# NJUVISION/PCGCv2

Measured on AMD Instinct MI355X. Metric: encode+decode Mpoints/sec at fixed bpp (r3 ckpt), vox10 frame, higher is better.
Workload: dtype f32

## Files before the change

### include/pcgc_hip.h

```cpp
#ifndef PCGC_HIP_H
#define PCGC_HIP_H

#include <stddef.h>
#include <stdint.h>

#ifdef __cplusplus
extern "C" {
#endif

const char* pcgc_last_error(void);
int pcgc_version(void);

int64_t pcgc_hash_capacity(int64_t n);
int pcgc_hash_clear(uint64_t* keys , int32_t* vals , int64_t cap, void* stream);
int pcgc_hash_insert(const int32_t* coords , int64_t n, int32_t stride, uint64_t* keys, int32_t* vals,
                     int64_t cap, void* stream);
int pcgc_hash_insert_policy(const int32_t* coords, int64_t n, int32_t stride, uint64_t* keys, int32_t* vals, int64_t cap,
                            int keep_last, void* stream);
int pcgc_hash_first_mask(const int32_t* coords, int64_t n, int32_t stride, const uint64_t* keys, const int32_t* vals,
                         int64_t cap, uint8_t* keep , int32_t* first_row , void* stream);

int pcgc_coords_check_order(const int32_t* coords , int64_t n, int32_t* out2 , void* stream);

int pcgc_coords_quantize(const int32_t* coords, int64_t n, int32_t stride_out, int32_t* out , void* stream);
int pcgc_coords_children(const int32_t* coords, int64_t n, int32_t stride_in, int32_t* out , void* stream);
int pcgc_coords_scale(const int32_t* coords, int64_t n, float factor, int32_t* out , void* stream);

size_t pcgc_scan_workspace_bytes(int64_t n);
int pcgc_mask_scan(const uint8_t* mask , int64_t n, int32_t* prefix , int32_t* total ,
                   void* workspace , size_t workspace_bytes, void* stream);
int pcgc_mask_scan_zeroed(const uint8_t* mask, int64_t n, int32_t* prefix, int32_t* total, void* workspace, size_t workspace_bytes,
                          void* stream);
int pcgc_compact_coords(const int32_t* coords, const uint8_t* mask, const int32_t* prefix, int64_t n,
                        int32_t* out , void* stream);
int pcgc_compact_feats(const float* in, int C, int in_ld, const uint8_t* mask, const int32_t* prefix, int64_t n,
                       float* out , void* stream);

int pcgc_kmap_k3(const int32_t* coords, int64_t n, int32_t stride, const uint64_t* keys, const int32_t* vals,
                 int64_t cap, int32_t* nbr , void* stream);

int pcgc_kmap_k3_children(const int32_t* parent_nbr, int64_t n_parent, int32_t* nbr , void* stream);
int pcgc_kmap_k3_prune(const int32_t* cand_nbr , int64_t n_cand, const uint8_t* mask, const int32_t* prefix,
                       const int32_t* orig , int64_t n_out, int32_t* nbr , void* stream);
int pcgc_kmap_k3_prune_parent(const int32_t* parent_nbr , int64_t n_parent, const uint8_t* mask,
                              const int32_t* prefix, const int32_t* orig, int64_t n_out, int32_t* nbr , void* stream);
int pcgc_kmap_k3_from_coarse(const int32_t* fine , int64_t n_fine, int32_t stride_fine,
                             const int32_t* parent_of , const int32_t* coarse_nbr ,
                             const int32_t* down , int64_t n_coarse, int32_t* nbr ,
                             void* stream);
int pcgc_down_maps(const int32_t* fine, const int32_t* first_row, const int32_t* prefix, int64_t n_fine, int32_t stride_fine,
                   int64_t n_coarse, int32_t* parent_of , int32_t* down , void* stream);
int pcgc_down_prepare(const int32_t* fine , int64_t n, int32_t stride_fine, int32_t* q ,
                      uint64_t* keys, int32_t* vals, int64_t cap, uint8_t* keep , int32_t* first_row ,
                      int32_t* prefix , int32_t* total , void* scan_ws, size_t scan_ws_bytes, void* stream);
int pcgc_down_finish(const int32_t* fine, const int32_t* q, const uint8_t* keep, const int32_t* first_row, const int32_t* prefix,
                     int64_t n, int32_t stride_fine, int64_t n_coarse, int32_t* coarse ,
                     int32_t* parent_of , int32_t* down , void* stream);
int pcgc_down_level(const int32_t* fine , int64_t n, int32_t stride_fine, int32_t* q, uint64_t* keys, int32_t* vals,
                    int64_t cap, uint8_t* keep, int32_t* first_row, int32_t* prefix, int32_t* total, void* scan_ws,
                    size_t scan_ws_bytes, int32_t* coarse , int32_t* parent_of ,
                    int32_t* down , int64_t* n_coarse_out , void* stream);
size_t pcgc_pyramid_scratch_bytes(int64_t n, int levels);
int pcgc_pyramid(const int32_t* fine , int64_t n, int32_t stride, int levels, void* scratch, size_t scratch_bytes,
                 int32_t* const* coarse, int32_t* const* parent_of, int32_t* const* down, int64_t* counts , void* stream);
int pcgc_compact_index(const uint8_t* mask, const int32_t* prefix, int64_t n, int32_t* orig , void* stream);

int pcgc_conv_gather(const int32_t* nbr, int K, int64_t n_out, const float* in, int64_t n_in , int Cin,
                     int in_ld, int in_coff, const float* W, const float* bias, const float* residual, int res_ld,
                     int res_coff, int relu, float* out, int Cout, int out_ld, int out_coff, void* stream);
int pcgc_last_conv_impl(void);
int pcgc_conv_gather_unit(const int32_t* nbr , int K, int64_t n_out, const float* W, const float* bias, int relu,
                          float* out, int Cout, int out_ld, void* stream);
int pcgc_conv_unit_from_coarse(const int32_t* fine , int64_t n_fine, int32_t stride_fine, const int32_t* parent_of,
                               const int32_t* coarse_nbr , const int32_t* down , int64_t n_coarse,
                               const float* W , const float* bias, int relu, float* out, int Cout, int out_ld, void* stream);
int pcgc_set_conv_impl(int impl);
int pcgc_set_up2_impl(int mfma);
int pcgc_irn_block(const int32_t* nbr , int64_t n, const float* x , int C, int x_ld,
                   const float* const* params, float* t_scratch, float* out, int out_ld, void* stream);
int pcgc_irn_pass(const int32_t* nbr, int64_t n, const float* x, int C, int x_ld, const float* const* params,
                  float* t_scratch, float* out, int out_ld, int pass, void* stream);
int pcgc_conv_up2(int64_t n_in, const float* in, int Cin, int in_ld, const float* W , const float* bias,
                  int relu, float* out , int Cout, void* stream);
int pcgc_conv_up2_gather(int64_t n_in, const float* in, int Cin, int in_ld, const int32_t* rows, const float* W ,
                         const float* bias, int relu, float* out , int Cout, void* stream);

int pcgc_conv_child(const int32_t* parent_nbr , int64_t n_parent, const float* in ,
                    int Cin, int in_ld, const float* table , int64_t table_bytes,
                    const float* bias, const float* residual, int res_ld, int relu, float* out, int Cout, int out_ld, void* stream);
int pcgc_irn_child_pass(const int32_t* parent_nbr, int64_t n_parent, int C, int pass, const float* in, int in_ld,
                        const float* table, int64_t table_bytes, const float* b0, const float* b1, const float* b2,
                        const float* x, int x_ld, float* out, int out_ld, void* stream);
int pcgc_irn_child_q4(const int32_t* parent_nbr, int64_t n_parent, int C, int pass, const float* in, int in_ld,
                      const float* table, int64_t table_bytes, const float* b0, const float* b1, const float* b2,
                      const float* x, int x_ld, float* out, int out_ld, void* stream);
int pcgc_cls_child_q4(const int32_t* parent_nbr, int64_t n_parent, const float* in, int Cin, int in_ld, const float* table,
                      int64_t table_bytes, const float* bias, float* out, void* stream);
int pcgc_irn_rows_pass(const int32_t* nbr, int64_t n, int C, int pass, const float* in, int in_ld, const float* table,
                       int64_t table_bytes, const float* b0, const float* b1, const float* b2, const float* x, int x_ld, float* out,
                       int out_ld, void* stream);
int pcgc_irn_rows_q4_pass(const int32_t* nbr, int64_t n, int C, int pass, const float* in, int in_ld, const float* table,
                          int64_t table_bytes, const float* b0, const float* b1, const float* b2, const float* x, int x_ld, float* out,
                          int out_ld, void* stream);
int pcgc_set_rows_q4_variant(int v);
int pcgc_conv_rows(const int32_t* nbr, int64_t n, const float* in, int Cin, int in_ld, const float* table, int64_t table_bytes,
                   const float* bias, const float* residual, int res_ld, int relu, float* out, int Cout, int out_ld, void* stream);
int pcgc_conv_down_rows(const int32_t* down, int64_t n_coarse, const float* in, int64_t n_in, int Cin, int in_ld, const float* table,
                        int64_t table_bytes, const float* bias, int relu, float* out, int Cout, int out_ld, void* stream);

int pcgc_conv_packed64(const int32_t* nbr, int64_t n, const float* in, int in_ld, const float* table, int64_t table_bytes,
                       const float* bias, int relu, float* out, int out_ld, void* stream);
int pcgc_set_packed_tuning(int rows, int waves);

int pcgc_set_convention(int what, int value);

size_t pcgc_topk_workspace_bytes(int64_t n);
int pcgc_topk_mask(const float* logits , int ld, int64_t n, int64_t k, uint8_t* mask ,
                   void* workspace, size_t workspace_bytes, void* stream);
int pcgc_topk_mask_segments(const float* logits, int ld, int nseg, const int64_t* seg_rows, const int64_t* seg_k, uint8_t* mask,
                            void* workspace, size_t workspace_bytes, void* stream);
size_t pcgc_topk_select_workspace_bytes(int64_t n);
int pcgc_topk_select(const float* logits , int ld, int nseg, const int64_t* seg_rows, const int64_t* seg_k,
                     const int32_t* coords, const int32_t* parent_coords, int32_t parent_stride,
                     uint8_t* bits, int32_t* wprefix, int32_t* orig, int32_t* out_coords, void* workspace, size_t workspace_bytes, void* stream);
int pcgc_kmap_k3_prune_sel(const int32_t* cand_nbr , int64_t n_cand, const uint8_t* bits, const int32_t* wprefix,
                           const int32_t* orig , int64_t n_out, int32_t* nbr , void* stream);
int pcgc_kmap_k3_prune_parent_sel(const int32_t* parent_nbr , int64_t n_parent, const uint8_t* bits, const int32_t* wprefix,
                                  const int32_t* orig, int64_t n_out, int32_t* nbr , void* stream);
int pcgc_gather_rows_f32_ld(const float* in, int C, int in_ld, const int32_t* orig, int64_t n_out, float* out , void* stream);
int pcgc_batch_counts(const int32_t* coords , int64_t n, int32_t* counts , void* stream);

size_t pcgc_sort_workspace_bytes(int64_t n);
int pcgc_sort_zyx(const int32_t* coords, int64_t n, int32_t* perm , void* workspace, size_t workspace_bytes,
                  void* stream);
int pcgc_sort_bzyx(const int32_t* coords, int64_t n, int32_t* perm , void* workspace, size_t workspace_bytes, void* stream);
int pcgc_gather_rows_i32x4(const int32_t* in, const int32_t* perm, int64_t n, int32_t* out, void* stream);
int pcgc_gather_rows_f32(const float* in, int C, const int32_t* perm, int64_t n, float* out, void* stream);

int pcgc_relu(const float* in, int64_t count, float* out, void* stream);
int pcgc_add(const float* a, const float* b, int64_t count, float* out, void* stream);

int pcgc_round_minmax(const float* feats, int64_t count, float* minmax , void* stream);
int pcgc_symbolize(const float* feats, int64_t count, float min_v, int16_t* sym , void* stream);
int pcgc_desymbolize(const int16_t* sym, int64_t count, float min_v, float* feats, void* stream);
int pcgc_quantize_symbols(const float* feats, int64_t count, float* minmax , int16_t* sym , void* stream);
int pcgc_quantize_symbols_segments(const float* feats, int C, int nseg, const int64_t* seg_rows, float* minmax, int16_t* sym, void* stream);
int pcgc_cdf_table(const float* params , int C, float min_v, float max_v, uint16_t* cdf_u16 ,
                   float* cdf_f32 , void* stream);


size_t pcgc_loss_workspace_bytes(int64_t elements);
int pcgc_hash_contains(const int32_t* coords , int64_t n, const uint64_t* keys, const int32_t* vals, int64_t cap,
                       const uint8_t* or_mask , uint8_t* mask , void* stream);
int pcgc_eb_likelihood(const float* feats, int ld, int64_t n, int C, const float* params , float bound, float* likelihood,
                       double* bits, void* workspace, size_t workspace_bytes, void* stream);
int pcgc_neg_log2_sum(const float* x, int ld, int64_t n, int C, double* bits , void* workspace, size_t workspace_bytes, void* stream);
int pcgc_bce_logits(const float* logits, int64_t ld, int64_t n, const uint8_t* truth , const uint8_t* pred ,
                    double* bce, int64_t* counts, void* workspace, size_t workspace_bytes, void* stream);

size_t pcgc_occ_workspace_bytes(int64_t n);
int pcgc_occ_symbols(const float* logits, int64_t ld, int64_t n, const uint8_t* truth , uint16_t* packed ,
                     int64_t* sums , void* workspace, size_t workspace_bytes, void* stream);
int pcgc_occ_tables(uint16_t* p1, int32_t* cost);

size_t pcgc_occ_rans_workspace_bytes(int64_t n, int steps);
int pcgc_occ_rans_encode(const uint16_t* packed , int64_t n, int steps, const int64_t* sums , uint8_t* payload,
                         size_t payload_capacity, int64_t* host3, void* workspace, size_t workspace_bytes, void* stream);
int pcgc_occ_rans_decode(const uint16_t* packed , int64_t n, const uint8_t* payload, int64_t payload_bytes, int steps,
                         uint8_t* mask , int64_t* host2, void* workspace, size_t workspace_bytes, void* stream);

size_t pcgc_conv_wgrad_workspace_bytes(int K, int64_t n_rows, int Cin, int Cout);
int64_t pcgc_conv_wgrad_rows_per_group(int K, int64_t n_rows, int Cin, int Cout);
int pcgc_conv_wgrad(const int32_t* nbr, int K, int64_t n_out, const float* x, int64_t n_in, int Cin, int x_ld, const float* gy, int Cout,
                    int gy_ld, float* gW, float* gb, void* workspace, size_t workspace_bytes, void* stream);
int pcgc_conv_up2_wgrad(int64_t n_in, const float* x, int64_t x_rows, int Cin, int x_ld, const int32_t* rows, const float* gy, int Cout,
                        int gy_ld, float* gW, float* gb, void* workspace, size_t workspace_bytes, void* stream);
int pcgc_kmap_invert(const int32_t* nbr, int K, int64_t n_out, int64_t n_in, int32_t* inv , void* stream);
int pcgc_relu_bwd(const float* g, int g_ld, const float* y, int y_ld, int64_t n, int C, float* out, int out_ld, void* stream);
int pcgc_scatter_rows(const float* gy, int C, int gy_ld, const int32_t* orig, int64_t n_rows, float* gx, int64_t n_out, int gx_ld, void* stream);
int pcgc_bce_logits_bwd(const float* logits, int64_t ld, int64_t n, const uint8_t* truth, double scale, float* g , void* stream);
size_t pcgc_eb_bwd_workspace_bytes(int64_t n, int C);
int pcgc_eb_likelihood_bwd(const float* feats, int ld, int64_t n, int C, const float* params , float bound, double scale,
                           float* gy, float* gparams, void* workspace, size_t workspace_bytes, void* stream);

int64_t pcgc_rc_encode(const uint16_t* cdf , int C, int Lp, const int16_t* sym , int64_t n,
                       uint8_t* out , int64_t cap);
int pcgc_rc_decode(const uint16_t* cdf, int C, int Lp, const uint8_t* in, int64_t nbytes, int16_t* sym, int64_t n);
#define PCGC_RC_CKPT_WORDS 6
int64_t pcgc_rc_encode_indexed(const uint16_t* cdf, int C, int Lp, const int16_t* sym, int64_t n, uint8_t* out, int64_t cap, int n_ckpt,
                               uint32_t* ckpt );
int pcgc_rc_decode_indexed(const uint16_t* cdf, int C, int Lp, const uint8_t* in, int64_t nbytes, int16_t* sym, int64_t n, int n_ckpt,
                           const uint32_t* ckpt);
int64_t pcgc_rc_encode_ctx(const uint16_t* cdf , int R, int Lp, const uint16_t* ctx , const int16_t* sym ,
                           int64_t n, uint8_t* out , int64_t cap);
int pcgc_rc_decode_ctx(const uint16_t* cdf, int R, int Lp, const uint16_t* ctx , const uint8_t* in, int64_t nbytes,
                       int16_t* sym , int64_t n);
int pcgc_set_rc_threads(int threads);
int pcgc_set_rc_lanes(int mode);
int pcgc_set_rc_impl(int impl);

int64_t pcgc_oct_encode(const int32_t* xyz , int64_t n, uint8_t* out, int64_t cap);
int64_t pcgc_oct_decode_count(const uint8_t* in, int64_t nbytes);
int pcgc_oct_decode(const uint8_t* in, int64_t nbytes, int32_t* xyz , int64_t n);
int pcgc_set_oct_tiled(int on);
int pcgc_set_oct_model(int model);
int pcgc_oct_warm(void);

int pcgc_d1_nn(const int32_t* a , int64_t na, const uint64_t* b_keys, const int32_t* b_vals, int64_t b_cap,
               const int32_t* offsets , int n_offsets, double* sum , uint64_t* max_d2 ,
               int32_t* unresolved , void* stream);
int pcgc_d1_cell_masks(const int32_t* b , int64_t nb, const uint64_t* cell_keys, const int32_t* cell_vals, int64_t cell_cap,
                       uint64_t* masks , int64_t n_cells, void* stream);
int pcgc_d1_nn_cells(const int32_t* a , int64_t na, const uint64_t* cell_keys, const int32_t* cell_vals, int64_t cell_cap,
                     const uint64_t* masks, const int32_t* offsets , int n_offsets, int32_t reach2, double* sum, uint64_t* max_d2,
                     int32_t* unresolved, void* stream);

int pcgc_d2_runs(const int32_t* qs , int64_t nq, int32_t* runlen , void* stream);
int pcgc_d2_count(const int32_t* p , int64_t n, const int32_t* sel, const uint64_t* cell_keys, const int32_t* cell_vals,
                  int64_t cell_cap, const uint64_t* masks, const uint64_t* keys, const int32_t* vals, int64_t cap, const int32_t* runlen,
                  const int32_t* offsets , int n_offsets, int32_t reach2, int64_t* best , int32_t* cnt ,
                  int32_t* unresolved , int32_t* n_unresolved , void* stream);
int pcgc_d2_fill(const int32_t* p, int64_t n, const int32_t* sel, const uint64_t* cell_keys, const int32_t* cell_vals, int64_t cell_cap,
                 const uint64_t* masks, const uint64_t* keys, const int32_t* vals, int64_t cap, const int32_t* runlen, const int32_t* perm,
                 const int32_t* offsets, int n_offsets, int32_t reach2, const int64_t* best, const int64_t* seg , int32_t* rows, void* stream);
int pcgc_d2_exhaustive(const int32_t* p, int64_t n, const int32_t* sel, const int32_t* qs, int64_t nq, const int32_t* perm, int fill,
                       int64_t* best, int32_t* cnt, const int64_t* seg, int32_t* rows, int32_t* n_empty , void* stream);
size_t pcgc_d2_scan_workspace_bytes(int64_t n);
int pcgc_d2_scan(const int32_t* cnt , int64_t n, int64_t* seg , void* workspace, size_t workspace_bytes, void* stream);
int pcgc_d2_segment_lowest(const int64_t* seg, int64_t n, int32_t* rows, int32_t cap, int32_t* kept, void* stream);
int pcgc_d2_recv_count(const int64_t* seg, const int32_t* kept, int64_t na, const int32_t* rows, int64_t nb, int32_t* rcnt, void* stream);
int pcgc_d2_recv_fill(const int64_t* seg, const int32_t* kept, int64_t na, const int32_t* rows, int64_t nb, const int64_t* rseg, int32_t* cursor,
                      int32_t* recv, void* stream);
int pcgc_d2_normals(const int64_t* rseg, const int32_t* recv, int64_t nb, const double* na, const int64_t* seg_ba, const int32_t* kept_ba,
                    const int32_t* rows_ba, double* nb_out, void* stream);
int pcgc_d2_c2p(const int32_t* p, int64_t n, const int32_t* q, const double* nq, const int64_t* seg, const int32_t* kept, const int32_t* rows,
                double* c2p, void* stream);
size_t pcgc_d2_reduce_workspace_bytes(void);
int pcgc_d2_reduce(const int64_t* c2c, const double* c2p, int64_t n, int64_t* c2c_sum_max, double* c2p_sum, void* workspace, size_t workspace_bytes,
                   void* stream);

size_t pcgc_attr_transfer_workspace_bytes(int64_t ns, int64_t nt, int channels);
int pcgc_attr_transfer(const int64_t* seg_st, const int32_t* kept_st, const int32_t* rows_st, int64_t ns, const int64_t* seg_ts,
                       const int32_t* kept_ts, const int32_t* rows_ts, int64_t nt, const uint8_t* attr_s, int channels, uint8_t* attr_t,
                       void* workspace, size_t workspace_bytes, void* stream);
int pcgc_colour_dist(const uint8_t* cp, int64_t n, const uint8_t* cq, int64_t nq, const int64_t* seg, const int32_t* kept, const int32_t* rows,
                     int64_t* yuv2, int32_t* rgb2, void* stream);
size_t pcgc_colour_reduce_workspace_bytes(void);
int pcgc_colour_reduce(const int64_t* yuv2, const int32_t* rgb2, int64_t n, int64_t* out, void* workspace, size_t workspace_bytes, void* stream);

int64_t pcgc_normals_ball_masks(int32_t r2, uint64_t* table );
size_t pcgc_normals_workspace_bytes(int64_t n);
int pcgc_normals_estimate(const int32_t* coords , int64_t n, const int32_t* qs , const int32_t* perm,
                          const uint64_t* cell_keys, const int32_t* cell_vals, int64_t cell_cap, const uint64_t* masks, const uint64_t* keys,
                          const int32_t* vals, int64_t cap, const int32_t* runlen, const uint64_t* ball , int32_t r2, int orient,
                          const double* viewpoint , int64_t* moments , double* normals ,
                          double* lam , int32_t* count , uint8_t* valid , void* workspace,
                          size_t workspace_bytes, void* stream);
int pcgc_set_normals_mapping(int mode);

int64_t pcgc_ply_read_ascii_geo(const char* path, int32_t* xyz , int64_t cap);
int pcgc_ply_write_ascii_geo(const char* path, const int32_t* xyz , int64_t n);
int pcgc_ply_write_ascii_geo_rgb(const char* path, const int32_t* xyz , const uint8_t* rgb , int64_t n);

typedef int (*pcgc_table_fn)(const float* params, int C, float min_v, float max_v, uint16_t* table_u16, float* cdf_f32);
int pcgc_items_encode(int n_items, const char* const* stems, const int16_t* sym, const int32_t* xyz, const int64_t* rows, const float* ranges,
                      int C, const int32_t* counts, const float* eb_params, pcgc_table_fn table_fn, int index_segments, int write_coords,
                      int threads);
int pcgc_items_probe(int n_items, const char* const* stems, int64_t* rows, int32_t* channels, float* ranges, int32_t* counts,
                     int32_t* native_coords);
int pcgc_items_decode(int n_items, const char* const* stems, const int64_t* rows, int C, const float* ranges, const int32_t* native_coords,
                      const float* eb_params, pcgc_table_fn table_fn, int use_sidecar, int16_t* sym, int32_t* xyz, int coord_layout,
                      int coord_scale, int threads);

int pcgc_level_prepare_children(const int32_t* coords, int64_t n, int32_t stride, uint64_t* keys, int32_t* vals, int64_t cap, int32_t* nbr,
                                int32_t* children, int32_t* nbr_children, void* stream);

int pcgc_frame_decode(const char* stem, int C, const float* eb_params, pcgc_table_fn table_fn, int use_sidecar, int coord_scale,
                      int64_t cap_rows, int16_t* sym, int32_t* level, int64_t* info, float* range, int threads);
int pcgc_frame_decode_begin(const char* stem, int C, const float* eb_params, pcgc_table_fn table_fn, int use_sidecar, int coord_scale,
                            int64_t cap_rows, int16_t* sym, int32_t* level, int64_t* info, float* range, int threads);
int pcgc_frame_decode_end(void);
int pcgc_frame_worker_test(int delay_us);

int pcgc_table_cache(int mode);

uint32_t pcgc_crc32(uint32_t crc, const uint8_t* buf, int64_t len);

int pcgc_mesh_read(const char* path, double* verts , int64_t vcap, int32_t* faces , int64_t fcap,
                   int64_t* counts );
size_t pcgc_mesh_cdf_workspace_bytes(int64_t T);
int pcgc_mesh_area_cdf(const double* verts , int64_t V, const int32_t* faces , int64_t T,
                       double* cdf , int32_t* bad_faces , void* workspace, size_t workspace_bytes, void* stream);
int pcgc_mesh_sample(const double* verts, int64_t V, const int32_t* faces, const double* cdf, int64_t T, uint64_t seed, uint64_t first,
                     int64_t n, int32_t* tri , double* points , void* stream);
size_t pcgc_mesh_voxelize_workspace_bytes(int32_t resolution);
int pcgc_mesh_voxelize(const double* verts, int64_t V, const int32_t* faces, const double* cdf, int64_t T, uint64_t seed, int64_t n,
                       const double* R , int32_t resolution, int32_t* out , int64_t cap,
                       int32_t* count , void* workspace , size_t workspace_bytes, void* stream);

#define PCGC_COLLATE_MAX_ITEMS 16
typedef struct pcgc_collate_item {
    int64_t offset;
    int32_t first_row, rows, width, symmetry, extent, reserved;
} pcgc_collate_item;
int pcgc_collate_rows(const uint8_t* arena , const pcgc_collate_item* items , int n_items,
                      int32_t* coords_out , float* feats_out , void* stream);

#ifdef __cplusplus
}
#endif
#endif
```

### pcgcv2_amd/_build.py

```python
import os
import subprocess
import sys
from concurrent.futures import ThreadPoolExecutor

HERE = os.path.dirname(os.path.abspath(__file__))
CSRC = os.path.join(HERE, 'csrc')
VARIANT = os.environ.get('PCGC_BUILD_VARIANT', '')
OBJ = os.path.join(CSRC, '_obj' + ('_' + VARIANT if VARIANT else ''))
LIB = os.path.join(HERE, 'libpcgc_hip' + ('_' + VARIANT if VARIANT else '') + '.so')
SOURCES = ['coords.hip', 'select.hip', 'conv.hip', 'child_conv.hip', 'child_conv32.hip', 'child_cls_w.hip', 'child_irn.hip', 'child_irn_a16.hip', 'child_irn_b16.hip',
           'child_irn_a32.hip', 'child_irn_b32.hip', 'child_q4.hip', 'rows_irn.hip', 'rows_q4.hip', 'conv_packed.hip', 'entropy.hip', 'loss.hip', 'occupancy.hip', 'occupancy_rans.hip', 'grad.hip', 'metric.hip', 'colour.hip', 'normals.hip', 'mesh.hip', 'collate.hip', 'hostcodec.cpp', 'ply.cpp', 'mesh_io.cpp']
HEADERS = [os.path.join(CSRC, 'pcgc_common.h'), os.path.join(CSRC, 'mfma_util.h'), os.path.join(CSRC, 'child_kernels.h'), os.path.join(CSRC, 'child_q4.h'), os.path.join(CSRC, 'q4x.h'), os.path.join(CSRC, 'q4x_sched.h'), os.path.join(CSRC, 'rows_q4_policy.h'), os.path.join(CSRC, 'eb_logits.h'), os.path.join(CSRC, 'occupancy_tables.h'), os.path.join(HERE, '..', 'include', 'pcgc_hip.h')]
FLAGS = ['--offload-arch=gfx950', '-O3', '-std=c++17', '-ffp-contract=off', '-fPIC', '-Wall', '-Wno-unused-result'] + \
        os.environ.get('PCGC_EXTRA_HIPCC_FLAGS', '').split()


def _hipcc():
    for c in (os.environ.get('HIPCC'), '/opt/rocm/bin/hipcc', 'hipcc'):
        if c and (os.path.isabs(c) and os.path.exists(c) or not os.path.isabs(c)):
            return c
    return 'hipcc'


def _stale(target, deps):
    if not os.path.exists(target):
        return True
    t = os.path.getmtime(target)
    return any(os.path.getmtime(d) > t for d in deps)


def build(force=False, verbose=False):
    os.makedirs(OBJ, exist_ok=True)
    if VARIANT:
        import shutil
        base = os.path.join(CSRC, '_obj')
        for src in SOURCES:
            o = src.rsplit('.', 1)[0] + '.o'
            if 'child_kernels.h' not in open(os.path.join(CSRC, src)).read() and os.path.exists(os.path.join(base, o)) \
                    and not os.path.exists(os.path.join(OBJ, o)):
                shutil.copy2(os.path.join(base, o), os.path.join(OBJ, o))
    hipcc = _hipcc()
    jobs = []
    only = [t for t in os.environ.get('PCGC_BUILD_ONLY', '').split(',') if t]
    for src in SOURCES:
        s = os.path.join(CSRC, src)
        o = os.path.join(OBJ, src.rsplit('.', 1)[0] + '.o')
        if only and os.path.exists(o):
            if src.rsplit('.', 1)[0] in only:
                jobs.append((o, [hipcc] + FLAGS + (['-x', 'hip'] if src.endswith('.hip') else []) + ['-c', s, '-o', o]))
            continue
        if force or _stale(o, [s] + HEADERS):
            lang = ['-x', 'hip'] if src.endswith('.hip') else []
            jobs.append((o, [hipcc] + FLAGS + lang + ['-c', s, '-o', o]))

    def run(job):
        o, cmd = job
        if verbose:
            print(' '.join(cmd), file=sys.stderr)
        r = subprocess.run(cmd, capture_output=True, text=True)
        if r.returncode != 0:
            raise RuntimeError('hipcc failed:\n' + ' '.join(cmd) + '\n' + r.stderr[-4000:])
        return o

    with ThreadPoolExecutor(max_workers=max(2, min(8, os.cpu_count() or 4))) as ex:
        list(ex.map(run, jobs))
    objs = [os.path.join(OBJ, s.rsplit('.', 1)[0] + '.o') for s in SOURCES]
    if force or jobs or _stale(LIB, objs):
        cmd = [hipcc, '--offload-arch=gfx950', '-shared', '-fPIC', '-o', LIB] + objs + ['-lz']
        r = subprocess.run(cmd, capture_output=True, text=True)
        if r.returncode != 0:
            raise RuntimeError('link failed:\n' + r.stderr[-4000:])
    if not VARIANT:
        build_reftable(force=force)
    return LIB


REFTABLE_LIB = os.path.join(HERE, 'libpcgc_reftable.so')


def build_reftable(force=False):
    src = os.path.join(CSRC, 'reftable.cpp')
    if not (force or _stale(REFTABLE_LIB, [src])):
        return REFTABLE_LIB
    import torch
    tdir = os.path.dirname(torch.__file__)
    cmd = ['g++', '-O2', '-std=c++17', '-fPIC', '-shared', f'-D_GLIBCXX_USE_CXX11_ABI={int(torch._C._GLIBCXX_USE_CXX11_ABI)}',
           '-I' + os.path.join(tdir, 'include'), '-I' + os.path.join(tdir, 'include', 'torch', 'csrc', 'api', 'include'), src,
           '-o', REFTABLE_LIB, '-L' + os.path.join(tdir, 'lib'), '-ltorch_cpu', '-lc10', '-Wl,-rpath,' + os.path.join(tdir, 'lib')]
    r = subprocess.run(cmd, capture_output=True, text=True)
    if r.returncode != 0:
        raise RuntimeError('g++ failed:\n' + ' '.join(cmd) + '\n' + r.stderr[-4000:])
    return REFTABLE_LIB


if __name__ == '__main__':
    print(build(force='--force' in sys.argv, verbose=True))
```

### pcgcv2_amd/_lib.py

```python
import ctypes as C
import os

_HERE = os.path.dirname(os.path.abspath(__file__))
LIB_PATH = os.environ.get('PCGC_LIB') or os.path.join(_HERE, 'libpcgc_hip.so')

vp, i64, i32, f32, sz = C.c_void_p, C.c_int64, C.c_int32, C.c_float, C.c_size_t
ci = C.c_int

SIGNATURES = {
    'pcgc_last_error': (C.c_char_p, []),
    'pcgc_version': (ci, []),
    'pcgc_hash_capacity': (i64, [i64]),
    'pcgc_hash_clear': (ci, [vp, vp, i64, vp]),
    'pcgc_hash_insert': (ci, [vp, i64, i32, vp, vp, i64, vp]),
    'pcgc_hash_insert_policy': (ci, [vp, i64, i32, vp, vp, i64, ci, vp]),
    'pcgc_set_convention': (ci, [ci, ci]),
    'pcgc_hash_first_mask': (ci, [vp, i64, i32, vp, vp, i64, vp, vp, vp]),
    'pcgc_coords_check_order': (ci, [vp, i64, vp, vp]),
    'pcgc_coords_quantize': (ci, [vp, i64, i32, vp, vp]),
    'pcgc_coords_children': (ci, [vp, i64, i32, vp, vp]),
    'pcgc_coords_scale': (ci, [vp, i64, f32, vp, vp]),
    'pcgc_scan_workspace_bytes': (sz, [i64]),
    'pcgc_mask_scan': (ci, [vp, i64, vp, vp, vp, sz, vp]),
    'pcgc_mask_scan_zeroed': (ci, [vp, i64, vp, vp, vp, sz, vp]),
    'pcgc_compact_coords': (ci, [vp, vp, vp, i64, vp, vp]),
    'pcgc_compact_feats': (ci, [vp, ci, ci, vp, vp, i64, vp, vp]),
    'pcgc_kmap_k3': (ci, [vp, i64, i32, vp, vp, i64, vp, vp]),
    'pcgc_kmap_k3_children': (ci, [vp, i64, vp, vp]),
    'pcgc_kmap_k3_prune': (ci, [vp, i64, vp, vp, vp, i64, vp, vp]),
    'pcgc_kmap_k3_prune_parent': (ci, [vp, i64, vp, vp, vp, i64, vp, vp]),
    'pcgc_kmap_k3_from_coarse': (ci, [vp, i64, i32, vp, vp, vp, i64, vp, vp]),
    'pcgc_down_maps': (ci, [vp, vp, vp, i64, i32, i64, vp, vp, vp]),
    'pcgc_down_prepare': (ci, [vp, i64, i32, vp, vp, vp, i64, vp, vp, vp, vp, vp, sz, vp]),
    'pcgc_down_finish': (ci, [vp, vp, vp, vp, vp, i64, i32, i64, vp, vp, vp, vp]),
    'pcgc_down_level': (ci, [vp, i64, i32, vp, vp, vp, i64, vp, vp, vp, vp, vp, sz, vp, vp, vp, vp, vp]),
    'pcgc_pyramid_scratch_bytes': (sz, [i64, ci]),
    'pcgc_pyramid': (ci, [vp, i64, i32, ci, vp, sz, vp, vp, vp, vp, vp]),
    'pcgc_compact_index': (ci, [vp, vp, i64, vp, vp]),
    'pcgc_conv_gather': (ci, [vp, ci, i64, vp, i64, ci, ci, ci, vp, vp, vp, ci, ci, ci, vp, ci, ci, ci, vp]),
    'pcgc_conv_gather_unit': (ci, [vp, ci, i64, vp, vp, ci, vp, ci, ci, vp]),
    'pcgc_conv_unit_from_coarse': (ci, [vp, i64, i32, vp, vp, vp, i64, vp, vp, ci, vp, ci, ci, vp]),
    'pcgc_set_conv_impl': (ci, [ci]),
    'pcgc_last_conv_impl': (ci, []),
    'pcgc_set_up2_impl': (ci, [ci]),
    'pcgc_irn_block': (ci, [vp, i64, vp, ci, ci, vp, vp, vp, ci, vp]),
    'pcgc_irn_pass': (ci, [vp, i64, vp, ci, ci, vp, vp, vp, ci, ci, vp]),
    'pcgc_conv_child': (ci, [vp, i64, vp, ci, ci, vp, i64, vp, vp, ci, ci, vp, ci, ci, vp]),
    'pcgc_irn_child_pass': (ci, [vp, i64, ci, ci, vp, ci, vp, i64, vp, vp, vp, vp, ci, vp, ci, vp]),
    'pcgc_irn_child_q4': (ci, [vp, i64, ci, ci, vp, ci, vp, i64, vp, vp, vp, vp, ci, vp, ci, vp]),
    'pcgc_cls_child_q4': (ci, [vp, i64, vp, ci, ci, vp, i64, vp, vp, vp]),
    'pcgc_conv_down_rows': (ci, [vp, i64, vp, i64, ci, ci, vp, i64, vp, ci, vp, ci, ci, vp]),
    'pcgc_conv_rows': (ci, [vp, i64, vp, ci, ci, vp, i64, vp, vp, ci, ci, vp, ci, ci, vp]),
    'pcgc_irn_rows_pass': (ci, [vp, i64, ci, ci, vp, ci, vp, i64, vp, vp, vp, vp, ci, vp, ci, vp]),
    'pcgc_irn_rows_q4_pass': (ci, [vp, i64, ci, ci, vp, ci, vp, i64, vp, vp, vp, vp, ci, vp, ci, vp]),
    'pcgc_set_rows_q4_variant': (ci, [ci]),
    'pcgc_conv_packed64': (ci, [vp, i64, vp, ci, vp, i64, vp, ci, vp, ci, vp]),
    'pcgc_set_packed_tuning': (ci, [ci, ci]),
    'pcgc_conv_up2': (ci, [i64, vp, ci, ci, vp, vp, ci, vp, ci, vp]),
    'pcgc_conv_up2_gather': (ci, [i64, vp, ci, ci, vp, vp, vp, ci, vp, ci, vp]),
    'pcgc_topk_workspace_bytes': (sz, [i64]),
    'pcgc_topk_mask': (ci, [vp, ci, i64, i64, vp, vp, sz, vp]),
    'pcgc_topk_mask_segments': (ci, [vp, ci, ci, vp, vp, vp, vp, sz, vp]),
    'pcgc_topk_select_workspace_bytes': (sz, [i64]),
    'pcgc_topk_select': (ci, [vp, ci, ci, vp, vp, vp, vp, i32, vp, vp, vp, vp, vp, sz, vp]),
    'pcgc_kmap_k3_prune_sel': (ci, [vp, i64, vp, vp, vp, i64, vp, vp]),
    'pcgc_kmap_k3_prune_parent_sel': (ci, [vp, i64, vp, vp, vp, i64, vp, vp]),
    'pcgc_gather_rows_f32_ld': (ci, [vp, ci, ci, vp, i64, vp, vp]),
    'pcgc_batch_counts': (ci, [vp, i64, vp, vp]),
    'pcgc_sort_bzyx': (ci, [vp, i64, vp, vp, sz, vp]),
    'pcgc_quantize_symbols_segments': (ci, [vp, ci, ci, vp, vp, vp, vp]),
    'pcgc_sort_workspace_bytes': (sz, [i64]),
    'pcgc_sort_zyx': (ci, [vp, i64, vp, vp, sz, vp]),
    'pcgc_gather_rows_i32x4': (ci, [vp, vp, i64, vp, vp]),
    'pcgc_gather_rows_f32': (ci, [vp, ci, vp, i64, vp, vp]),
    'pcgc_relu': (ci, [vp, i64, vp, vp]),
    'pcgc_add': (ci, [vp, vp, i64, vp, vp]),
    'pcgc_round_minmax': (ci, [vp, i64, vp, vp]),
    'pcgc_symbolize': (ci, [vp, i64, f32, vp, vp]),
    'pcgc_desymbolize': (ci, [vp, i64, f32, vp, vp]),
    'pcgc_quantize_symbols': (ci, [vp, i64, vp, vp, vp]),
    'pcgc_cdf_table': (ci, [vp, ci, f32, f32, vp, vp, vp]),
    'pcgc_loss_workspace_bytes': (sz, [i64]),
    'pcgc_hash_contains': (ci, [vp, i64, vp, vp, i64, vp, vp, vp]),
    'pcgc_eb_likelihood': (ci, [vp, ci, i64, ci, vp, f32, vp, vp, vp, sz, vp]),
    'pcgc_neg_log2_sum': (ci, [vp, ci, i64, ci, vp, vp, sz, vp]),
    'pcgc_bce_logits': (ci, [vp, i64, i64, vp, vp, vp, vp, vp, sz, vp]),
    'pcgc_occ_workspace_bytes': (sz, [i64]),
    'pcgc_occ_symbols': (ci, [vp, i64, i64, vp, vp, vp, vp, sz, vp]),
    'pcgc_occ_tables': (ci, [vp, vp]),
    'pcgc_occ_rans_workspace_bytes': (sz, [i64, ci]),
    'pcgc_occ_rans_encode': (ci, [vp, i64, ci, vp, vp, sz, vp, vp, sz, vp]),
    'pcgc_occ_rans_decode': (ci, [vp, i64, vp, i64, ci, vp, vp, vp, sz, vp]),
    'pcgc_conv_wgrad_workspace_bytes': (sz, [ci, i64, ci, ci]),
    'pcgc_conv_wgrad_rows_per_group': (i64, [ci, i64, ci, ci]),
    'pcgc_conv_wgrad': (ci, [vp, ci, i64, vp, i64, ci, ci, vp, ci, ci, vp, vp, vp, sz, vp]),
    'pcgc_conv_up2_wgrad': (ci, [i64, vp, i64, ci, ci, vp, vp, ci, ci, vp, vp, vp, sz, vp]),
    'pcgc_kmap_invert': (ci, [vp, ci, i64, i64, vp, vp]),
    'pcgc_relu_bwd': (ci, [vp, ci, vp, ci, i64, ci, vp, ci, vp]),
    'pcgc_scatter_rows': (ci, [vp, ci, ci, vp, i64, vp, i64, ci, vp]),
    'pcgc_bce_logits_bwd': (ci, [vp, i64, i64, vp, C.c_double, vp, vp]),
    'pcgc_eb_bwd_workspace_bytes': (sz, [i64, ci]),
    'pcgc_eb_likelihood_bwd': (ci, [vp, ci, i64, ci, vp, f32, C.c_double, vp, vp, vp, sz, vp]),
    'pcgc_d1_cell_masks': (ci, [vp, i64, vp, vp, i64, vp, i64, vp]),
    'pcgc_d1_nn_cells': (ci, [vp, i64, vp, vp, i64, vp, vp, ci, i32, vp, vp, vp, vp]),
    'pcgc_d1_nn': (ci, [vp, i64, vp, vp, i64, vp, ci, vp, vp, vp, vp]),
    'pcgc_d2_runs': (ci, [vp, i64, vp, vp]),
    'pcgc_d2_count': (ci, [vp, i64, vp, vp, vp, i64, vp, vp, vp, i64, vp, vp, ci, i32, vp, vp, vp, vp, vp]),
    'pcgc_d2_fill': (ci, [vp, i64, vp, vp, vp, i64, vp, vp, vp, i64, vp, vp, vp, ci, i32, vp, vp, vp, vp]),
    'pcgc_d2_exhaustive': (ci, [vp, i64, vp, vp, i64, vp, ci, vp, vp, vp, vp, vp, vp]),
    'pcgc_d2_scan_workspace_bytes': (sz, [i64]),
    'pcgc_d2_scan': (ci, [vp, i64, vp, vp, sz, vp]),
    'pcgc_d2_segment_lowest': (ci, [vp, i64, vp, i32, vp, vp]),
    'pcgc_d2_recv_count': (ci, [vp, vp, i64, vp, i64, vp, vp]),
    'pcgc_d2_recv_fill': (ci, [vp, vp, i64, vp, i64, vp, vp, vp, vp]),
    'pcgc_d2_normals': (ci, [vp, vp, i64, vp, vp, vp, vp, vp, vp]),
    'pcgc_d2_c2p': (ci, [vp, i64, vp, vp, vp, vp, vp, vp, vp]),
    'pcgc_d2_reduce_workspace_bytes': (sz, []),
    'pcgc_d2_reduce': (ci, [vp, vp, i64, vp, vp, vp, sz, vp]),
    'pcgc_attr_transfer_workspace_bytes': (sz, [i64, i64, ci]),
    'pcgc_attr_transfer': (ci, [vp, vp, vp, i64, vp, vp, vp, i64, vp, ci, vp, vp, sz, vp]),
    'pcgc_colour_dist': (ci, [vp, i64, vp, i64, vp, vp, vp, vp, vp, vp]),
    'pcgc_colour_reduce_workspace_bytes': (sz, []),
    'pcgc_colour_reduce': (ci, [vp, vp, i64, vp, vp, sz, vp]),
    'pcgc_normals_ball_masks': (i64, [i32, vp]),
    'pcgc_normals_workspace_bytes': (sz, [i64]),
    'pcgc_normals_estimate': (ci, [vp, i64, vp, vp, vp, vp, i64, vp, vp, vp, i64, vp, vp, i32, ci, vp, vp, vp, vp, vp, vp, vp, sz, vp]),
    'pcgc_set_normals_mapping': (ci, [ci]),
    'pcgc_rc_encode': (i64, [vp, ci, ci, vp, i64, vp, i64]),
    'pcgc_rc_decode': (ci, [vp, ci, ci, vp, i64, vp, i64]),
    'pcgc_set_rc_impl': (ci, [ci]),
    'pcgc_rc_encode_indexed': (i64, [vp, ci, ci, vp, i64, vp, i64, ci, vp]),
    'pcgc_rc_decode_indexed': (ci, [vp, ci, ci, vp, i64, vp, i64, ci, vp]),
    'pcgc_rc_encode_ctx': (i64, [vp, ci, ci, vp, vp, i64, vp, i64]),
    'pcgc_rc_decode_ctx': (ci, [vp, ci, ci, vp, vp, i64, vp, i64]),
    'pcgc_set_rc_threads': (ci, [ci]),
    'pcgc_set_rc_lanes': (ci, [ci]),
    'pcgc_set_oct_tiled': (ci, [ci]),
    'pcgc_set_oct_model': (ci, [ci]),
    'pcgc_oct_warm': (ci, []),
    'pcgc_oct_encode': (i64, [vp, i64, vp, i64]),
    'pcgc_oct_decode_count': (i64, [vp, i64]),
    'pcgc_oct_decode': (ci, [vp, i64, vp, i64]),
    'pcgc_items_encode': (ci, [ci, vp, vp, vp, vp, vp, ci, vp, vp, vp, ci, ci, ci]),
    'pcgc_items_probe': (ci, [ci, vp, vp, vp, vp, vp, vp]),
    'pcgc_items_decode': (ci, [ci, vp, vp, ci, vp, vp, vp, vp, ci, vp, vp, ci, ci, ci]),
    'pcgc_level_prepare_children': (ci, [vp, i64, i32, vp, vp, i64, vp, vp, vp, vp]),
    'pcgc_frame_decode': (ci, [C.c_char_p, ci, vp, vp, ci, ci, i64, vp, vp, vp, vp, ci]),
    'pcgc_frame_decode_begin': (ci, [C.c_char_p, ci, vp, vp, ci, ci, i64, vp, vp, vp, vp, ci]),
    'pcgc_frame_decode_end': (ci, []),
    'pcgc_frame_worker_test': (ci, [ci]),
    'pcgc_table_cache': (ci, [ci]),
    'pcgc_crc32': (C.c_uint32, [C.c_uint32, vp, i64]),
    'pcgc_ply_read_ascii_geo': (i64, [C.c_char_p, vp, i64]),
    'pcgc_ply_write_ascii_geo': (ci, [C.c_char_p, vp, i64]),
    'pcgc_ply_write_ascii_geo_rgb': (ci, [C.c_char_p, vp, vp, i64]),
    'pcgc_mesh_read': (ci, [C.c_char_p, vp, i64, vp, i64, vp]),
    'pcgc_mesh_cdf_workspace_bytes': (sz, [i64]),
    'pcgc_mesh_area_cdf': (ci, [vp, i64, vp, i64, vp, vp, vp, sz, vp]),
    'pcgc_mesh_sample': (ci, [vp, i64, vp, vp, i64, C.c_uint64, C.c_uint64, i64, vp, vp, vp]),
    'pcgc_mesh_voxelize_workspace_bytes': (sz, [i32]),
    'pcgc_mesh_voxelize': (ci, [vp, i64, vp, vp, i64, C.c_uint64, i64, vp, i32, vp, i64, vp, vp, sz, vp]),
    'pcgc_collate_rows': (ci, [vp, vp, ci, vp, vp, vp]),
}


class CollateItem(C.Structure):
    _fields_ = [('offset', i64), ('first_row', i32), ('rows', i32), ('width', i32), ('symmetry', i32), ('extent', i32), ('reserved', i32)]


class PcgcError(RuntimeError):
    pass


_lib = None


def lib():
    global _lib
    if _lib is None:
        if not os.path.exists(LIB_PATH):
            raise PcgcError(f'{LIB_PATH} not found: run `python -c "import __graft_entry__ as g; g.build()"` '
                            '(hipcc --offload-arch=gfx950). The HIP library is mandatory; there is no fallback path.')
        l = C.CDLL(LIB_PATH)
        for name, (res, args) in SIGNATURES.items():
            fn = getattr(l, name)
            fn.restype, fn.argtypes = res, args
        _lib = l
    return _lib


REFTABLE_PATH = os.path.join(_HERE, 'libpcgc_reftable.so')
_reftable = None


def reftable_lib():
    global _reftable
    if _reftable is None:
        if not os.path.exists(REFTABLE_PATH):
            raise PcgcError(f'{REFTABLE_PATH} not found: run `python -c "import __graft_entry__ as g; g.build()"`')
        import torch
        l = C.CDLL(REFTABLE_PATH)
        l.pcgc_reference_table.restype = ci
        l.pcgc_reference_table.argtypes = [vp, ci, f32, f32, vp, vp]
        l.pcgc_reference_table_clear.restype = ci
        l.pcgc_reference_table_clear.argtypes = []
        _reftable = l
    return _reftable


def check(rc, what=''):
    if rc != 0:
        raise PcgcError(f'{what or "pcgc call"} failed ({rc}): {lib().pcgc_last_error().decode()}')
```

### pcgcv2_amd/autoencoder.py

```python
import torch

from . import derived, dispatch, ops
from .nn import MinkowskiConvolution as Conv, MinkowskiGenerativeConvolutionTranspose as UpConv, MinkowskiPruning
from .sparse import CoordMap, SparseTensor


class InceptionResNet(torch.nn.Module):

    def __init__(self, channels):
        super().__init__()
        c = channels
        self.conv0_0 = Conv(c, c // 4, 3)
        self.conv0_1 = Conv(c // 4, c // 2, 3)
        self.conv1_0 = Conv(c, c // 4, 1)
        self.conv1_1 = Conv(c // 4, c // 4, 3)
        self.conv1_2 = Conv(c // 4, c // 2, 1)

    def forward(self, x):
        c = x.F.shape[1]
        children = x.cmap.origin is not None and x.cmap.origin[0] == 'children'
        fam = dispatch.select('irn', (c,), x.F.shape[0], 'children' if children else 'plain', extent=x.F.shape[0] * max(c, x.F.stride(0)) * 4,
                              contiguous=x.F.is_contiguous()).family
        if fam != 'unfused':
            params = [p for m in (self.conv0_0, self.conv0_1, self.conv1_0, self.conv1_1, self.conv1_2) for p in (m.kernel, m.bias)]
            if fam == 'rows64':
                y = ops.irn_block_rows64(x.cmap.k3, x.F, params, self._tables('child', ops.child_irn_tables, params))
            elif fam == 'child':
                big = x.F.shape[0] >= 8 * ops.PATH.CHILD_Q4_MIN_PARENTS
                q4 = self._tables('q4', ops.child_q4_tables, params) if (c == 16 and ops.PATH.CHILD_Q4 and big) else None
                y = ops.irn_block_child(x.cmap.origin[1].k3, x.F, params, self._tables('child', ops.child_irn_tables, params), q4_table=q4)
            elif fam == 'rows32q4':
                y = ops.irn_block_rows32_q4(x.cmap.k3, x.F, params, self._tables('rows_q4', ops.rows_q4_tables, params))
            elif fam == 'rows32':
                y = ops.irn_block_rows32(x.cmap.k3, x.F, params, self._tables('rows32', ops.rows_irn32_tables, params))
            else:
                y = ops.irn_block(x.cmap.k3, x.F, params)
            return SparseTensor(y, coordinate_map=x.cmap)
        out = torch.empty_like(x.F)
        a = self.conv0_0(x, relu=True)
        self.conv0_1(a, out=out[:, :c // 2], residual=x.F[:, :c // 2])
        b = self.conv1_1(self.conv1_0(x, relu=True), relu=True)
        self.conv1_2(b, out=out[:, c // 2:], residual=x.F[:, c // 2:])
        return SparseTensor(out, coordinate_map=x.cmap)

    def _tables(self, kind, build, params):
        return derived.fetch(self.__dict__.setdefault('_derived', {}), kind, params, lambda: build(params))

    def _drop_derived(self):
        self.__dict__.pop('_derived', None)

    def weights_changed(self):
        derived.weights_changed(self)


def make_layer(block, block_layers, channels):
    return torch.nn.Sequential(*[block(channels=channels) for _ in range(block_layers)])


class Encoder(torch.nn.Module):

    def __init__(self, channels=[1, 16, 32, 64, 32, 8]):
        super().__init__()
        ch = channels
        self.conv0 = Conv(ch[0], ch[1], 3)
        self.down0 = Conv(ch[1], ch[2], 2, 2)
        self.block0 = make_layer(InceptionResNet, 3, ch[2])
        self.conv1 = Conv(ch[2], ch[2], 3)
        self.down1 = Conv(ch[2], ch[3], 2, 2)
        self.block1 = make_layer(InceptionResNet, 3, ch[3])
        self.conv2 = Conv(ch[3], ch[3], 3)
        self.down2 = Conv(ch[3], ch[4], 2, 2)
        self.block2 = make_layer(InceptionResNet, 3, ch[4])
        self.conv3 = Conv(ch[4], ch[5], 3)

    def forward(self, x):
        out0 = self.block0(self.down0(self.conv0(x, relu=True), relu=True))
        out1 = self.block1(self.down1(self.conv1(out0, relu=True), relu=True))
        out2 = self.block2(self.down2(self.conv2(out1, relu=True), relu=True))
        out2 = self.conv3(out2)
        return [out2, out1, out0]


class Decoder(torch.nn.Module):

    def __init__(self, channels=[8, 64, 32, 16]):
        super().__init__()
        ch = channels
        for l in range(3):
            setattr(self, f'up{l}', UpConv(ch[l], ch[l + 1], 2, 2))
            setattr(self, f'conv{l}', Conv(ch[l + 1], ch[l + 1], 3))
            setattr(self, f'block{l}', make_layer(InceptionResNet, 3, ch[l + 1]))
            setattr(self, f'conv{l}_cls', Conv(ch[l + 1], 1, 3))
        self.pruning = MinkowskiPruning()

    def prune_voxel(self, data, data_cls, nums, ground_truth=None, training=False):
        if training:
            return self._prune_voxel_training(data, data_cls, nums, ground_truth)
        cand = data.cmap
        rows = [len(data_cls)] if len(nums) == 1 else cand.batch_rows
        if len(rows) != len(nums):
            raise ValueError(f'prune_voxel: {len(nums)} budgets for a batch of {len(rows)} items')
        keep = [int(min(r, max(int(n), 0))) for r, n in zip(rows, nums)]
        if dispatch.select('prune', (data.F.shape[1],), len(data_cls)).family != 'select':
            mask = ops.topk_mask(data_cls.F, keep[0]) if len(nums) == 1 else ops.topk_mask_segments(data_cls.F, rows, keep)
            return self.pruning(data, mask, n_keep=sum(keep), keep_per_item=None if len(nums) == 1 else keep)
        if cand._C is None and cand.origin is not None and cand.origin[0] == 'children':
            parent = cand.origin[1]
            bits, wprefix, orig, coords = ops.topk_select(data_cls.F, rows, keep, parent_coords=parent.C, parent_stride=parent.stride)
        else:
            bits, wprefix, orig, coords = ops.topk_select(data_cls.F, rows, keep, coords=cand.C)
        cmap = CoordMap(coords, cand.stride, unique=True, origin=('selected', cand, bits, wprefix, orig))
        if len(nums) > 1:
            cmap._batch_rows = list(keep)
        src = data.F
        out = SparseTensor(lambda: ops.gather_rows(src, orig), coordinate_map=cmap)
        out._F_rows = (src, orig)
        return out

    def _prune_voxel_training(self, data, data_cls, nums, ground_truth):
        if ground_truth is None:
            raise ValueError('prune_voxel(training=True) needs the ground truth of the level')
        from .data_utils import isin_mask
        cand = data.cmap
        rows = [len(data_cls)] if len(nums) == 1 else cand.batch_rows
        if len(rows) != len(nums):
            raise ValueError(f'prune_voxel: {len(nums)} budgets for a batch of {len(rows)} items')
        keep = [int(min(r, max(int(n), 0))) for r, n in zip(rows, nums)]
        topk = ops.topk_mask(data_cls.F, keep[0]) if len(nums) == 1 else ops.topk_mask_segments(data_cls.F, rows, keep)
        mask = isin_mask(cand.C, ground_truth, or_mask=topk)
        return self.pruning(data, mask)

    def forward(self, x, nums_list, ground_truth_list=(None, None, None), training=False):
        out, cls_list = x, []
        for l in range(3):
            out = getattr(self, f'up{l}')(out, relu=True)
            out = getattr(self, f'conv{l}')(out, relu=True)
            out = getattr(self, f'block{l}')(out)
            cls = getattr(self, f'conv{l}_cls')(out)
            cls_list.append(cls)
            out = self.prune_voxel(out, cls, nums_list[l], ground_truth_list[l], training)
        return cls_list, out
```

### pcgcv2_amd/csrc/coords.hip

```cpp
#include <stdarg.h>
#include "pcgc_common.h"

static thread_local char g_err[512] = "";
void pcgc_set_error(const char* fmt, ...) {
    va_list ap; va_start(ap, fmt); vsnprintf(g_err, sizeof(g_err), fmt, ap); va_end(ap);
}
extern "C" const char* pcgc_last_error(void) { return g_err; }
extern "C" int pcgc_version(void) { return 1; }

extern "C" int64_t pcgc_hash_capacity(int64_t n) {
    int64_t cap = 1024;
    while (cap < 2 * n) cap <<= 1;
    return cap;
}

__global__ void k_hash_clear(uint64_t* keys, int32_t* vals, int64_t cap) {
    int64_t i = (int64_t)blockIdx.x * blockDim.x + threadIdx.x;
    if (i < cap) { keys[i] = PCGC_EMPTY_KEY; vals[i] = 0x7fffffff; }
}

__global__ void k_hash_insert(const int4* __restrict__ coords, int64_t n, uint64_t* keys, int32_t* vals, uint64_t cap_mask) {
    int64_t i = (int64_t)blockIdx.x * blockDim.x + threadIdx.x;
    int4 c = make_int4(-1, -1, -1, -1);
    if (i < n) c = coords[i];
// ... 29 lines not shown
                if (seen == old) break;
                old = seen;
            }
            return;
        }
        h = (h + 1) & cap_mask;
    }
}
__global__ void k_hash_first_mask(const int4* __restrict__ coords, int64_t n, const uint64_t* __restrict__ keys,
                                  const int32_t* __restrict__ vals, uint64_t cap_mask, uint8_t* keep, int32_t* first_row) {
    int64_t i = (int64_t)blockIdx.x * blockDim.x + threadIdx.x;
    if (i >= n) return;
    int4 c = coords[i];
    int32_t f = hash_lookup(keys, vals, cap_mask, c.x, c.y, c.z, c.w);
    keep[i] = f == (int32_t)i;
    if (first_row) first_row[i] = f;
}

__global__ void k_coords_check_order(const int4* __restrict__ coords, int64_t n, int32_t* __restrict__ out2) {
    int64_t i = (int64_t)blockIdx.x * blockDim.x + threadIdx.x;
    bool oob = false, desc = false;
    if (i < n) {
        const int4 c = coords[i];
        oob = !coord_in_range(c.x, c.y, c.z, c.w);
        if (i > 0) {
            const int4 p = coords[i - 1];
            desc = coord_key(c.x & 15, c.y & 0xFFFFF, c.z & 0xFFFFF, c.w & 0xFFFFF) < coord_key(p.x & 15, p.y & 0xFFFFF, p.z & 0xFFFFF, p.w & 0xFFFFF);
        }
    }
    const unsigned long long b = __ballot(oob), d = __ballot(desc);
    if ((threadIdx.x & 63) == 0) {
        if (b) atomicAdd(out2, (int32_t)__popcll(b));
        if (d) atomicAdd(out2 + 1, (int32_t)__popcll(d));
    }
}
extern "C" int pcgc_coords_check_order(const int32_t* coords, int64_t n, int32_t* out2, void* stream) {
    PCGC_REQUIRE(out2 != nullptr, "null counters");
    hipMemsetAsync(out2, 0, 2 * sizeof(int32_t), S(stream));
    if (n > 0) hipLaunchKernelGGL(k_coords_check_order, dim3(grid_for(n, 256)), dim3(256), 0, S(stream), (const int4*)coords, n, out2);
    PCGC_CHECK_LAUNCH("coords_check_order");
    return 0;
}
extern "C" int pcgc_hash_clear(uint64_t* keys, int32_t* vals, int64_t cap, void* stream) {
    PCGC_REQUIRE(cap > 0 && (cap & (cap - 1)) == 0, "capacity must be a power of two");
    hipLaunchKernelGGL(k_hash_clear, dim3(grid_for(cap, 256)), dim3(256), 0, S(stream), keys, vals, cap);
    PCGC_CHECK_LAUNCH("hash_clear");
    return 0;
}
extern "C" int pcgc_hash_insert(const int32_t* coords, int64_t n, int32_t stride, uint64_t* keys, int32_t* vals, int64_t cap,
                                void* stream) {
    (void)stride;
    PCGC_REQUIRE(cap >= 2 * n && (cap & (cap - 1)) == 0, "capacity must be a power of two >= 2n");
    if (n == 0) return 0;
    hipLaunchKernelGGL(k_hash_insert, dim3(grid_for(n, 256)), dim3(256), 0, S(stream), (const int4*)coords, n,
                       keys, vals, (uint64_t)(cap - 1));
    PCGC_CHECK_LAUNCH("hash_insert");
    return 0;
}
extern "C" int pcgc_hash_insert_policy(const int32_t* coords, int64_t n, int32_t stride, uint64_t* keys, int32_t* vals, int64_t cap,
                                       int keep_last, void* stream) {
    if (!keep_last) return pcgc_hash_insert(coords, n, stride, keys, vals, cap, stream);
    PCGC_REQUIRE(cap >= 2 * n && (cap & (cap - 1)) == 0, "capacity must be a power of two >= 2n");
    if (n == 0) return 0;
    hipLaunchKernelGGL(k_hash_insert_last, dim3(grid_for(n, 256)), dim3(256), 0, S(stream), (const int4*)coords, n,
                       keys, vals, (uint64_t)(cap - 1));
    PCGC_CHECK_LAUNCH("hash_insert_policy");
    return 0;
}
extern "C" int pcgc_hash_first_mask(const int32_t* coords, int64_t n, int32_t stride, const uint64_t* keys,
                                    const int32_t* vals, int64_t cap, uint8_t* keep, int32_t* first_row, void* stream) {
    (void)stride;
    if (n == 0) return 0;
    hipLaunchKernelGGL(k_hash_first_mask, dim3(grid_for(n, 256)), dim3(256), 0, S(stream), (const int4*)coords, n,
                       keys, vals, (uint64_t)(cap - 1), keep, first_row);
    PCGC_CHECK_LAUNCH("hash_first_mask");
    return 0;
}

__global__ void k_coords_quantize(const int4* __restrict__ in, int64_t n, int32_t s, int4* out) {
    int64_t i = (int64_t)blockIdx.x * blockDim.x + threadIdx.x;
    if (i >= n) return;
    int4 c = in[i];
    auto fl = [s](int32_t v) { return (v >= 0 ? v / s : -((-v + s - 1) / s)) * s; };
    out[i] = make_int4(c.x, fl(c.y), fl(c.z), fl(c.w));
}
__global__ void k_coords_children(const int4* __restrict__ in, int64_t n, int32_t h, int4* out) {
    int64_t t = (int64_t)blockIdx.x * blockDim.x + threadIdx.x;
    if (t >= 8 * n) return;
    int4 c = in[t >> 3]; int k = (int)(t & 7);
    out[t] = make_int4(c.x, c.y + (k & 1) * h, c.z + ((k >> 1) & 1) * h, c.w + (k >> 2) * h);
}
__global__ void k_coords_scale(const int4* __restrict__ in, int64_t n, float f, int4* out) {
    int64_t i = (int64_t)blockIdx.x * blockDim.x + threadIdx.x;
    if (i >= n) return;
    int4 c = in[i];
    out[i] = make_int4(c.x, (int32_t)rintf((float)c.y * f), (int32_t)rintf((float)c.z * f), (int32_t)rintf((float)c.w * f));
}
extern "C" int pcgc_coords_quantize(const int32_t* coords, int64_t n, int32_t stride_out, int32_t* out, void* stream) {
    PCGC_REQUIRE(stride_out > 0, "stride must be positive");
    if (n == 0) return 0;
    hipLaunchKernelGGL(k_coords_quantize, dim3(grid_for(n, 256)), dim3(256), 0, S(stream), (const int4*)coords, n,
                       stride_out, (int4*)out);
    PCGC_CHECK_LAUNCH("coords_quantize");
    return 0;
}
extern "C" int pcgc_coords_children(const int32_t* coords, int64_t n, int32_t stride_in, int32_t* out, void* stream) {
    PCGC_REQUIRE(stride_in >= 2 && (stride_in & 1) == 0, "input stride must be even");
    if (n == 0) return 0;
    hipLaunchKernelGGL(k_coords_children, dim3(grid_for(8 * n, 256)), dim3(256), 0, S(stream), (const int4*)coords, n,
                       stride_in / 2, (int4*)out);
    PCGC_CHECK_LAUNCH("coords_children");
    return 0;
}
extern "C" int pcgc_coords_scale(const int32_t* coords, int64_t n, float factor, int32_t* out, void* stream) {
    if (n == 0) return 0;
    hipLaunchKernelGGL(k_coords_scale, dim3(grid_for(n, 256)), dim3(256), 0, S(stream), (const int4*)coords, n, factor,
                       (int4*)out);
    PCGC_CHECK_LAUNCH("coords_scale");
    return 0;
}

__global__ void __launch_bounds__(256) k_kmap_k3(const int4* __restrict__ coords, int64_t n, int32_t s,
                                                 const uint64_t* __restrict__ keys, const int32_t* __restrict__ vals,
                                                 uint64_t cap_mask, int32_t* __restrict__ nbr) {
    int64_t t = (int64_t)blockIdx.x * blockDim.x + threadIdx.x;
    if (t >= 27 * n) return;
    int k = (int)(t / n); int64_t o = t - (int64_t)k * n;
    int4 c = coords[o];
    int dx = (k % 3 - 1) * s, dy = ((k / 3) % 3 - 1) * s, dz = (k / 9 - 1) * s;
    nbr[t] = (k == 13) ? (int32_t)o : hash_lookup(keys, vals, cap_mask, c.x, c.y + dx, c.z + dy, c.w + dz);
}
extern "C" int pcgc_kmap_k3(const int32_t* coords, int64_t n, int32_t stride, const uint64_t* keys, const int32_t* vals,
                            int64_t cap, int32_t* nbr, void* stream) {
    if (n == 0) return 0;
    hipLaunchKernelGGL(k_kmap_k3, dim3(grid_for(27 * n, 256)), dim3(256), 0, S(stream), (const int4*)coords, n, stride,
                       keys, vals, (uint64_t)(cap - 1), nbr);
    PCGC_CHECK_LAUNCH("kmap_k3");
    return 0;
}

__global__ void __launch_bounds__(256) k_kmap_children(const int32_t* __restrict__ pnbr, int64_t np, int32_t* __restrict__ nbr) {
    int64_t c = (int64_t)blockIdx.x * blockDim.x + threadIdx.x;
    int64_t n = 8 * np;
    if (c >= n) return;
    int64_t i = c >> 3; int j = (int)(c & 7);
#pragma unroll
    for (int k = 0; k < 27; ++k) {
        int kp, jn; child_offset(j, k, kp, jn);
        int32_t pn = pnbr[(int64_t)kp * np + i];
        nbr[(int64_t)k * n + c] = pn < 0 ? -1 : 8 * pn + jn;
    }
}
__global__ void __launch_bounds__(256) k_kmap_prune(const int32_t* __restrict__ cand, int64_t n_cand,
                                                    const uint8_t* __restrict__ mask, const int32_t* __restrict__ prefix,
                                                    const int32_t* __restrict__ orig, int64_t n_out, int32_t* __restrict__ nbr) {
    int64_t r = (int64_t)blockIdx.x * blockDim.x + threadIdx.x;
    if (r >= n_out) return;
    int64_t o = orig[r];
#pragma unroll
    for (int k = 0; k < 27; ++k) {
        int32_t m = cand[(int64_t)k * n_cand + o];
        nbr[(int64_t)k * n_out + r] = (m >= 0 && mask[m]) ? prefix[m] : -1;
    }
}
__global__ void __launch_bounds__(256) k_kmap_prune_parent(const int32_t* __restrict__ pnbr, int64_t np,
                                                           const uint8_t* __restrict__ mask, const int32_t* __restrict__ prefix,
                                                           const int32_t* __restrict__ orig, int64_t n_out, int32_t* __restrict__ nbr) {
    int64_t r = (int64_t)blockIdx.x * blockDim.x + threadIdx.x;
    if (r >= n_out) return;
    const int64_t o = orig[r];
    const int64_t i = o >> 3; const int j = (int)(o & 7);
#pragma unroll
    for (int k = 0; k < 27; ++k) {
        int kp, jn; child_offset(j, k, kp, jn);
        const int32_t pn = pnbr[(int64_t)kp * np + i];
        const int64_t m = pn < 0 ? -1 : 8 * (int64_t)pn + jn;
        nbr[(int64_t)k * n_out + r] = (m >= 0 && mask[m]) ? prefix[m] : -1;
    }
}
__global__ void __launch_bounds__(256) k_kmap_prune_sel(const int32_t* __restrict__ cand, int64_t n_cand, const uint64_t* __restrict__ bits,
                                                        const int32_t* __restrict__ wprefix, const int32_t* __restrict__ orig,
                                                        int64_t n_out, int32_t* __restrict__ nbr) {
    int64_t r = (int64_t)blockIdx.x * blockDim.x + threadIdx.x;
    if (r >= n_out) return;
    int64_t o = orig[r];
#pragma unroll
    for (int k = 0; k < 27; ++k) {
        int32_t m = cand[(int64_t)k * n_cand + o];
        nbr[(int64_t)k * n_out + r] = m >= 0 ? sel_rank(bits, wprefix, m) : -1;
    }
}
__global__ void __launch_bounds__(256) k_kmap_prune_parent_sel(const int32_t* __restrict__ pnbr, int64_t np, const uint64_t* __restrict__ bits,
                                                               const int32_t* __restrict__ wprefix, const int32_t* __restrict__ orig,
                                                               int64_t n_out, int32_t* __restrict__ nbr) {
    int64_t r = (int64_t)blockIdx.x * blockDim.x + threadIdx.x;
    if (r >= n_out) return;
    const int64_t o = orig[r];
    const int64_t i = o >> 3; const int j = (int)(o & 7);
#pragma unroll
    for (int k = 0; k < 27; ++k) {
        int kp, jn; child_offset(j, k, kp, jn);
        const int32_t pn = pnbr[(int64_t)kp * np + i];
        nbr[(int64_t)k * n_out + r] = pn < 0 ? -1 : sel_rank(bits, wprefix, 8 * (int64_t)pn + jn);
    }
}
__global__ void __launch_bounds__(256) k_kmap_from_coarse(const int4* __restrict__ fine, int64_t nf, int32_t stride_f,
                                                          const int32_t* __restrict__ parent_of,
                                                          const int32_t* __restrict__ pnbr, const int32_t* __restrict__ down,
                                                          int64_t nc, int32_t* __restrict__ nbr) {
    int64_t c = (int64_t)blockIdx.x * blockDim.x + threadIdx.x;
    if (c >= nf) return;
    int4 q = fine[c];
    int j = ((q.y / stride_f) & 1) | (((q.z / stride_f) & 1) << 1) | (((q.w / stride_f) & 1) << 2);
    int64_t p = parent_of[c];
#pragma unroll
    for (int k = 0; k < 27; ++k) {
        int32_t r;
        if (k == 13) r = (int32_t)c;
        else {
            int kp, jn; child_offset(j, k, kp, jn);
            int32_t pn = pnbr[(int64_t)kp * nc + p];
            r = pn < 0 ? -1 : down[(int64_t)jn * nc + pn];
        }
        nbr[(int64_t)k * nf + c] = r;
    }
}
__global__ void k_down_maps(const int4* __restrict__ fine, const int32_t* __restrict__ first_row,
                            const int32_t* __restrict__ prefix, int64_t nf, int32_t stride_f, int64_t nc,
                            int32_t* __restrict__ parent_of, int32_t* __restrict__ down) {
    int64_t c = (int64_t)blockIdx.x * blockDim.x + threadIdx.x;
    if (c >= nf) return;
    int4 q = fine[c];
    int j = ((q.y / stride_f) & 1) | (((q.z / stride_f) & 1) << 1) | (((q.w / stride_f) & 1) << 2);
    int32_t p = prefix[first_row[c]];
    parent_of[c] = p;
    down[(int64_t)j * nc + p] = (int32_t)c;
}
__global__ void k_compact_index(const uint8_t* __restrict__ mask, const int32_t* __restrict__ prefix, int64_t n, int32_t* orig) {
    int64_t i = (int64_t)blockIdx.x * blockDim.x + threadIdx.x;
    if (i < n && mask[i]) orig[prefix[i]] = (int32_t)i;
}

extern "C" int pcgc_kmap_k3_children(const int32_t* parent_nbr, int64_t n_parent, int32_t* nbr, void* stream) {
    if (n_parent == 0) return 0;
    hipLaunchKernelGGL(k_kmap_children, dim3(grid_for(8 * n_parent, 256)), dim3(256), 0, S(stream), parent_nbr, n_parent, nbr);
    PCGC_CHECK_LAUNCH("kmap_k3_children");
    return 0;
}
extern "C" int pcgc_kmap_k3_prune(const int32_t* cand_nbr, int64_t n_cand, const uint8_t* mask, const int32_t* prefix,
                                  const int32_t* orig, int64_t n_out, int32_t* nbr, void* stream) {
    if (n_out == 0) return 0;
    hipLaunchKernelGGL(k_kmap_prune, dim3(grid_for(n_out, 256)), dim3(256), 0, S(stream), cand_nbr, n_cand, mask, prefix, orig,
                       n_out, nbr);
    PCGC_CHECK_LAUNCH("kmap_k3_prune");
    return 0;
}
extern "C" int pcgc_kmap_k3_prune_parent(const int32_t* parent_nbr, int64_t n_parent, const uint8_t* mask, const int32_t* prefix,
                                         const int32_t* orig, int64_t n_out, int32_t* nbr, void* stream) {
    if (n_out == 0) return 0;
    hipLaunchKernelGGL(k_kmap_prune_parent, dim3(grid_for(n_out, 256)), dim3(256), 0, S(stream), parent_nbr, n_parent, mask, prefix,
                       orig, n_out, nbr);
    PCGC_CHECK_LAUNCH("kmap_k3_prune_parent");
    return 0;
}
extern "C" int pcgc_kmap_k3_prune_sel(const int32_t* cand_nbr, int64_t n_cand, const uint8_t* bits, const int32_t* wprefix,
                                      const int32_t* orig, int64_t n_out, int32_t* nbr, void* stream) {
    PCGC_REQUIRE(((uintptr_t)bits & 7) == 0, "bits must be 8-byte aligned");
    if (n_out == 0) return 0;
    hipLaunchKernelGGL(k_kmap_prune_sel, dim3(grid_for(n_out, 256)), dim3(256), 0, S(stream), cand_nbr, n_cand, (const uint64_t*)bits, wprefix,
                       orig, n_out, nbr);
    PCGC_CHECK_LAUNCH("kmap_k3_prune_sel");
    return 0;
}
extern "C" int pcgc_kmap_k3_prune_parent_sel(const int32_t* parent_nbr, int64_t n_parent, const uint8_t* bits, const int32_t* wprefix,
                                             const int32_t* orig, int64_t n_out, int32_t* nbr, void* stream) {
    PCGC_REQUIRE(((uintptr_t)bits & 7) == 0, "bits must be 8-byte aligned");
    if (n_out == 0) return 0;
    hipLaunchKernelGGL(k_kmap_prune_parent_sel, dim3(grid_for(n_out, 256)), dim3(256), 0, S(stream), parent_nbr, n_parent, (const uint64_t*)bits,
                       wprefix, orig, n_out, nbr);
    PCGC_CHECK_LAUNCH("kmap_k3_prune_parent_sel");
    return 0;
}
extern "C" int pcgc_kmap_k3_from_coarse(const int32_t* fine, int64_t n_fine, int32_t stride_fine, const int32_t* parent_of,
                                        const int32_t* coarse_nbr, const int32_t* down, int64_t n_coarse, int32_t* nbr,
                                        void* stream) {
    if (n_fine == 0) return 0;
    hipLaunchKernelGGL(k_kmap_from_coarse, dim3(grid_for(n_fine, 256)), dim3(256), 0, S(stream), (const int4*)fine, n_fine,
                       stride_fine, parent_of, coarse_nbr, down, n_coarse, nbr);
    PCGC_CHECK_LAUNCH("kmap_k3_from_coarse");
    return 0;
}
extern "C" int pcgc_down_maps(const int32_t* fine, const int32_t* first_row, const int32_t* prefix, int64_t n_fine,
                              int32_t stride_fine, int64_t n_coarse, int32_t* parent_of, int32_t* down, void* stream) {
    if (n_coarse > 0) {
        hipError_t e = hipMemsetAsync(down, 0xFF, (size_t)n_coarse * 8 * sizeof(int32_t), S(stream));
        if (e != hipSuccess) { pcgc_set_error("down_maps: %s", hipGetErrorString(e)); return -1; }
    }
    if (n_fine == 0) return 0;
    hipLaunchKernelGGL(k_down_maps, dim3(grid_for(n_fine, 256)), dim3(256), 0, S(stream), (const int4*)fine, first_row, prefix,
                       n_fine, stride_fine, n_coarse, parent_of, down);
    PCGC_CHECK_LAUNCH("down_maps");
    return 0;
}
extern "C" int pcgc_down_prepare(const int32_t* fine, int64_t n, int32_t stride_fine, int32_t* q, uint64_t* keys, int32_t* vals,
                                 int64_t cap, uint8_t* keep, int32_t* first_row, int32_t* prefix, int32_t* total, void* scan_ws,
                                 size_t scan_ws_bytes, void* stream) {
    int rc;
    if ((rc = pcgc_coords_quantize(fine, n, 2 * stride_fine, q, stream))) return rc;
    if ((rc = pcgc_hash_clear(keys, vals, cap, stream))) return rc;
    if ((rc = pcgc_hash_insert(q, n, 2 * stride_fine, keys, vals, cap, stream))) return rc;
    if ((rc = pcgc_hash_first_mask(q, n, 2 * stride_fine, keys, vals, cap, keep, first_row, stream))) return rc;
    return pcgc_mask_scan(keep, n, prefix, total, scan_ws, scan_ws_bytes, stream);
}
extern "C" int pcgc_down_finish(const int32_t* fine, const int32_t* q, const uint8_t* keep, const int32_t* first_row,
                                const int32_t* prefix, int64_t n, int32_t stride_fine, int64_t n_coarse, int32_t* coarse,
                                int32_t* parent_of, int32_t* down, void* stream) {
    int rc;
    if ((rc = pcgc_compact_coords(q, keep, prefix, n, coarse, stream))) return rc;
    return pcgc_down_maps(fine, first_row, prefix, n, stride_fine, n_coarse, parent_of, down, stream);
}
extern "C" int pcgc_down_level(const int32_t* fine, int64_t n, int32_t stride_fine, int32_t* q, uint64_t* keys, int32_t* vals,
                               int64_t cap, uint8_t* keep, int32_t* first_row, int32_t* prefix, int32_t* total, void* scan_ws,
                               size_t scan_ws_bytes, int32_t* coarse, int32_t* parent_of, int32_t* down, int64_t* n_coarse_out,
                               void* stream) {
    PCGC_REQUIRE(n_coarse_out != nullptr, "null count");
    int rc = pcgc_down_prepare(fine, n, stride_fine, q, keys, vals, cap, keep, first_row, prefix, total, scan_ws, scan_ws_bytes, stream);
    if (rc) return rc;
    static thread_local int32_t* host_total = nullptr;
    if (!host_total && hipHostMalloc((void**)&host_total, 64, hipHostMallocDefault) != hipSuccess) {
        host_total = nullptr; pcgc_set_error("down_level: cannot allocate pinned memory"); return -1;
    }
    hipError_t e = hipMemcpyAsync(host_total, total, sizeof(int32_t), hipMemcpyDeviceToHost, S(stream));
    if (e == hipSuccess) e = hipStreamSynchronize(S(stream));
    if (e != hipSuccess) { pcgc_set_error("down_level: %s", hipGetErrorString(e)); return -1; }
    const int64_t n_coarse = *host_total;
    *n_coarse_out = n_coarse;
    return pcgc_down_finish(fine, q, keep, first_row, prefix, n, stride_fine, n_coarse, coarse, parent_of, down, stream);
}
constexpr int PYR_MAX = 4;
struct PyrArgs {
    uint64_t* keys[PYR_MAX]; int32_t* vals[PYR_MAX]; int32_t* first[PYR_MAX]; uint8_t* keep[PYR_MAX];
    int32_t s[PYR_MAX]; uint64_t cap_mask; int levels;
};
__device__ static inline int4 pyr_quantise(int4 c, int32_t s) { return make_int4(c.x, c.y / s * s, c.z / s * s, c.w / s * s); }
__global__ void k_pyr_insert_level(const int4* __restrict__ fine, int64_t n, PyrArgs a, int l) {
    const int64_t i = (int64_t)blockIdx.x * blockDim.x + threadIdx.x;
    int4 c = make_int4(-1, -1, -1, -1);
    bool ok = false;
    if (i < n && (l == 0 || a.keep[l - 1][i])) { c = fine[i]; ok = coord_in_range(c.x, c.y, c.z, c.w); }
    const int4 q = pyr_quantise(c, a.s[l]);
    const uint64_t key = ok ? coord_key(q.x, q.y, q.z, q.w) : PCGC_EMPTY_KEY;
    const uint64_t left = __shfl_up((unsigned long long)key, 1, 64);
    if (!ok || ((threadIdx.x & 63) != 0 && left == key)) return;
    uint64_t* keys = a.keys[l]; int32_t* vals = a.vals[l];
    uint64_t h = hash_slot(key, a.cap_mask);
    for (;;) {
        unsigned long long prev = __builtin_nontemporal_load((const unsigned long long*)&keys[h]);
        if (prev == PCGC_EMPTY_KEY) prev = atomicCAS((unsigned long long*)&keys[h], (unsigned long long)PCGC_EMPTY_KEY, (unsigned long long)key);
        if (prev == PCGC_EMPTY_KEY || prev == key) { if (__builtin_nontemporal_load(&vals[h]) > (int32_t)i) atomicMin(&vals[h], (int32_t)i); return; }
        h = (h + 1) & a.cap_mask;
    }
}
__global__ void k_pyr_first_level(const int4* __restrict__ fine, int64_t n, PyrArgs a, int l) {
    const int64_t i = (int64_t)blockIdx.x * blockDim.x + threadIdx.x;
    if (i >= n) return;
    if (l > 0 && !a.keep[l - 1][i]) { a.keep[l][i] = 0; return; }
    const int4 q = pyr_quantise(fine[i], a.s[l]);
    const int32_t f = hash_lookup(a.keys[l], a.vals[l], a.cap_mask, q.x, q.y, q.z, q.w);
    a.first[l][i] = f;
    a.keep[l][i] = f == (int32_t)i;
}

struct PyrOut { int4* coarse[PYR_MAX]; int32_t* parent_of[PYR_MAX]; int32_t* down[PYR_MAX]; const int32_t* prefix[PYR_MAX]; int64_t count[PYR_MAX]; int32_t stride; };
__global__ void k_pyr_finish(const int4* __restrict__ fine, int64_t n, PyrArgs a, PyrOut o) {
    const int64_t i = (int64_t)blockIdx.x * blockDim.x + threadIdx.x;
    if (i >= n) return;
    const int4 c = fine[i];
    bool kept_below = true; int32_t j = (int32_t)i;
#pragma unroll
    for (int l = 0; l < PYR_MAX; ++l) {
        if (l >= a.levels || !kept_below) break;
        const int32_t s_cur = o.stride << l;
        const int k = ((c.y / s_cur) & 1) | (((c.z / s_cur) & 1) << 1) | (((c.w / s_cur) & 1) << 2);
        const int32_t p = o.prefix[l][a.first[l][i]];
        o.parent_of[l][j] = p;
        o.down[l][(int64_t)k * o.count[l] + p] = j;
        kept_below = a.keep[l][i] != 0;
        if (kept_below) { o.coarse[l][p] = pyr_quantise(c, a.s[l]); j = p; }
    }
}
extern "C" size_t pcgc_pyramid_scratch_bytes(int64_t n, int levels) {
    const size_t cap = (size_t)pcgc_hash_capacity(n), scan = (pcgc_scan_workspace_bytes(n) + 15) & ~(size_t)15, nn = ((size_t)n + 15) & ~(size_t)15;
    return 64 + (size_t)levels * (scan + cap * 12 + nn * 4 * 2 + nn) + 64;
}
extern "C" int pcgc_pyramid(const int32_t* fine, int64_t n, int32_t stride, int levels, void* scratch, size_t scratch_bytes,
                            int32_t* const* coarse, int32_t* const* parent_of, int32_t* const* down, int64_t* counts, void* stream) {
    PCGC_REQUIRE(levels >= 1 && levels <= PYR_MAX, "1 to 4 levels");
    PCGC_REQUIRE(fine && scratch && coarse && parent_of && down && counts, "null argument");
    PCGC_REQUIRE(scratch_bytes >= pcgc_pyramid_scratch_bytes(n, levels) && ((uintptr_t)scratch & 15) == 0, "scratch too small or misaligned");
    PCGC_REQUIRE(stride >= 1 && (int64_t)stride << levels < ((int64_t)1 << 30), "bad stride");
    if (n == 0) { for (int l = 0; l < levels; ++l) counts[l] = 0; return 0; }
    hipStream_t s = S(stream);
    const size_t cap = (size_t)pcgc_hash_capacity(n), scan = (pcgc_scan_workspace_bytes(n) + 15) & ~(size_t)15, nn = ((size_t)n + 15) & ~(size_t)15;
    PyrArgs a; a.levels = levels; a.cap_mask = (uint64_t)cap - 1;
    int32_t* prefix[PYR_MAX]; void* scan_ws[PYR_MAX];
    char* p = (char*)scratch;
    int32_t* totals = (int32_t*)p; p += 64;
    for (int l = 0; l < levels; ++l) { scan_ws[l] = p; p += scan; }
    const size_t zero_bytes = (size_t)(p - (char*)scratch);
    uint64_t* keys0 = (uint64_t*)p;
    for (int l = 0; l < levels; ++l) { a.keys[l] = (uint64_t*)p; p += cap * 8; }
    int32_t* vals0 = (int32_t*)p;
    for (int l = 0; l < levels; ++l) { a.vals[l] = (int32_t*)p; p += cap * 4; }
    for (int l = 0; l < levels; ++l) {
        a.first[l] = (int32_t*)p; p += nn * 4;
        prefix[l] = (int32_t*)p; p += nn * 4;
        a.keep[l] = (uint8_t*)p; p += nn;
        a.s[l] = stride << (l + 1);
    }
    int rc;
    hipError_t e = hipMemsetAsync(scratch, 0, zero_bytes, s);
    if (e != hipSuccess) { pcgc_set_error("pyramid: %s", hipGetErrorString(e)); return -1; }
    hipLaunchKernelGGL(k_hash_clear, dim3(grid_for((int64_t)cap * levels, 256)), dim3(256), 0, s, keys0, vals0, (int64_t)cap * levels);
    const dim3 g(grid_for(n, 256)), b(256);
    for (int l = 0; l < levels; ++l) {
        hipLaunchKernelGGL(k_pyr_insert_level, g, b, 0, s, (const int4*)fine, n, a, l);
        hipLaunchKernelGGL(k_pyr_first_level, g, b, 0, s, (const int4*)fine, n, a, l);
    }
    for (int l = 0; l < levels; ++l)
        if ((rc = pcgc_mask_scan_zeroed(a.keep[l], n, prefix[l], totals + l, scan_ws[l], pcgc_scan_workspace_bytes(n), stream))) return rc;
    static thread_local int32_t* host_total = nullptr;
    if (!host_total && hipHostMalloc((void**)&host_total, 64, hipHostMallocDefault) != hipSuccess) { host_total = nullptr; pcgc_set_error("pyramid: cannot allocate pinned memory"); return -1; }
    e = hipMemcpyAsync(host_total, totals, (size_t)levels * sizeof(int32_t), hipMemcpyDeviceToHost, s);
    if (e == hipSuccess) e = hipStreamSynchronize(s);
    if (e != hipSuccess) { pcgc_set_error("pyramid: %s", hipGetErrorString(e)); return -1; }
    PyrOut o; o.stride = stride;
    for (int l = 0; l < levels; ++l) {
        counts[l] = host_total[l];
        o.coarse[l] = (int4*)coarse[l]; o.parent_of[l] = parent_of[l]; o.down[l] = down[l]; o.prefix[l] = prefix[l]; o.count[l] = counts[l];
        if (counts[l] > 0 && (e = hipMemsetAsync(down[l], 0xFF, (size_t)counts[l] * 8 * sizeof(int32_t), s)) != hipSuccess) { pcgc_set_error("pyramid: %s", hipGetErrorString(e)); return -1; }
    }
    hipLaunchKernelGGL(k_pyr_finish, g, b, 0, s, (const int4*)fine, n, a, o);
    PCGC_CHECK_LAUNCH("pyramid");
    return 0;
}
extern "C" int pcgc_compact_index(const uint8_t* mask, const int32_t* prefix, int64_t n, int32_t* orig, void* stream) {
    if (n == 0) return 0;
    hipLaunchKernelGGL(k_compact_index, dim3(grid_for(n, 256)), dim3(256), 0, S(stream), mask, prefix, n, orig);
    PCGC_CHECK_LAUNCH("compact_index");
    return 0;
}

__global__ void __launch_bounds__(256) k_d1_nn(const int4* __restrict__ a, int64_t na, const uint64_t* __restrict__ keys,
                                               const int32_t* __restrict__ vals, uint64_t cap_mask,
                                               const int4* __restrict__ offsets, int n_off, double* __restrict__ sum,
                                               unsigned long long* __restrict__ max_d2, int32_t* __restrict__ unresolved) {
    int64_t i = (int64_t)blockIdx.x * blockDim.x + threadIdx.x;
    double mine = 0.0; unsigned long long mymax = 0; int miss = 0;
    if (i < na) {
        const int4 c = a[i];
        int found = -1;
        for (int t = 0; t < n_off; ++t) {
            const int4 o = offsets[t];
            if (hash_lookup(keys, vals, cap_mask, c.x, c.y + o.x, c.z + o.y, c.w + o.z) >= 0) { found = o.w; break; }
        }
        if (found >= 0) { mine = (double)found; mymax = (unsigned long long)found; } else miss = 1;
    }
#pragma unroll
    for (int d = 32; d > 0; d >>= 1) {
        mine += __shfl_xor(mine, d, 64);
        const unsigned long long om = __shfl_xor(mymax, d, 64); mymax = om > mymax ? om : mymax;
        miss += __shfl_xor(miss, d, 64);
    }
    if ((threadIdx.x & 63) == 0) {
        if (mine != 0.0) atomicAdd(sum, mine);
        if (mymax) atomicMax(max_d2, mymax);
        if (miss) atomicAdd(unresolved, miss);
    }
}
extern "C" int pcgc_d1_nn(const int32_t* a, int64_t na, const uint64_t* b_keys, const int32_t* b_vals, int64_t b_cap,
                          const int32_t* offsets, int n_offsets, double* sum, uint64_t* max_d2, int32_t* unresolved,
                          void* stream) {
    PCGC_REQUIRE(b_cap > 0 && (b_cap & (b_cap - 1)) == 0, "bad hash capacity");
    hipError_t e = hipMemsetAsync(sum, 0, 8, S(stream));
    if (e == hipSuccess) e = hipMemsetAsync(max_d2, 0, 8, S(stream));
    if (e == hipSuccess) e = hipMemsetAsync(unresolved, 0, 4, S(stream));
    if (e != hipSuccess) { pcgc_set_error("d1_nn: %s", hipGetErrorString(e)); return -1; }
    if (na == 0) return 0;
    hipLaunchKernelGGL(k_d1_nn, dim3(grid_for(na, 256)), dim3(256), 0, S(stream), (const int4*)a, na, b_keys, b_vals,
                       (uint64_t)(b_cap - 1), (const int4*)offsets, n_offsets, sum, (unsigned long long*)max_d2, unresolved);
    PCGC_CHECK_LAUNCH("d1_nn");
    return 0;
}

__global__ void k_d1_cell_masks(const int4* __restrict__ b, int64_t nb, const uint64_t* __restrict__ ckeys, const int32_t* __restrict__ cvals,
                                uint64_t cmask, unsigned long long* __restrict__ masks) {
    const int64_t i = (int64_t)blockIdx.x * blockDim.x + threadIdx.x;
    if (i >= nb) return;
    const int4 c = b[i];
    const int32_t row = hash_lookup(ckeys, cvals, cmask, c.x, c.y & ~3, c.z & ~3, c.w & ~3);
    if (row >= 0) atomicOr(&masks[row], 1ull << ((c.y & 3) | ((c.z & 3) << 2) | ((c.w & 3) << 4)));
}
__global__ void __launch_bounds__(256) k_d1_nn_cells(const int4* __restrict__ a, int64_t na, const uint64_t* __restrict__ ckeys,
                                                     const int32_t* __restrict__ cvals, uint64_t cmask,
                                                     const unsigned long long* __restrict__ masks, const int4* __restrict__ offsets, int n_off,
                                                     int32_t reach2, double* __restrict__ sum, unsigned long long* __restrict__ max_d2,
                                                     int32_t* __restrict__ unresolved) {
    const int64_t i = (int64_t)blockIdx.x * blockDim.x + threadIdx.x;
    double mine = 0.0; unsigned long long mymax = 0; int miss = 0;
    if (i < na) {
        const int4 c = a[i];
        const int lx = c.y & 3, ly = c.z & 3, lz = c.w & 3;
        const int X = c.y & ~3, Y = c.z & ~3, Z = c.w & ~3;
        int best = 0x7FFFFFFF;
        for (int t = 0; t < n_off; ++t) {
            const int4 o = offsets[t];
            if (o.w >= best) break;
            const int32_t row = hash_lookup(ckeys, cvals, cmask, c.x, X + 4 * o.x, Y + 4 * o.y, Z + 4 * o.z);
            if (row < 0) continue;
            unsigned long long m = masks[row];
            const int bx = 4 * o.x - lx, by = 4 * o.y - ly, bz = 4 * o.z - lz;
            while (m) {
                const int bit = __ffsll((long long)m) - 1;
                m &= m - 1;
                const int dx = bx + (bit & 3), dy = by + ((bit >> 2) & 3), dz = bz + (bit >> 4);
                const int d2 = dx * dx + dy * dy + dz * dz;
                best = d2 < best ? d2 : best;
            }
        }
        if (best < reach2) { mine = (double)best; mymax = (unsigned long long)best; } else miss = 1;
    }
#pragma unroll
    for (int d = 32; d > 0; d >>= 1) {
        mine += __shfl_xor(mine, d, 64);
        const unsigned long long om = __shfl_xor(mymax, d, 64); mymax = om > mymax ? om : mymax;
        miss += __shfl_xor(miss, d, 64);
    }
    if ((threadIdx.x & 63) == 0) {
        if (mine != 0.0) atomicAdd(sum, mine);
        if (mymax) atomicMax(max_d2, mymax);
        if (miss) atomicAdd(unresolved, miss);
    }
}
extern "C" int pcgc_d1_cell_masks(const int32_t* b, int64_t nb, const uint64_t* cell_keys, const int32_t* cell_vals, int64_t cell_cap,
                                  uint64_t* masks, int64_t n_cells, void* stream) {
    PCGC_REQUIRE(cell_cap > 0 && (cell_cap & (cell_cap - 1)) == 0, "bad hash capacity");
    hipError_t e = hipMemsetAsync(masks, 0, (size_t)n_cells * 8, S(stream));
    if (e != hipSuccess) { pcgc_set_error("d1_cell_masks: %s", hipGetErrorString(e)); return -1; }
    if (nb == 0) return 0;
    hipLaunchKernelGGL(k_d1_cell_masks, dim3(grid_for(nb, 256)), dim3(256), 0, S(stream), (const int4*)b, nb, cell_keys, cell_vals,
                       (uint64_t)(cell_cap - 1), (unsigned long long*)masks);
    PCGC_CHECK_LAUNCH("d1_cell_masks");
    return 0;
}
extern "C" int pcgc_d1_nn_cells(const int32_t* a, int64_t na, const uint64_t* cell_keys, const int32_t* cell_vals, int64_t cell_cap,
                                const uint64_t* masks, const int32_t* offsets, int n_offsets, int32_t reach2, double* sum, uint64_t* max_d2,
                                int32_t* unresolved, void* stream) {
    PCGC_REQUIRE(cell_cap > 0 && (cell_cap & (cell_cap - 1)) == 0, "bad hash capacity");
    hipError_t e = hipMemsetAsync(sum, 0, 8, S(stream));
    if (e == hipSuccess) e = hipMemsetAsync(max_d2, 0, 8, S(stream));
    if (e == hipSuccess) e = hipMemsetAsync(unresolved, 0, 4, S(stream));
    if (e != hipSuccess) { pcgc_set_error("d1_nn_cells: %s", hipGetErrorString(e)); return -1; }
    if (na == 0) return 0;
    hipLaunchKernelGGL(k_d1_nn_cells, dim3(grid_for(na, 256)), dim3(256), 0, S(stream), (const int4*)a, na, cell_keys, cell_vals,
                       (uint64_t)(cell_cap - 1), (const unsigned long long*)masks, (const int4*)offsets, n_offsets, reach2, sum,
                       (unsigned long long*)max_d2, unresolved);
    PCGC_CHECK_LAUNCH("d1_nn_cells");
    return 0;
}

extern "C" int pcgc_level_prepare_children(const int32_t* coords, int64_t n, int32_t stride, uint64_t* keys, int32_t* vals, int64_t cap, int32_t* nbr,
                                           int32_t* children, int32_t* nbr_children, void* stream) {
    PCGC_REQUIRE(coords && keys && vals && nbr && children && nbr_children, "null argument");
    if (int rc = pcgc_hash_clear(keys, vals, cap, stream)) return rc;
    if (int rc = pcgc_hash_insert(coords, n, stride, keys, vals, cap, stream)) return rc;
    if (int rc = pcgc_kmap_k3(coords, n, stride, keys, vals, cap, nbr, stream)) return rc;
    if (int rc = pcgc_coords_children(coords, n, stride, children, stream)) return rc;
    return pcgc_kmap_k3_children(nbr, n, nbr_children, stream);
}
```

### pcgcv2_amd/csrc/pcgc_common.h

```cpp
#pragma once
#include <hip/hip_runtime.h>
#include <stdint.h>
#include <stdio.h>
#include "../../include/pcgc_hip.h"

void pcgc_set_error(const char* fmt, ...);

#define PCGC_CHECK_LAUNCH(name)                                                            \
    do {                                                                                   \
        hipError_t e__ = hipGetLastError();                                                \
        if (e__ != hipSuccess) { pcgc_set_error("%s: %s", name, hipGetErrorString(e__)); return -1; } \
    } while (0)

#define PCGC_REQUIRE(cond, msg)                                                            \
    do { if (!(cond)) { pcgc_set_error("%s: %s", __func__, msg); return -2; } } while (0)

static inline hipStream_t S(void* s) { return (hipStream_t)s; }
static inline unsigned grid_for(int64_t n, int block) { return (unsigned)((n + block - 1) / block); }

__device__ static inline unsigned xcd_tile(unsigned b, unsigned nb) {
    const unsigned q = nb >> 3, r = nb & 7, x = b & 7;
    return (x < r ? x * (q + 1) : r * (q + 1) + (x - r) * q) + (b >> 3);
}

#define PCGC_EMPTY_KEY 0xFFFFFFFFFFFFFFFFull
__host__ __device__ static inline bool coord_in_range(int32_t b, int32_t x, int32_t y, int32_t z) {
    return ((uint32_t)x < (1u << 20)) && ((uint32_t)y < (1u << 20)) && ((uint32_t)z < (1u << 20)) && ((uint32_t)b < 16u) &&
           !(b == 15 && (x & y & z) == 0xFFFFF);
}
__host__ __device__ static inline uint64_t coord_key(int32_t b, int32_t x, int32_t y, int32_t z) {
    return ((uint64_t)b << 60) | ((uint64_t)z << 40) | ((uint64_t)y << 20) | (uint64_t)x;
}
__device__ static inline uint64_t mix64(uint64_t v) {
    v ^= v >> 33; v *= 0xff51afd7ed558ccdull; v ^= v >> 33; v *= 0xc4ceb9fe1a85ec53ull; v ^= v >> 33; return v;
}
__device__ static inline uint64_t hash_slot(uint64_t key, uint64_t cap_mask) { return mix64(key) & cap_mask; }
__device__ static inline int32_t hash_lookup(const uint64_t* __restrict__ keys, const int32_t* __restrict__ vals,
                                             uint64_t cap_mask, int32_t b, int32_t x, int32_t y, int32_t z) {
    if (!coord_in_range(b, x, y, z)) return -1;
    uint64_t key = coord_key(b, x, y, z);
    uint64_t h = hash_slot(key, cap_mask);
    for (;;) {
        uint64_t k = keys[h];
        if (k == key) return vals[h];
        if (k == PCGC_EMPTY_KEY) return -1;
        h = (h + 1) & cap_mask;
    }
}

__device__ static inline int32_t sel_rank(const uint64_t* __restrict__ bits, const int32_t* __restrict__ wprefix, int64_t m) {
    const uint64_t w = bits[m >> 6], bit = 1ull << (m & 63);
    return (w & bit) ? wprefix[m >> 6] + (int32_t)__popcll(w & (bit - 1)) : -1;
}

__device__ static inline void child_offset(int j, int k, int& kp, int& jn) {
    int tx = (j & 1) + (k % 3 - 1), ty = ((j >> 1) & 1) + ((k / 3) % 3 - 1), tz = (j >> 2) + (k / 9 - 1);
    int px = tx < 0 ? -1 : (tx > 1 ? 1 : 0), py = ty < 0 ? -1 : (ty > 1 ? 1 : 0), pz = tz < 0 ? -1 : (tz > 1 ? 1 : 0);
    kp = (px + 1) + 3 * (py + 1) + 9 * (pz + 1);
    jn = (tx & 1) | ((ty & 1) << 1) | ((tz & 1) << 2);
}
```

### pcgcv2_amd/csrc/select.hip

```cpp
#include <algorithm>
#include <cstring>
#include "pcgc_common.h"
#include <rocprim/rocprim.hpp>

constexpr int SCAN_TILE = 2048;

__device__ static inline int block_exclusive_scan_256(int v, int* total_out) {
    __shared__ int wave_sums[4];
    int lane = threadIdx.x & 63, w = threadIdx.x >> 6;
    int incl = v;
#pragma unroll
    for (int d = 1; d < 64; d <<= 1) { int t = __shfl_up(incl, d, 64); if (lane >= d) incl += t; }
    if (lane == 63) wave_sums[w] = incl;
    __syncthreads();
    int base = 0, tot = 0;
#pragma unroll
    for (int i = 0; i < 4; ++i) { int s = wave_sums[i]; if (i < w) base += s; tot += s; }
    __syncthreads();
    if (total_out) *total_out = tot;
    return base + incl - v;
}

__device__ static inline int load_mask8(const uint8_t* mask, int64_t n, int64_t base, uint8_t m[8]) {
    int cnt = 0;
    if (base + 8 <= n && ((uintptr_t)(mask + base) & 7) == 0) {
        uint64_t w = *(const uint64_t*)(mask + base);
#pragma unroll
        for (int j = 0; j < 8; ++j) { m[j] = ((w >> (8 * j)) & 0xff) ? 1 : 0; cnt += m[j]; }
    } else {
#pragma unroll
        for (int j = 0; j < 8; ++j) { m[j] = (base + j < n && mask[base + j]) ? 1 : 0; cnt += m[j]; }
    }
    return cnt;
}

constexpr uint64_t SCAN_AGG = 1ull << 62, SCAN_INCL = 2ull << 62;
__global__ void __launch_bounds__(256) k_scan_lookback(const uint8_t* __restrict__ mask, int64_t n, int64_t n_tiles,
                                                       unsigned long long* desc, int32_t* ticket, int32_t* __restrict__ prefix,
                                                       int32_t* total, const uint32_t* enable) {
    if (enable && *enable == 0) return;
    __shared__ int tile_s, excl_s;
    if (threadIdx.x == 0) tile_s = atomicAdd(ticket, 1);
    __syncthreads();
    const int64_t tile = tile_s;
    uint8_t m[8];
    const int64_t base = tile * SCAN_TILE + threadIdx.x * 8;
    const int cnt = load_mask8(mask, n, base, m);
    int tot;
    int ex = block_exclusive_scan_256(cnt, &tot);
    if (threadIdx.x < 64) {
        const int lane = threadIdx.x;
        int excl = 0;
        if (tile == 0) {
            if (lane == 0) __hip_atomic_store(&desc[0], SCAN_INCL | (uint64_t)(uint32_t)tot, __ATOMIC_RELAXED, __HIP_MEMORY_SCOPE_AGENT);
        } else {
            if (lane == 0) __hip_atomic_store(&desc[tile], SCAN_AGG | (uint64_t)(uint32_t)tot, __ATOMIC_RELAXED, __HIP_MEMORY_SCOPE_AGENT);
            for (int64_t j = tile - 1;; j -= 64) {
                const int64_t idx = j - lane;
                unsigned long long d = SCAN_INCL;
                if (idx >= 0) {
                    do { d = __hip_atomic_load(&desc[idx], __ATOMIC_RELAXED, __HIP_MEMORY_SCOPE_AGENT); } while ((d >> 62) == 0);
                }
                const unsigned long long incl = __ballot((d >> 62) == 2);
                const int first = incl ? (int)__ffsll((long long)incl) - 1 : 63;
                int v = lane <= first ? (int)(uint32_t)d : 0;
#pragma unroll
                for (int o = 32; o > 0; o >>= 1) v += __shfl_xor(v, o, 64);
                excl += v;
                if (incl) break;
            }
            if (lane == 0) __hip_atomic_store(&desc[tile], SCAN_INCL | (uint64_t)(uint32_t)(excl + tot), __ATOMIC_RELAXED, __HIP_MEMORY_SCOPE_AGENT);
        }
        if (lane == 0) { excl_s = excl; if (tile == n_tiles - 1) *total = excl + tot; }
    }
    __syncthreads();
    ex += excl_s;
#pragma unroll
    for (int j = 0; j < 8; ++j) { if (base + j < n) prefix[base + j] = ex; ex += m[j]; }
}

static int64_t scan_tiles(int64_t n) { return (n + SCAN_TILE - 1) / SCAN_TILE; }
extern "C" size_t pcgc_scan_workspace_bytes(int64_t n) { return (size_t)(scan_tiles(n) + 2) * sizeof(uint64_t); }

static void launch_scan(const uint8_t* mask, int64_t n, int32_t* prefix, int32_t* total, void* workspace, const uint32_t* enable, hipStream_t s) {
    const int64_t tiles = scan_tiles(n);
    unsigned long long* desc = (unsigned long long*)workspace;
    hipLaunchKernelGGL(k_scan_lookback, dim3((unsigned)tiles), dim3(256), 0, s, mask, n, tiles, desc, (int32_t*)(desc + tiles), prefix, total, enable);
}
extern "C" int pcgc_mask_scan_zeroed(const uint8_t* mask, int64_t n, int32_t* prefix, int32_t* total, void* workspace,
                                     size_t workspace_bytes, void* stream) {
    PCGC_REQUIRE(workspace_bytes >= pcgc_scan_workspace_bytes(n), "workspace too small");
    PCGC_REQUIRE(((uintptr_t)workspace & 7) == 0, "workspace must be 8-byte aligned");
    if (n == 0) return 0;
    launch_scan(mask, n, prefix, total, workspace, nullptr, S(stream));
    PCGC_CHECK_LAUNCH("mask_scan");
    return 0;
}
extern "C" int pcgc_mask_scan(const uint8_t* mask, int64_t n, int32_t* prefix, int32_t* total, void* workspace,
                              size_t workspace_bytes, void* stream) {
    PCGC_REQUIRE(workspace_bytes >= pcgc_scan_workspace_bytes(n), "workspace too small");
    PCGC_REQUIRE(((uintptr_t)workspace & 7) == 0, "workspace must be 8-byte aligned");
    if (n == 0) { (void)hipMemsetAsync(total, 0, 4, S(stream)); return 0; }
    (void)hipMemsetAsync(workspace, 0, pcgc_scan_workspace_bytes(n), S(stream));
    launch_scan(mask, n, prefix, total, workspace, nullptr, S(stream));
    PCGC_CHECK_LAUNCH("mask_scan");
    return 0;
}

__global__ void k_compact_coords(const int4* __restrict__ in, const uint8_t* __restrict__ mask,
                                 const int32_t* __restrict__ prefix, int64_t n, int4* __restrict__ out) {
    int64_t i = (int64_t)blockIdx.x * blockDim.x + threadIdx.x;
    if (i < n && mask[i]) out[prefix[i]] = in[i];
}
__global__ void k_compact_feats4(const float* __restrict__ in, int C4, int in_ld, const uint8_t* __restrict__ mask,
                                 const int32_t* __restrict__ prefix, int64_t n, float* __restrict__ out) {
    int64_t t = (int64_t)blockIdx.x * blockDim.x + threadIdx.x;
    int64_t i = t / C4; int c = (int)(t % C4);
    if (i < n && mask[i])
        *(float4*)(out + (int64_t)prefix[i] * (C4 * 4) + 4 * c) = *(const float4*)(in + i * in_ld + 4 * c);
}
__global__ void k_compact_feats1(const float* __restrict__ in, int C, int in_ld, const uint8_t* __restrict__ mask,
                                 const int32_t* __restrict__ prefix, int64_t n, float* __restrict__ out) {
    int64_t t = (int64_t)blockIdx.x * blockDim.x + threadIdx.x;
    int64_t i = t / C; int c = (int)(t % C);
    if (i < n && mask[i]) out[(int64_t)prefix[i] * C + c] = in[i * in_ld + c];
}
extern "C" int pcgc_compact_coords(const int32_t* coords, const uint8_t* mask, const int32_t* prefix, int64_t n,
                                   int32_t* out, void* stream) {
    if (n == 0) return 0;
    hipLaunchKernelGGL(k_compact_coords, dim3(grid_for(n, 256)), dim3(256), 0, S(stream), (const int4*)coords, mask, prefix,
                       n, (int4*)out);
    PCGC_CHECK_LAUNCH("compact_coords");
    return 0;
}
extern "C" int pcgc_compact_feats(const float* in, int C, int in_ld, const uint8_t* mask, const int32_t* prefix, int64_t n,
                                  float* out, void* stream) {
    if (n == 0) return 0;
    if (C % 4 == 0 && in_ld % 4 == 0 && (((uintptr_t)in | (uintptr_t)out) & 15) == 0)
        hipLaunchKernelGGL(k_compact_feats4, dim3(grid_for(n * (C / 4), 256)), dim3(256), 0, S(stream), in, C / 4, in_ld, mask,
                           prefix, n, out);
    else
        hipLaunchKernelGGL(k_compact_feats1, dim3(grid_for(n * C, 256)), dim3(256), 0, S(stream), in, C, in_ld, mask, prefix,
                           n, out);
    PCGC_CHECK_LAUNCH("compact_feats");
    return 0;
}

struct TopkState { uint32_t prefix; uint32_t tie; int64_t k_remaining; uint32_t done; uint32_t count_eq; };
constexpr int TOPK_MAX_SEGS = 16;
struct TopkSegs { int n; long long off[TOPK_MAX_SEGS + 1]; long long k[TOPK_MAX_SEGS]; };

__device__ static inline uint32_t order_key(float f) {
    f = f + 0.0f;
    uint32_t b = __float_as_uint(f);
    return (b & 0x80000000u) ? ~b : (b | 0x80000000u);
}
constexpr int TOPK_PASSES = 3, TOPK_BINS = 2048;
__host__ __device__ static inline int topk_shift(int pass) { return pass == 0 ? 21 : (pass == 1 ? 10 : 0); }
__host__ __device__ static inline int topk_bits(int pass) { return pass == 2 ? 10 : 11; }
__global__ void __launch_bounds__(256) k_topk_init(TopkState* st, uint32_t* hist, TopkSegs segs, unsigned long long* scan_ws, int64_t scan_words, uint32_t* any_tie) {
    const int y = blockIdx.x;
    if (threadIdx.x == 0) { st[y].prefix = 0; st[y].tie = 0; st[y].k_remaining = segs.k[y]; st[y].done = 0; st[y].count_eq = 0; }
    for (int b = threadIdx.x; b < TOPK_BINS; b += blockDim.x) hist[TOPK_BINS * y + b] = 0;
    if (y == 0) {
        if (threadIdx.x == 0) *any_tie = 0;
        for (int64_t i = threadIdx.x; i < scan_words; i += blockDim.x) scan_ws[i] = 0;
    }
}
__global__ void __launch_bounds__(256) k_topk_hist(const float* __restrict__ v_all, int ld, TopkSegs segs, TopkState* st_all,
                                                   int pass, uint32_t* hist_all, uint32_t* any_tie) {
    __shared__ uint32_t h[TOPK_BINS];
    __shared__ int64_t S[257];
    __shared__ bool last_s;
    __shared__ int pick_s;
    const int t = threadIdx.x, y = blockIdx.y;
    const float* __restrict__ v = v_all + segs.off[y] * ld;
    const int64_t n = segs.off[y + 1] - segs.off[y];
    TopkState* st = st_all + y;
    uint32_t* hist = hist_all + TOPK_BINS * y;
    const int shift = topk_shift(pass), nb = 1 << topk_bits(pass);
    const uint32_t dmask = (uint32_t)nb - 1u;
    for (int b = t; b < nb; b += 256) h[b] = 0;
    __syncthreads();
    const uint32_t prefix = st->prefix;
    const uint32_t pmask = pass == 0 ? 0u : (0xFFFFFFFFu << (shift + topk_bits(pass)));
    const int64_t step = (int64_t)gridDim.x * blockDim.x;
    int64_t i = (int64_t)blockIdx.x * blockDim.x + t;
    for (; i + 7 * step < n; i += 8 * step) {
        float f[8];
#pragma unroll
        for (int u = 0; u < 8; ++u) f[u] = v[(i + u * step) * ld];
#pragma unroll
        for (int u = 0; u < 8; ++u) {
            const uint32_t key = order_key(f[u]);
            if ((key & pmask) == prefix) atomicAdd(&h[(key >> shift) & dmask], 1u);
        }
    }
    for (; i < n; i += step) {
        uint32_t key = order_key(v[i * ld]);
        if ((key & pmask) == prefix) atomicAdd(&h[(key >> shift) & dmask], 1u);
    }
    __syncthreads();
    uint32_t seen = 0;
    for (int b = t; b < nb; b += 256) if (h[b]) seen += atomicAdd(&hist[b], h[b]);
    asm volatile("s_waitcnt vmcnt(0)" : "+v"(seen) :: "memory");
    __syncthreads();
    if (t == 0) last_s = atomicAdd(&st->done, 1u) == gridDim.x - 1;
    __syncthreads();
    if (!last_s) return;
    const int PER = nb >> 8;
    uint32_t mine[TOPK_BINS / 256];
    int64_t gsum = 0;
#pragma unroll
    for (int e = 0; e < TOPK_BINS / 256; ++e) {
        mine[e] = e < PER ? __hip_atomic_load(&hist[t * PER + e], __ATOMIC_RELAXED, __HIP_MEMORY_SCOPE_AGENT) : 0u;
        gsum += mine[e];
    }
    S[t] = gsum;
    if (t == 0) { S[256] = 0; pick_s = -1; }
    __syncthreads();
    for (int off = 1; off < 256; off <<= 1) {
        const int64_t add = t + off < 256 ? S[t + off] : 0;
        __syncthreads();
        S[t] += add;
        __syncthreads();
    }
    const int64_t need = st->k_remaining;
    __syncthreads();
    const bool group_hit = t == 0 ? (S[1] < need) : (S[t] >= need && (S[t + 1] < need || t == 255));
    if (group_hit) {
        int64_t above = S[t + 1];
        int d = t * PER;
        uint32_t cnt = mine[0];
        bool found = false;
#pragma unroll
        for (int e = TOPK_BINS / 256 - 1; e >= 0; --e) {
            if (e < PER && !found) {
                if (above + mine[e] >= need || (t == 0 && e == 0)) { d = t * PER + e; cnt = mine[e]; found = true; }
                else above += mine[e];
            }
        }
        const int64_t rem = need - above;
        st->prefix = prefix | ((uint32_t)d << shift);
        st->k_remaining = rem;
        st->done = 0;
        if (pass == TOPK_PASSES - 1) {
            st->count_eq = cnt;
            st->tie = rem < (int64_t)cnt ? 1u : 0u;
            if (rem < (int64_t)cnt) atomicOr(any_tie, 1u);
        }
    }
    for (int b = t; b < nb; b += 256) hist[b] = 0;
}
__global__ void k_topk_mask(const float* __restrict__ v, int ld, TopkSegs segs, const TopkState* st_all, uint8_t* mask, uint8_t* eq) {
    const int y = blockIdx.y;
    const int64_t i = (int64_t)blockIdx.x * blockDim.x + threadIdx.x, n = segs.off[y + 1] - segs.off[y];
    if (i >= n) return;
    const int64_t g = segs.off[y] + i;
    const TopkState* st = st_all + y;
    const uint32_t key = order_key(v[g * ld]), T = st->prefix;
    const bool tie = st->tie != 0;
    mask[g] = (key > T) || (key == T && !tie);
    eq[g] = tie && key == T;
}
__global__ void k_topk_tie_fix(const TopkState* st_all, TopkSegs segs, const uint8_t* __restrict__ eq, const int32_t* __restrict__ eq_rank,
                               int tie_high, uint8_t* mask) {
    const int y = blockIdx.y;
    const TopkState* st = st_all + y;
    if (st->tie == 0) return;
    const int64_t i = (int64_t)blockIdx.x * blockDim.x + threadIdx.x, n = segs.off[y + 1] - segs.off[y];
    if (i >= n) return;
    const int64_t g = segs.off[y] + i;
    if (!eq[g]) return;
    const int64_t need = st->k_remaining, r = (int64_t)eq_rank[g] - (int64_t)eq_rank[segs.off[y]];
    mask[g] = tie_high ? r >= (int64_t)st->count_eq - need : r < need;
}
static int g_topk_tie_high = 0;
extern "C" int pcgc_set_convention(int what, int value) {
    if (what == 0) { g_topk_tie_high = value ? 1 : 0; return 0; }
    pcgc_set_error("set_convention: unknown convention %d", what);
    return -2;
}
static size_t align256(size_t v) { return (v + 255) & ~(size_t)255; }
extern "C" size_t pcgc_topk_workspace_bytes(int64_t n) {
    return 1024 + (size_t)TOPK_MAX_SEGS * TOPK_BINS * 4 + align256((size_t)n) + align256((size_t)n * 4) + 256 + align256(pcgc_scan_workspace_bytes(n));
}
static int topk_segments(const float* logits, int ld, const TopkSegs& segs, uint8_t* mask, void* workspace, size_t workspace_bytes, void* stream) {
    const int64_t n = segs.off[segs.n];
    PCGC_REQUIRE(workspace_bytes >= pcgc_topk_workspace_bytes(n), "workspace too small");
    PCGC_REQUIRE(((uintptr_t)workspace & 7) == 0, "workspace must be 8-byte aligned");
    if (n == 0) return 0;
    char* ws = (char*)workspace;
    TopkState* st = (TopkState*)ws;
    uint32_t* any_tie = (uint32_t*)(ws + 768); ws += 1024;
    uint32_t* hist = (uint32_t*)ws; ws += (size_t)TOPK_MAX_SEGS * TOPK_BINS * 4;
    uint8_t* eq = (uint8_t*)ws; ws += align256((size_t)n);
    int32_t* rank = (int32_t*)ws; ws += align256((size_t)n * 4);
    int32_t* total = (int32_t*)ws; ws += 256;
    void* scan_ws = ws;
    int64_t nmax = 0;
    for (int b = 0; b < segs.n; ++b) nmax = std::max<int64_t>(nmax, segs.off[b + 1] - segs.off[b]);
    unsigned g = grid_for(nmax, 256 * 8); if (g > 256) g = 256; if (g < 1) g = 1;
    hipLaunchKernelGGL(k_topk_init, dim3(segs.n), dim3(256), 0, S(stream), st, hist, segs, (unsigned long long*)scan_ws,
                       (int64_t)(pcgc_scan_workspace_bytes(n) / 8), any_tie);
    for (int pass = 0; pass < TOPK_PASSES; ++pass)
        hipLaunchKernelGGL(k_topk_hist, dim3(g, segs.n), dim3(256), 0, S(stream), logits, ld, segs, st, pass, hist, any_tie);
    hipLaunchKernelGGL(k_topk_mask, dim3(grid_for(nmax, 256), segs.n), dim3(256), 0, S(stream), logits, ld, segs, st, mask, eq);
    launch_scan(eq, n, rank, total, scan_ws, any_tie, S(stream));
    hipLaunchKernelGGL(k_topk_tie_fix, dim3(grid_for(nmax, 256), segs.n), dim3(256), 0, S(stream), st, segs, eq, rank, g_topk_tie_high, mask);
    PCGC_CHECK_LAUNCH("topk_mask");
    return 0;
}
extern "C" int pcgc_topk_mask(const float* logits, int ld, int64_t n, int64_t k, uint8_t* mask, void* workspace,
                              size_t workspace_bytes, void* stream) {
    if (n == 0) return 0;
    if (k >= n) { (void)hipMemsetAsync(mask, 1, (size_t)n, S(stream)); return 0; }
    if (k <= 0) { (void)hipMemsetAsync(mask, 0, (size_t)n, S(stream)); return 0; }
    TopkSegs segs{};
    segs.n = 1; segs.off[0] = 0; segs.off[1] = n; segs.k[0] = k;
    return topk_segments(logits, ld, segs, mask, workspace, workspace_bytes, stream);
}

extern "C" int pcgc_topk_mask_segments(const float* logits, int ld, int nseg, const int64_t* seg_rows, const int64_t* seg_k,
                                       uint8_t* mask, void* workspace, size_t workspace_bytes, void* stream) {
    PCGC_REQUIRE(nseg >= 0 && nseg <= TOPK_MAX_SEGS && (nseg == 0 || (seg_rows && seg_k)), "at most 16 segments");
    if (nseg == 0) return 0;
    TopkSegs segs{};
    segs.n = nseg; segs.off[0] = 0;
    for (int b = 0; b < nseg; ++b) {
        PCGC_REQUIRE(seg_rows[b] >= 0, "negative segment");
        segs.off[b + 1] = segs.off[b] + seg_rows[b];
        segs.k[b] = seg_k[b] < 0 ? 0 : (seg_k[b] > seg_rows[b] ? seg_rows[b] : seg_k[b]);
    }
    return topk_segments(logits, ld, segs, mask, workspace, workspace_bytes, stream);
}

struct SelSeg { uint32_t T; int64_t need, thr, K0, G0, E0; };
__device__ static inline int4 child_coords(const int4* __restrict__ parent, int64_t g, int32_t h) {
    const int4 c = parent[g >> 3]; const int k = (int)(g & 7);
    return make_int4(c.x, c.y + (k & 1) * h, c.z + ((k >> 1) & 1) * h, c.w + (k >> 2) * h);
}
__global__ void __launch_bounds__(256) k_topk_select(const float* __restrict__ v, int ld, TopkSegs segs, const TopkState* __restrict__ st_all,
                                                     const int4* __restrict__ coords, const int4* __restrict__ parent, int32_t half,
                                                     int tie_high, int64_t n, int64_t n_tiles, unsigned long long* desc, int32_t* ticket,
                                                     uint8_t* __restrict__ bits, int32_t* __restrict__ wprefix,
                                                     int32_t* __restrict__ orig, int4* __restrict__ out_coords) {
    __shared__ SelSeg seg[TOPK_MAX_SEGS];
    __shared__ int tile_s, exg_s, exe_s;
    const int t = threadIdx.x;
    if (t == 0) {
        tile_s = atomicAdd(ticket, 1);
        int64_t K0 = 0, G0 = 0, E0 = 0;
        for (int b = 0; b < segs.n; ++b) {
            const TopkState s = st_all[b];
            const int64_t need = s.k_remaining < (int64_t)s.count_eq ? s.k_remaining : (int64_t)s.count_eq;
            seg[b].T = s.prefix; seg[b].need = need; seg[b].thr = (int64_t)s.count_eq - need;
            seg[b].K0 = K0; seg[b].G0 = G0; seg[b].E0 = E0;
            K0 += segs.k[b]; G0 += segs.k[b] - need; E0 += s.count_eq;
        }
    }
    __syncthreads();
    const int64_t tile = tile_s;
    const int64_t base = tile * SCAN_TILE + t * 8;
    uint32_t key[8];
    if (ld == 1 && base + 8 <= n && ((uintptr_t)(v + base) & 15) == 0) {
        const float4 a = *(const float4*)(v + base), b4 = *(const float4*)(v + base + 4);
        key[0] = order_key(a.x); key[1] = order_key(a.y); key[2] = order_key(a.z); key[3] = order_key(a.w);
        key[4] = order_key(b4.x); key[5] = order_key(b4.y); key[6] = order_key(b4.z); key[7] = order_key(b4.w);
    } else {
#pragma unroll
        for (int j = 0; j < 8; ++j) key[j] = base + j < n ? order_key(v[(base + j) * ld]) : 0u;
    }
    int b0 = 0;
    while (b0 + 1 < segs.n && base >= segs.off[b0 + 1]) ++b0;
    uint32_t gt = 0, eq = 0;
    {
        int b = b0;
#pragma unroll
        for (int j = 0; j < 8; ++j) {
            const int64_t g = base + j;
            while (b + 1 < segs.n && g >= segs.off[b + 1]) ++b;
            if (g < n) {
                const uint32_t T = seg[b].T;
                gt |= (uint32_t)(key[j] > T) << j;
                eq |= (uint32_t)(key[j] == T) << j;
            }
        }
    }
    int tot;
    const int packed = __popc(gt) | (__popc(eq) << 16);
    const int ex = block_exclusive_scan_256(packed, &tot);
    if (t < 64) {
        const int lane = t;
        int exg = 0, exe = 0;
        const unsigned long long own = ((unsigned long long)(uint32_t)(tot & 0xFFFF) << 31) | (unsigned long long)(uint32_t)(tot >> 16);
        if (tile == 0) {
            if (lane == 0) __hip_atomic_store(&desc[0], SCAN_INCL | own, __ATOMIC_RELAXED, __HIP_MEMORY_SCOPE_AGENT);
        } else {
// ... 192 lines not shown
```

### pcgcv2_amd/ops.py

```python
import os as _os

import numpy as np
import torch

from ._lib import lib, check, PcgcError


def _stream(t=None):
    if t is None:
        return torch.cuda.current_stream().cuda_stream
    return torch.cuda.current_stream(t.device).cuda_stream


def _p(t):
    return None if t is None else t.data_ptr()


def _dev(t, dtype, what):
    if not t.is_cuda:
        raise PcgcError(f'{what}: expected a ROCm device tensor, got {t.device} (no CPU fallback exists)')
    if t.dtype != dtype:
        raise PcgcError(f'{what}: expected {dtype}, got {t.dtype}')
    if not t.is_contiguous():
        raise PcgcError(f'{what}: tensor must be contiguous')
# ... 4 lines not shown
    return _dev(t, torch.int32, what)


def _f32(t, what='feats'):
    if t.dtype != torch.float32 or not t.is_cuda:
        raise PcgcError(f'{what}: expected float32 device tensor, got {t.dtype} on {t.device}')
    return t


def _ld(t):
    if t.dim() != 2 or t.stride(1) != 1:
        raise PcgcError('feature views must be 2-D with unit column stride')
    return t.stride(0)


MFMA_F32_PEAK_TFLOPS = 157.3
_CHILD_WEIGHT = None


def child_pairs(parent_nbr):
    global _CHILD_WEIGHT
    if _CHILD_WEIGHT is None or _CHILD_WEIGHT.device != parent_nbr.device:
        w = np.zeros(27, np.int64)
        for kp, jc, reach in _halo_cells():
            w[kp] += len(reach)
        _CHILD_WEIGHT = torch.from_numpy(w).to(parent_nbr.device)
    return int(((parent_nbr >= 0).sum(1) * _CHILD_WEIGHT).sum().item())


class _Profile:

    TIE = 0.05

    def __init__(self):
        self.reset(False)

    def reset(self, enabled=False, only=None):
        self.enabled = enabled
        self.only = None if only is None else frozenset(only)
        self.counting = False
        self.records = {}
        self.pairs = {}

    def want(self, key):
        return self.enabled and (self.only is None or key in self.only)

    @staticmethod
    def name_of(kernel):
        return kernel.split(' (')[0]

    def bracket(self, key, kernel, n, gathered, flops, compulsory=None, mfma_issued=None, pairs=None):
        e0, e1 = torch.cuda.Event(enable_timing=True), torch.cuda.Event(enable_timing=True)
        r = self.records.setdefault(key, {'kernel': kernel, 'n': n, 'gathered': gathered, 'flops': flops, 'compulsory': compulsory,
                                          'mfma_issued': mfma_issued, 'pairs': pairs, 'events': []})
        r['events'].append((e0, e1))
        return e0, e1

    def count(self, nbr):
        n = nbr.shape[1]
        if n not in self.pairs:
            self.pairs[n] = int((nbr >= 0).sum().item())

    def count_children(self, parent_nbr):
        n = 8 * parent_nbr.shape[1]
        if n not in self.pairs:
            self.pairs[n] = child_pairs(parent_nbr)

    def detail(self):
        out = []
        for key, r in self.records.items():
            ts = sorted(e0.elapsed_time(e1) for e0, e1 in r['events'])
            ms = sum(ts)
            us = ms / len(ts) * 1e3
            med = (ts[len(ts) // 2] if len(ts) % 2 else 0.5 * (ts[len(ts) // 2 - 1] + ts[len(ts) // 2])) * 1e3
            d = {'key': key, 'name': self.name_of(r['kernel']), 'kernel': r['kernel'], 'n_out': r['n'], 'launches': len(ts), 'ms': ms, 'avg_us': us, 'median_us': med}
            P = r['pairs'] if r['pairs'] is not None else self.pairs.get(r['n'])
            if P is not None:
                d['pairs'] = P
                d['gathered_bytes'] = r['gathered'](P)
                d['flops'] = r['flops'](P)
                d['gathered_GBps'] = d['gathered_bytes'] / (us * 1e-6) / 1e9
                d['TFLOPs'] = d['flops'] / (us * 1e-6) / 1e12
                if r['compulsory'] is not None:
                    d['compulsory_bytes'] = r['compulsory']
                    d['compulsory_GBps'] = r['compulsory'] / (us * 1e-6) / 1e9
                if r['mfma_issued'] is not None:
                    issued = r['mfma_issued'](P) if callable(r['mfma_issued']) else r['mfma_issued']
                    d['mfma_issued_flops'] = issued
                    d['mfma_issued_TFLOPs'] = issued / (us * 1e-6) / 1e12
            out.append(d)
        return sorted(out, key=lambda d: -d['ms'])

    def families(self, steps, peak_gbs):
        groups = {}
        for d in self.detail():
            if 'pairs' in d:
                groups.setdefault(d['name'], []).append(d)
        fam = []
        for name, ds in groups.items():
            ms = sum(d['ms'] for d in ds)
            med_ms = sum(d['median_us'] * d['launches'] for d in ds) * 1e-3
            fl = sum(d['flops'] * d['launches'] for d in ds)
            comp = sum(d.get('compulsory_bytes', 0) * d['launches'] for d in ds)
            issued = sum(d.get('mfma_issued_flops', 0) * d['launches'] for d in ds)
            f = {'kernel': name, 'levels': sorted({d['n_out'] for d in ds}), 'launches_per_step': round(sum(d['launches'] for d in ds) / steps, 2),
                 'us_per_step': round(ms * 1e3 / steps, 1), 'median_us_per_step': round(med_ms * 1e3 / steps, 1),
                 'TFLOPs': round(fl / (ms * 1e-3) / 1e12, 2), 'frac': round(fl / (ms * 1e-3) / 1e12 / MFMA_F32_PEAK_TFLOPS, 4),
                 'issued_over_algorithmic': round(issued / fl, 2) if issued and fl else None,
                 'compulsory_frac_of_hbm': round(comp / (ms * 1e-3) / 1e9 / peak_gbs, 4)}
            fam.append(f)
        return sorted(fam, key=lambda f: f['kernel'])

    def dominant(self, steps, peak_gbs):
        fam = self.families(steps, peak_gbs)
        if not fam:
            return None, ()
        top = max(f['median_us_per_step'] for f in fam)
        tied = [f for f in fam if f['median_us_per_step'] >= (1.0 - self.TIE) * top]
        best = min(tied, key=lambda f: (f['frac'], f['kernel']))
        keys = tuple(k for k, r in self.records.items() if self.name_of(r['kernel']) == best['kernel'])
        return best['kernel'], keys

    def summary(self, peak_gbs, steps, name=None):
        d_all = [r for r in self.detail() if 'pairs' in r]
        if not d_all:
            return None
        if name is None:
            name, _ = self.dominant(steps, peak_gbs)
        d = [r for r in d_all if r['name'] == name]
        if not d:
            return None
        t_s = sum(r['ms'] for r in d) * 1e-3
        launches = sum(r['launches'] for r in d)
        fl = sum(r['flops'] * r['launches'] for r in d)
        comp = sum(r.get('compulsory_bytes', 0) * r['launches'] for r in d)
        gath = sum(r['gathered_bytes'] * r['launches'] for r in d)
        issued = sum(r.get('mfma_issued_flops', 0) * r['launches'] for r in d)
        tf, cg = fl / t_s / 1e12, comp / t_s / 1e9
        hbm_frac, mfma_frac = cg / peak_gbs, tf / MFMA_F32_PEAK_TFLOPS
        is_mfma = issued > 0 and max(mfma_frac, issued / t_s / 1e12 / MFMA_F32_PEAK_TFLOPS) >= hbm_frac
        roof = {'bound': 'mfma' if is_mfma else 'hbm'}
        if is_mfma:
            roof.update(achieved=round(tf, 2), peak=MFMA_F32_PEAK_TFLOPS, unit='TFLOP/s', frac=round(mfma_frac, 4))
        else:
            roof.update(achieved=round(cg, 2), peak=peak_gbs, unit='GB/s', frac=round(hbm_frac, 4))
        roof.update(traffic=None, kernel=name, description=d[0]['kernel'], avg_launch_us=round(t_s * 1e6 / launches, 2), launches_timed=launches,
                    launches_per_step=round(launches / steps, 2),
                    selection=f'kernel NAME with the largest per-step time (median launch time x launches, levels pooled); names within {int(self.TIE * 100)} % '
                              'are tied and the lowest fraction of peak wins',
                    levels=[{'n_out': r['n_out'], 'pairs': r['pairs'], 'launches': r['launches'], 'avg_launch_us': round(r['avg_us'], 2),
                             'flops_per_launch': r['flops'], 'frac_of_fp32_mfma_peak': round(r['TFLOPs'] / MFMA_F32_PEAK_TFLOPS, 4),
                             'compulsory_bytes_per_launch': r.get('compulsory_bytes'),
                             'mfma_issued_flops_per_launch': r.get('mfma_issued_flops')} for r in sorted(d, key=lambda r: -r['n_out'])],
                    algorithmic={'flops_per_launch': fl / launches, 'TFLOPs': round(tf, 2), 'frac_of_fp32_mfma_peak': round(mfma_frac, 4),
                                 'compulsory_bytes_per_launch': comp / launches, 'compulsory_GBps': round(cg, 1), 'frac_of_hbm_peak': round(hbm_frac, 4),
                                 'gathered_bytes_per_launch': gath / launches, 'gathered_GBps': round(gath / t_s / 1e9, 1),
                                 'note': 'per-launch figures are means over the launches of this kernel name (levels pooled: see `levels`); gathered = SURVEY 8d '
                                         'formula, every (in,out) pair charged — the row re-use is served by L2/LDS, not HBM'})
        if issued:
            roof['mfma_issued'] = {'flops_per_launch': issued / launches, 'TFLOPs': round(issued / t_s / 1e12, 2),
                                   'pipe_utilisation': round(issued / t_s / 1e12 / MFMA_F32_PEAK_TFLOPS, 4), 'issued_over_algorithmic': round(issued / fl, 2),
                                   'note': 'fp32 MFMA flops issued (zero-padded columns and absent rows included) / time'}
        roof['all_launches'] = self.aggregate(peak_gbs, steps)
        return roof

    def aggregate(self, peak_gbs, steps):
        d = [r for r in self.detail() if 'pairs' in r]
        tot_g = sum(r['gathered_bytes'] * r['launches'] for r in d)
        tot_c = sum(r.get('compulsory_bytes', 0) * r['launches'] for r in d)
        tot_f = sum(r['flops'] * r['launches'] for r in d)
        tot_ms = sum(r['ms'] for r in d)
        return {'ms_per_step': round(tot_ms / steps, 3), 'launches_per_step': round(sum(r['launches'] for r in d) / steps, 2),
                'GFLOP_per_step': round(tot_f / steps / 1e9, 2),
                'TFLOPs': round(tot_f / (tot_ms * 1e-3) / 1e12, 2), 'frac_of_fp32_mfma_peak': round(tot_f / (tot_ms * 1e-3) / 1e12 / MFMA_F32_PEAK_TFLOPS, 4),
                'compulsory_GBps': round(tot_c / (tot_ms * 1e-3) / 1e9, 1), 'frac_of_hbm_peak': round(tot_c / (tot_ms * 1e-3) / 1e9 / peak_gbs, 4),
                'gathered_GBps': round(tot_g / (tot_ms * 1e-3) / 1e9, 1)}


PROFILE = _Profile()


from .pathconfig import PathConfig, FIELDS as _PATH_FIELDS

PATH = PathConfig.from_env()


def configure(cfg=None, **changes):
    global PATH
    prev = PATH
    PATH = (PATH if cfg is None else cfg).replace(**changes)
    return prev


class path:

    def __init__(self, **changes):
        self.changes = changes

    def __enter__(self):
        self.prev = configure(**self.changes)
        return PATH

    def __exit__(self, *exc):
        configure(self.prev)
        return False


class _OpsModule(type(_os)):

    def __getattr__(self, name):
        if name in _PATH_FIELDS:
            return getattr(self.__dict__['PATH'], name)
        raise AttributeError(f"module 'pcgcv2_amd.ops' has no attribute '{name}'")

    def __setattr__(self, name, value):
        if name in _PATH_FIELDS:
            self.__dict__['PATH'] = self.__dict__['PATH'].replace(**{name: value})
        else:
            super().__setattr__(name, value)


import sys as _sys
_sys.modules[__name__].__class__ = _OpsModule


class HashTable:

    def __init__(self, coords, stride, keep_last=False):
        n = coords.shape[0]
        self.cap = int(lib().pcgc_hash_capacity(n))
        self.stride = int(stride)
        self.keys = torch.empty(self.cap, dtype=torch.int64, device=coords.device)
        self.vals = torch.empty(self.cap, dtype=torch.int32, device=coords.device)
        check(lib().pcgc_hash_clear(_p(self.keys), _p(self.vals), self.cap, _stream(self.keys)), 'hash_clear')
        check(lib().pcgc_hash_insert_policy(_p(_i32(coords)), n, self.stride, _p(self.keys), _p(self.vals), self.cap, int(keep_last),
                                            _stream(coords)), 'hash_insert')


def level_prepare_children(coords, stride):
    n, dev = coords.shape[0], coords.device
    table = HashTable.__new__(HashTable)
    table.cap, table.stride = int(lib().pcgc_hash_capacity(n)), int(stride)
    table.keys = torch.empty(table.cap, dtype=torch.int64, device=dev)
    table.vals = torch.empty(table.cap, dtype=torch.int32, device=dev)
    ints = torch.empty(27 * n + 32 * n + 27 * 8 * n, dtype=torch.int32, device=dev)
    nbr, children, nbr_c = ints[:27 * n].view(27, n), ints[27 * n:59 * n].view(8 * n, 4), ints[59 * n:].view(27, 8 * n)
    check(lib().pcgc_level_prepare_children(_p(_i32(coords)), n, int(stride), _p(table.keys), _p(table.vals), table.cap, _p(nbr), _p(children),
                                            _p(nbr_c), _stream(coords)), 'level_prepare_children')
    return table, nbr, children, nbr_c


def check_coords(coords, what='coordinates'):
    out2 = torch.empty(2, dtype=torch.int32, device=coords.device)
    check(lib().pcgc_coords_check_order(_p(_i32(coords)), coords.shape[0], _p(out2), _stream(coords)), 'coords_check_order')
    n_bad, descents = out2.tolist()
    if n_bad:
        raise PcgcError(f'{what}: {n_bad} of {coords.shape[0]} rows are outside the supported range '
                        '(0 <= x, y, z < 2^20, 0 <= batch < 16)')
    return int(descents)


def first_occurrence_mask(coords, table, want_rows=False):
    n = coords.shape[0]
    keep = torch.empty(n, dtype=torch.uint8, device=coords.device)
    first = torch.empty(n, dtype=torch.int32, device=coords.device) if want_rows else None
    check(lib().pcgc_hash_first_mask(_p(_i32(coords)), n, table.stride, _p(table.keys), _p(table.vals), table.cap, _p(keep),
                                     _p(first), _stream(coords)), 'hash_first_mask')
    return (keep, first) if want_rows else keep


def down_maps(fine, first_row, prefix, stride_fine, n_coarse):
    n = fine.shape[0]
    parent_of = torch.empty(n, dtype=torch.int32, device=fine.device)
    down = torch.empty((8, n_coarse), dtype=torch.int32, device=fine.device)
    check(lib().pcgc_down_maps(_p(_i32(fine)), _p(first_row), _p(prefix), n, int(stride_fine), n_coarse, _p(parent_of), _p(down),
                               _stream(fine)), 'down_maps')
    return parent_of, down


def down_level(fine, stride_fine):
    import ctypes
    fine = _i32(fine)
    n, dev = fine.shape[0], fine.device
    cap = int(lib().pcgc_hash_capacity(n))
    ws_bytes = int(lib().pcgc_scan_workspace_bytes(n))
    a8 = lambda v: (v + 7) & ~7
    off, sizes = 0, []
    for nbytes in (16 * n, 8 * cap, 4 * cap, 4 * n, 4 * n, 8, n, ws_bytes):
        sizes.append((off, nbytes)); off += a8(nbytes)
    scratch = torch.empty(off, dtype=torch.uint8, device=dev)
    part = lambda i, dt: scratch[sizes[i][0]:sizes[i][0] + sizes[i][1]].view(dt)
    q, keys, vals, first_row, prefix, total, keep, ws = (part(0, torch.int32), part(1, torch.int64), part(2, torch.int32), part(3, torch.int32),
                                                       part(4, torch.int32), part(5, torch.int32), part(6, torch.uint8), part(7, torch.uint8))
    outbuf = torch.empty(13 * n, dtype=torch.int32, device=dev)
    coarse_ub, parent_of, down_ub = outbuf[:4 * n].view(n, 4), outbuf[4 * n:5 * n], outbuf[5 * n:]
    n_coarse = ctypes.c_int64(0)
    check(lib().pcgc_down_level(_p(fine), n, int(stride_fine), _p(q), _p(keys), _p(vals), cap, _p(keep), _p(first_row), _p(prefix),
                                _p(total), _p(ws), ws_bytes, _p(coarse_ub), _p(parent_of), _p(down_ub), ctypes.byref(n_coarse),
                                _stream(fine)), 'down_level')
    nc = int(n_coarse.value)
    return coarse_ub[:nc], parent_of, down_ub[:8 * nc].view(8, nc)


def pyramid(fine, stride_fine, levels):
    import ctypes
    fine = _i32(fine)
    n, dev = fine.shape[0], fine.device
    nbytes = int(lib().pcgc_pyramid_scratch_bytes(n, levels))
    scratch = torch.empty(nbytes, dtype=torch.uint8, device=dev)
    outbuf = torch.empty(levels * 13 * n, dtype=torch.int32, device=dev)
    parts = [(outbuf[13 * n * l:13 * n * l + 4 * n].view(n, 4), outbuf[13 * n * l + 4 * n:13 * n * l + 5 * n], outbuf[13 * n * l + 5 * n:13 * n * (l + 1)])
             for l in range(levels)]
    ptrs = lambda k: (ctypes.c_void_p * levels)(*[p[k].data_ptr() for p in parts])
    counts = (ctypes.c_int64 * levels)()
    check(lib().pcgc_pyramid(_p(fine), n, int(stride_fine), int(levels), _p(scratch), nbytes, ptrs(0), ptrs(1), ptrs(2), counts, _stream(fine)),
          'pyramid')
    out, below = [], n
    for l, (coarse_ub, parent_ub, down_ub) in enumerate(parts):
        nc = int(counts[l])
        out.append((coarse_ub[:nc], parent_ub[:below], down_ub[:8 * nc].view(8, nc)))
        below = nc
    return out


def compact_index(mask, prefix, n_out):
    orig = torch.empty(n_out, dtype=torch.int32, device=mask.device)
    check(lib().pcgc_compact_index(_p(mask), _p(prefix), mask.shape[0], _p(orig), _stream(mask)), 'compact_index')
    return orig


def kmap_k3_children(parent_nbr):
    n_parent = parent_nbr.shape[1]
    nbr = torch.empty((27, 8 * n_parent), dtype=torch.int32, device=parent_nbr.device)
    check(lib().pcgc_kmap_k3_children(_p(parent_nbr), n_parent, _p(nbr), _stream(parent_nbr)), 'kmap_k3_children')
    return nbr


def kmap_k3_prune(cand_nbr, mask, prefix, orig):
    n_out = orig.shape[0]
    nbr = torch.empty((27, n_out), dtype=torch.int32, device=cand_nbr.device)
    check(lib().pcgc_kmap_k3_prune(_p(cand_nbr), cand_nbr.shape[1], _p(mask), _p(prefix), _p(orig), n_out, _p(nbr), _stream(cand_nbr)),
          'kmap_k3_prune')
    return nbr


def kmap_k3_prune_parent(parent_nbr, mask, prefix, orig):
    n_out = orig.shape[0]
    nbr = torch.empty((27, n_out), dtype=torch.int32, device=parent_nbr.device)
    check(lib().pcgc_kmap_k3_prune_parent(_p(parent_nbr), parent_nbr.shape[1], _p(mask), _p(prefix), _p(orig), n_out, _p(nbr),
                                          _stream(parent_nbr)), 'kmap_k3_prune_parent')
    return nbr


def kmap_k3_from_coarse(fine, stride_fine, parent_of, coarse_nbr, down):
    n = fine.shape[0]
    nbr = torch.empty((27, n), dtype=torch.int32, device=fine.device)
    check(lib().pcgc_kmap_k3_from_coarse(_p(_i32(fine)), n, int(stride_fine), _p(parent_of), _p(coarse_nbr), _p(down),
                                         coarse_nbr.shape[1], _p(nbr), _stream(fine)), 'kmap_k3_from_coarse')
    return nbr


def mask_scan(mask):
    n = mask.shape[0]
    prefix = torch.empty(n, dtype=torch.int32, device=mask.device)
    total = torch.empty(1, dtype=torch.int32, device=mask.device)
    ws_bytes = int(lib().pcgc_scan_workspace_bytes(n))
    ws = torch.empty(ws_bytes, dtype=torch.uint8, device=mask.device)
    check(lib().pcgc_mask_scan(_p(_dev(mask, torch.uint8, 'mask')), n, _p(prefix), _p(total), _p(ws), ws_bytes, _stream(mask)),
          'mask_scan')
    return prefix, total


def compact_coords(coords, mask, prefix, n_out):
    out = torch.empty((n_out, 4), dtype=torch.int32, device=coords.device)
    check(lib().pcgc_compact_coords(_p(_i32(coords)), _p(mask), _p(prefix), coords.shape[0], _p(out), _stream(coords)),
          'compact_coords')
    return out


def compact_feats(feats, mask, prefix, n_out):
    _f32(feats)
    C = feats.shape[1]
    out = torch.empty((n_out, C), dtype=torch.float32, device=feats.device)
    check(lib().pcgc_compact_feats(_p(feats), C, _ld(feats), _p(mask), _p(prefix), feats.shape[0], _p(out), _stream(feats)),
          'compact_feats')
    return out


def coords_quantize(coords, stride_out):
    out = torch.empty_like(coords)
    check(lib().pcgc_coords_quantize(_p(_i32(coords)), coords.shape[0], int(stride_out), _p(out), _stream(coords)), 'coords_quantize')
    return out


def coords_children(coords, stride_in):
    out = torch.empty((8 * coords.shape[0], 4), dtype=torch.int32, device=coords.device)
    check(lib().pcgc_coords_children(_p(_i32(coords)), coords.shape[0], int(stride_in), _p(out), _stream(coords)), 'coords_children')
    return out


def coords_scale(coords, factor):
    out = torch.empty_like(coords)
    check(lib().pcgc_coords_scale(_p(_i32(coords)), coords.shape[0], float(np.float32(factor)), _p(out), _stream(coords)),
          'coords_scale')
    return out


def kmap_k3(coords, stride, table):
    n = coords.shape[0]
    nbr = torch.empty((27, n), dtype=torch.int32, device=coords.device)
    check(lib().pcgc_kmap_k3(_p(_i32(coords)), n, int(stride), _p(table.keys), _p(table.vals), table.cap, _p(nbr), _stream(coords)),
          'kmap_k3')
    return nbr


def set_conv_impl(impl):
    check(lib().pcgc_set_conv_impl(int(impl)), 'set_conv_impl')


def conv_gather(nbr, x, W, bias, out=None, residual=None, relu=False, n_out=None):
    _f32(x, 'x'); _f32(W, 'W')
    if W.dim() == 2:
        K, (Cin, Cout) = 1, W.shape
    else:
        K, Cin, Cout = W.shape
    if x.shape[1] != Cin:
        raise PcgcError(f'conv_gather: input has {x.shape[1]} channels, kernel expects {Cin}')
    if nbr is None:
        n_out = x.shape[0]
    else:
        n_out = nbr.shape[1]
        if nbr.shape[0] != K:
            raise PcgcError('conv_gather: kernel map / kernel volume mismatch')
    if out is None:
        out = torch.empty((n_out, Cout), dtype=torch.float32, device=x.device)
    res_p, res_ld = (None, 0) if residual is None else (_p(_f32(residual)), _ld(residual))
    prof = K == 27 and PROFILE.want(('conv', Cin, Cout, n_out))
    if prof:
        mfma = Cin in (16, 32, 64) and Cout in (16, 32, 64) and n_out >= 8192
        e0, e1 = PROFILE.bracket(('conv', Cin, Cout, n_out), f'k3 gather conv Cin={Cin} Cout={Cout} (k_conv_gather_mfma*/dma, per-row gather)', n_out,
                                 lambda P, a=Cin, b=Cout, n=n_out: P * a * 4 + P * 8 + n * b * 4,
                                 lambda P, a=Cin, b=Cout: 2 * P * a * b,
                                 compulsory=x.shape[0] * Cin * 4 + 27 * n_out * 4 + n_out * Cout * 4,
                                 mfma_issued=(2 * 27 * ((n_out + 15) // 16 * 16) * Cin * Cout) if mfma else None)
        e0.record()
    check(lib().pcgc_conv_gather(_p(nbr), K, n_out, _p(x), x.shape[0], Cin, _ld(x), 0, _p(W), _p(bias), res_p, res_ld, 0, int(relu),
                                 _p(out), Cout, _ld(out), 0, _stream(nbr)), 'conv_gather')
    if prof:
        e1.record()
    elif PROFILE.counting and K == 27:
        PROFILE.count(nbr)
    return out




def conv_gather_unit(nbr, W, bias, relu=False):
    _f32(W, 'W')
    K, Cin, Cout = W.shape
    if Cin != 1 or nbr.shape[0] != K:
        raise PcgcError('conv_gather_unit: kernel [K, 1, Cout] and a [K, n] map expected')
    n_out = nbr.shape[1]
    out = torch.empty((n_out, Cout), dtype=torch.float32, device=W.device)
    key = ('conv', 1, Cout, n_out)
    prof = K == 27 and PROFILE.want(key)
    if prof:
        e0, e1 = PROFILE.bracket(key, f'k3 conv 1->{Cout} on the unit input (k_conv_unit: kernel map only, no feature gather)', n_out,
                                 lambda P, b=Cout, n=n_out: P * 4 + P * 8 + n * b * 4, lambda P, b=Cout: 2 * P * b,
                                 compulsory=27 * n_out * 4 + n_out * Cout * 4)
        e0.record()
    check(lib().pcgc_conv_gather_unit(_p(nbr), K, n_out, _p(W), _p(bias), int(relu), _p(out), Cout, Cout, _stream(nbr)), 'conv_gather_unit')
    if prof:
        e1.record()
    elif PROFILE.counting and K == 27:
        PROFILE.count(nbr)
    return out


def conv_unit_from_coarse(fine, stride_fine, parent_of, coarse_nbr, down, W, bias, relu=False):
    _f32(W, 'W')
    K, Cin, Cout = W.shape
    if Cin != 1 or K != 27:
        raise PcgcError('conv_unit_from_coarse: kernel [27, 1, Cout] expected')
    n = fine.shape[0]
    out = torch.empty((n, Cout), dtype=torch.float32, device=W.device)
    key = ('conv', 1, Cout, n)
    prof = PROFILE.want(key)
    if prof:
        e0, e1 = PROFILE.bracket(key, f'k3 conv 1->{Cout} on the unit input (k_conv_unit_coarse: presence from the parent level\'s map, no map of its own)', n,
                                 lambda P, b=Cout, n=n: P * 4 + P * 8 + n * b * 4, lambda P, b=Cout: 2 * P * b,
                                 compulsory=n * 16 + n * 4 + n * Cout * 4)
        e0.record()
    check(lib().pcgc_conv_unit_from_coarse(_p(_i32(fine)), n, int(stride_fine), _p(parent_of), _p(coarse_nbr), _p(down), coarse_nbr.shape[1],
                                           _p(W), _p(bias), int(relu), _p(out), Cout, Cout, _stream(fine)), 'conv_unit_from_coarse')
    if prof:
        e1.record()
    return out


def set_up2_impl(mfma):
    check(lib().pcgc_set_up2_impl(int(mfma)), 'set_up2_impl')




def _irn_pass_formulas(n, C, map_bytes, names):
    Q = C // 4
    return ((1, names[0], lambda P: (P * C * 4 + P * 8 + n * Q * 4) + n * (C + Q) * 4, lambda P: 2 * P * C * Q + 2 * n * C * Q,
             n * C * 4 + map_bytes + n * 2 * Q * 4),
            (2, names[1], lambda P: (P * Q * 4 + P * 8 + n * 2 * Q * 4) + (P * Q * 4 + P * 8 + n * Q * 4) + n * 3 * Q * 4,
             lambda P: 2 * P * Q * 2 * Q + 2 * P * Q * Q + 2 * n * Q * 2 * Q,
             n * 2 * Q * 4 + map_bytes + n * C * 4 + n * C * 4))


def irn_block(nbr, x, params):
    import ctypes
    _f32(x, 'x')
    n, C = x.shape
    t = torch.empty((n, C // 2), dtype=torch.float32, device=x.device)
    out = torch.empty((n, C), dtype=torch.float32, device=x.device)
    arr = (ctypes.c_void_p * 10)(*[p.data_ptr() for p in params])
    if PROFILE.counting:
        PROFILE.count(nbr)
    name_a, name_b = (f'k_irn_a<{C}, 16>', f'k_irn_b<{C}, 16>') if C == 64 else (f'k_irn_a_split<{C}>', f'k_irn_b_split<{C}>')
    if not (PROFILE.want((name_a, n)) or PROFILE.want((name_b, n))):
        check(lib().pcgc_irn_block(_p(nbr), n, _p(x), C, _ld(x), arr, _p(t), _p(out), C, _stream(nbr)), 'irn_block')
        return out
    Q = C // 4
    passes = _irn_pass_formulas(n, C, 27 * n * 4, (name_a, name_b))
    for ps, name, bf, ff, comp in passes:
        prof = PROFILE.want((name, n))
        if prof:
            e0, e1 = PROFILE.bracket((name, n), name + ' (per-row gather, VALU)', n, bf, ff, compulsory=comp)
            e0.record()
        check(lib().pcgc_irn_pass(_p(nbr), n, _p(x), C, _ld(x), arr, _p(t), _p(out), C, ps, _stream(nbr)), 'irn_pass')
        if prof:
            e1.record()
    return out




def irn_block_rows64(nbr, x, params, tables):
    _f32(x, 'x')
    n = x.shape[0]
    ta, tb = tables
    t = torch.empty((n, 32), dtype=torch.float32, device=x.device)
    out = torch.empty((n, 64), dtype=torch.float32, device=x.device)
    P = [p.data_ptr() for p in params]
    s = _stream(x)
    if PROFILE.counting:
        PROFILE.count(nbr)
    tiles = (n + 15) // 16
    forms = _irn_pass_formulas(n, 64, 27 * n * 4, ('k_rows_irn_a64', 'k_rows_irn_b64'))
    per_tile = (27 * 16 + 16, 27 * 12 + 8)
    calls = (lambda: lib().pcgc_irn_rows_pass(_p(nbr), n, 64, 1, _p(x), _ld(x), _p(ta), ta.numel() * 4, P[1], P[5], None, None, 0, _p(t), 32, s),
             lambda: lib().pcgc_irn_rows_pass(_p(nbr), n, 64, 2, _p(t), 32, _p(tb), tb.numel() * 4, P[3], P[7], P[9], _p(x), _ld(x), _p(out), 64, s))
    for (ps, name, bf, ff, comp), call, mf in zip(forms, calls, per_tile):
        prof = PROFILE.want((name, n))
        if prof:
            e0, e1 = PROFILE.bracket((name, n), name + ' (fused InceptionResNet pass on a plain level, LDS-resident table + per-wave row ring, fp32 MFMA)', n, bf, ff,
                                     compulsory=comp, mfma_issued=tiles * mf * 2048)
            e0.record()
        check(call(), 'irn_rows_pass')
        if prof:
            e1.record()
    return out


def _rows_irn32_index():
    C, Q = 32, 8
    shapes = [(27, C, Q), (27, Q, 2 * Q), (C, Q), (27, Q, Q), (Q, 2 * Q)]
    off, Ws = 0, []
    for shp in shapes:
        n = int(np.prod(shp))
        Ws.append(np.arange(off, off + n, dtype=np.int64).reshape(shp))
        off += n
    W00, W01, W10, W11, W12 = Ws
    fa = [_fragment([W00[k][:, co] for co in range(Q)] + [(W10[:, co] if k == 13 else None) for co in range(Q)], 2) for k in range(27)]
    pad = lambda w: np.concatenate([np.full(Q, -1, np.int64), w])
    fb = [_fragment([W01[k][:, co] for co in range(16)], 1, KS=2, k0=0) for k in range(27)]
    fb += [_fragment([pad(W11[k][:, co]) for co in range(Q)] + [None] * Q, 1, KS=2, k0=2) for k in range(27)]
    fb.append(_fragment([W12[:, co] for co in range(16)], 1, KS=2, k0=0))
    return np.concatenate([f.reshape(-1) for f in fa]), np.concatenate([f.reshape(-1) for f in fb])


def rows_irn32_tables(params):
    W00, b00, W01, b01, W10, b10, W11, b11, W12, b12 = params
    ia, ib = _table_index(('rows_irn32', W00.device), _rows_irn32_index)
    flat = torch.cat([w.detach().reshape(-1) for w in (W00, W01, W10, W11, W12)])
    return _gather_table(ia, flat), _gather_table(ib, flat)




def irn_block_rows32(nbr, x, params, tables):
    _f32(x, 'x')
    n = x.shape[0]
    ta, tb = tables
    t = torch.empty((n, 16), dtype=torch.float32, device=x.device)
    out = torch.empty((n, 32), dtype=torch.float32, device=x.device)
    P = [p.data_ptr() for p in params]
    s = _stream(x)
    if PROFILE.counting:
        PROFILE.count(nbr)
    tiles = (n + 15) // 16
    forms = _irn_pass_formulas(n, 32, 27 * n * 4, ('k_rows_irn_a32', 'k_rows_irn_b32'))
    per_tile = (27 * 8, 27 * 4 + 2)
    calls = (lambda: lib().pcgc_irn_rows_pass(_p(nbr), n, 32, 1, _p(x), _ld(x), _p(ta), ta.numel() * 4, P[1], P[5], None, None, 0, _p(t), 16, s),
             lambda: lib().pcgc_irn_rows_pass(_p(nbr), n, 32, 2, _p(t), 16, _p(tb), tb.numel() * 4, P[3], P[7], P[9], _p(x), _ld(x), _p(out), 32, s))
    for (ps, name, bf, ff, comp), call, mf in zip(forms, calls, per_tile):
        prof = PROFILE.want((name, n))
        if prof:
            e0, e1 = PROFILE.bracket((name, n), name + ' (fused InceptionResNet pass on a plain level, LDS-resident table + per-wave row ring, packed-N fp32 MFMA)', n, bf, ff,
                                     compulsory=comp, mfma_issued=tiles * mf * 2048)
            e0.record()
        check(call(), 'irn_rows_pass')
        if prof:
            e1.record()
    return out


def rows32_pass(nbr, x, params, tables, ps, t=None):
    n = x.shape[0]
    ta, tb = tables
    P = [p.data_ptr() for p in params]
    s = _stream(x)
    if ps == 1:
        t = torch.empty((n, 16), dtype=torch.float32, device=x.device)
        check(lib().pcgc_irn_rows_pass(_p(nbr), n, 32, 1, _p(x), _ld(x), _p(ta), ta.numel() * 4, P[1], P[5], None, None, 0, _p(t), 16, s), 'irn_rows_pass')
        return t
    out = torch.empty((n, 32), dtype=torch.float32, device=x.device)
    check(lib().pcgc_irn_rows_pass(_p(nbr), n, 32, 2, _p(t), 16, _p(tb), tb.numel() * 4, P[3], P[7], P[9], _p(x), _ld(x), _p(out), 32, s), 'irn_rows_pass')
    return out


def rows_q4_tables(params):
    W00, b00, W01, b01, W10, b10, W11, b11, W12, b12 = params
    C = W00.shape[1]
    if C != 32:
        raise PcgcError('rows_q4_tables: C = 32')
    a0 = W00.detach().reshape(27, 2, 16, 2, 4).permute(0, 1, 3, 4, 2).reshape(-1)
    a1 = W10.detach().reshape(2, 16, 2, 4).permute(0, 2, 3, 1).reshape(-1)
    x01 = W01.detach().reshape(27, 8, 2, 2, 4).permute(0, 2, 4, 3, 1).reshape(27, 2, 64)
    y11 = W11.detach().reshape(27, 8, 2, 4).permute(0, 3, 2, 1).reshape(27, 1, 64)
    w12 = W12.detach().reshape(8, 2, 2, 4).permute(1, 3, 2, 0).reshape(-1)
    return torch.cat([a0, a1]).contiguous(), torch.cat([torch.cat([x01, y11], 1).reshape(-1), w12]).contiguous()




def rows_q4_pass(nbr, x, params, tables, ps, t=None):
    n = x.shape[0]
    ta, tb = tables
    P = [p.data_ptr() for p in params]
    s = _stream(x)
    if ps == 1:
        t = torch.empty((n, 16), dtype=torch.float32, device=x.device)
        check(lib().pcgc_irn_rows_q4_pass(_p(nbr), n, 32, 1, _p(x), _ld(x), _p(ta), ta.numel() * 4, P[1], P[5], None, None, 0, _p(t), 16, s), 'irn_rows_q4_pass')
        return t
    out = torch.empty((n, 32), dtype=torch.float32, device=x.device)
    check(lib().pcgc_irn_rows_q4_pass(_p(nbr), n, 32, 2, _p(t), 16, _p(tb), tb.numel() * 4, P[3], P[7], P[9], _p(x), _ld(x), _p(out), 32, s), 'irn_rows_q4_pass')
    return out


def irn_block_rows32_q4(nbr, x, params, tables):
    _f32(x, 'x')
    n = x.shape[0]
    ta, tb = tables
    t = torch.empty((n, 16), dtype=torch.float32, device=x.device)
    out = torch.empty((n, 32), dtype=torch.float32, device=x.device)
    P = [p.data_ptr() for p in params]
    s = _stream(x)
    if PROFILE.counting:
        PROFILE.count(nbr)
    tiles = (n + 63) // 64
    forms = _irn_pass_formulas(n, 32, 27 * n * 4, ('k_rows_q4_a32', 'k_rows_q4_b32'))
    per_tile = (112 * 16, 81 * 16 + 32)
    calls = (lambda: lib().pcgc_irn_rows_q4_pass(_p(nbr), n, 32, 1, _p(x), _ld(x), _p(ta), ta.numel() * 4, P[1], P[5], None, None, 0, _p(t), 16, s),
             lambda: lib().pcgc_irn_rows_q4_pass(_p(nbr), n, 32, 2, _p(t), 16, _p(tb), tb.numel() * 4, P[3], P[7], P[9], _p(x), _ld(x), _p(out), 32, s))
    for (ps, name, bf, ff, comp), call, mf in zip(forms, calls, per_tile):
        prof = PROFILE.want((name, n))
        if prof:
            e0, e1 = PROFILE.bracket((name, n), name + ' (fused InceptionResNet pass on a plain level, quad-block 4x4x1 fp32 MFMA, lane = row)', n, bf, ff,
                                     compulsory=comp, mfma_issued=tiles * mf * 512)
            e0.record()
        check(call(), 'irn_rows_q4_pass')
        if prof:
            e1.record()
    return out


def set_rows_q4_variant(v):
    check(lib().pcgc_set_rows_q4_variant(int(v)), 'set_rows_q4_variant')




def _halo_cells():
    P1 = (0, 1, 1, 2)
    B = (1, 0, 1, 0)
    cells = []
    for cz in range(4):
        for cy in range(4):
            for cx in range(4):
                kp = P1[cz] * 9 + P1[cy] * 3 + P1[cx]
                jc = B[cx] + 2 * B[cy] + 4 * B[cz]
                reach = []
                for j in range(8):
                    kx, ky, kz = cx - (j & 1), cy - ((j >> 1) & 1), cz - (j >> 2)
                    if 0 <= kx <= 2 and 0 <= ky <= 2 and 0 <= kz <= 2:
                        reach.append((j, kz * 9 + ky * 3 + kx))
                cells.append((kp, jc, reach))
    assert sum(len(r) for _, _, r in cells) == 216
    return cells


def child_conv_table(W):
    K, Cin, Cout = W.shape
    NB, NT = Cin // 16, Cout // 16
    return W.detach().reshape(K, NB, 4, 4, NT, 16).permute(0, 4, 1, 3, 5, 2).contiguous().reshape(-1)


def _fragment(col_weights, NB, KS=4, k0=0, half=False):
    ncol = 8 if half else 16
    out = np.full((NB, 4, ncol, KS), -1, np.int64)
    for mi, w in enumerate(col_weights):
        if w is None:
            continue
        for cb in range(NB):
            for jj in range(KS):
                for mq in range(4):
                    ch = 16 * cb + 4 * (k0 + jj) + mq
                    if ch < len(w):
                        out[cb, mq, mi, jj] = w[ch]
    return out.reshape(NB, -1)


_TABLE_INDEX = {}


def _table_index(key, make):
    hit = _TABLE_INDEX.get(key)
    if hit is None:
        made = make()
        dev = key[-1]
        up = lambda a: None if a is None else torch.from_numpy(a).to(dev)
        hit = tuple(up(a) for a in made) if isinstance(made, tuple) else up(made)
        if torch.device(dev).type == 'cuda':
            torch.cuda.current_stream(dev).synchronize()
        _TABLE_INDEX[key] = hit
    return hit


def _gather_table(index, flat):
    return torch.where(index >= 0, flat[index.clamp(min=0)], torch.zeros((), dtype=flat.dtype, device=flat.device)).contiguous()


def _cls_index(C):
    nb = C // 16
    rowf = nb * 16 + 4
    idx = np.full(((125 * rowf * 4 + 1023) // 1024 * 256,), -1, np.int64)
    for kz in range(3):
        for ky in range(3):
            for kx in range(3):
                r = 25 * (kz + 1) + 5 * (ky + 1) + (kx + 1)
                k = 9 * kz + 3 * ky + kx
                for cb in range(nb):
                    for mq in range(4):
                        for jj in range(4):
                            idx[r * rowf + cb * 16 + mq * 4 + jj] = k * C + 16 * cb + 4 * jj + mq
    return idx


def child_cls_table(W):
    C = W.shape[1]
    return _gather_table(_table_index(('cls', C, W.device), lambda: _cls_index(C)), W.detach().reshape(-1))


def _q4_cls_index(C):
    W = np.arange(27 * C, dtype=np.int64).reshape(27, C)
    frags = []
    for c, (kp, jc, reach) in enumerate(_halo_cells()):
        cz = c >> 4
        kof = dict(reach)
        for h in range(2):
            if not 0 <= cz - h <= 2:
                continue
            f = np.full((4, C), -1, np.int64)
            for sidx in range(4):
                if 4 * h + sidx in kof:
                    f[sidx] = W[kof[4 * h + sidx]]
            frags.append(f.reshape(-1))
    assert len(frags) == 96
    return np.concatenate(frags)


# ... 1348 lines not shown
```

### pcgcv2_amd/pathconfig.py

```python
import dataclasses
import os


def _env(name, default='1'):
    return os.environ.get(name, default) != '0'


@dataclasses.dataclass(frozen=True)
class PathConfig:
    UNIT_INPUT_CONV: bool = True
    UNIT_CONV_MAPLESS: bool = True
    FUSE_IRN: bool = True
    ROWS_IRN64: bool = True
    ROWS_IRN64_MIN: int = 1024
    ROWS_IRN32: bool = True
    ROWS_IRN32_MIN: int = 1024
    ROWS_IRN32_MAX: int = 0xF0000000 // (32 * 4) - 1
    ROWS_Q4: bool = True
    ROWS_Q4_MIN: int = 150_000
    CHILD_MFMA: bool = True
    CHILD_Q4: bool = True
    CHILD_Q4_MIN_PARENTS: int = 200_000
    ROWS_CONV: bool = True
    ROWS_CONV_MIN: int = 1024
    PACKED_CONV64: bool = True
    PACKED_CONV64_MIN: int = 512
    ROWS_DOWN: bool = True
    ROWS_DOWN_MIN: int = 1024
    ONE_SWEEP_PRUNE: bool = True
    D1_CELLS: bool = True

    @classmethod
    def from_env(cls):
        off = {f.name: False for f in dataclasses.fields(cls) if f.type in (bool, 'bool') and not _env('PCGC_' + f.name)}
        return cls(**off)

    def replace(self, **changes):
        unknown = set(changes) - FIELDS
        if unknown:
            raise AttributeError(f'PathConfig has no field(s) {sorted(unknown)}')
        return dataclasses.replace(self, **changes)

    def switches(self):
        return {f.name: getattr(self, f.name) for f in dataclasses.fields(self) if isinstance(getattr(self, f.name), bool)}


FIELDS = frozenset(f.name for f in dataclasses.fields(PathConfig))
```

### pcgcv2_amd/sparse.py

```python
import torch

from . import ops
from ._lib import PcgcError


def require_gpu(device):
    device = torch.device(device)
    if device.type != 'cuda':
        raise PcgcError(f'pcgcv2_amd runs on an MI355X (torch device "cuda" on ROCm); got "{device}". '
                        'There is no CPU execution path.')
    return device


HASH_LEVEL_MAX = 1 << 15


class CoordMap:

    def __init__(self, coords, stride, unique=False, origin=None, lazy=None):
        self._C = coords
        self._n, self.device = (int(lazy[0]), lazy[1]) if coords is None else (coords.shape[0], coords.device)
        self.stride = int(stride)
        self.origin = origin
        self._table = None
        self._k3 = None
        self._down = None
        self._parent_of = None
        self._unique = unique
        self._prepared_up = None
        self._batch_rows = None
        self.descents = None

    def __len__(self):
        return self._n

    @property
    def C(self):
        if self._C is None:
            parent = self.origin[1]
            self._C = ops.coords_children(parent.C, parent.stride)
        return self._C

    @property
    def batch_rows(self):
        if self._batch_rows is None:
            self._batch_rows = ops.batch_counts(self.C) if len(self) else [0]
        return self._batch_rows

    @property
    def table(self):
        if self._table is None:
            self._table = ops.HashTable(self.C, self.stride)
        return self._table

    @property
    def k3(self):
        if self._k3 is None:
            kind = self.origin[0] if self.origin else None
            if len(self) == 0:
                self._k3 = torch.empty((27, 0), dtype=torch.int32, device=self.device)
            elif kind == 'children':
                self._k3 = ops.kmap_k3_children(self.origin[1].k3)
            elif kind == 'pruned':
                _, cand, mask, prefix = self.origin
                orig = ops.compact_index(mask, prefix, len(self))
                if cand._k3 is None and cand.origin is not None and cand.origin[0] == 'children':
                    self._k3 = ops.kmap_k3_prune_parent(cand.origin[1].k3, mask, prefix, orig)
                else:
                    self._k3 = ops.kmap_k3_prune(cand.k3, mask, prefix, orig)
            elif kind == 'selected':
                _, cand, bits, wprefix, orig = self.origin
                if cand._k3 is None and cand.origin is not None and cand.origin[0] == 'children':
                    self._k3 = ops.kmap_k3_prune_parent_sel(cand.origin[1].k3, bits, wprefix, orig)
                else:
                    self._k3 = ops.kmap_k3_prune_sel(cand.k3, bits, wprefix, orig)
            elif len(self) > HASH_LEVEL_MAX and self.stride <= (1 << 18):
                coarse, down = self.down()
                self._k3 = ops.kmap_k3_from_coarse(self.C, self.stride, self._parent_of, coarse.k3, down)
            else:
                self._k3 = ops.kmap_k3(self.C, self.stride, self.table)
        return self._k3

    def mapless_unit_conv(self):
        return (ops.PATH.UNIT_CONV_MAPLESS and self._k3 is None and self.origin is None and len(self) > HASH_LEVEL_MAX and self.stride <= (1 << 18))

    def down(self):
        if self._down is None:
            coarse_C, self._parent_of, down = ops.down_level(self.C, self.stride)
            self._down = (CoordMap(coarse_C, 2 * self.stride, unique=True), down)
        return self._down

    def build_pyramid(self, levels):
        chain, lvl = [], self
        while lvl._down is not None and len(chain) < levels:
            lvl = lvl._down[0]; chain.append(lvl)
        todo = levels - len(chain)
        if todo > 0:
            for coarse_C, parent_of, down in ops.pyramid(lvl.C, lvl.stride, todo):
                lvl._parent_of = parent_of
                nxt = CoordMap(coarse_C, 2 * lvl.stride, unique=True)
                lvl._down = (nxt, down)
                lvl = nxt
        return lvl

    def up(self):
        if self._prepared_up is not None:
            child, self._prepared_up = self._prepared_up, None
            return child
        child = CoordMap(None, self.stride // 2, unique=True, origin=('children', self), lazy=(8 * len(self), self.device))
        if self._batch_rows is not None:
            child._batch_rows = [8 * r for r in self._batch_rows]
        return child

    def prepare_up(self):
        if (self.origin is None and self._table is None and self._k3 is None and self._prepared_up is None and 0 < len(self) <= HASH_LEVEL_MAX
                and self.stride >= 2 and self._batch_rows is None):
            self._table, self._k3, kids, kids_k3 = ops.level_prepare_children(self.C, self.stride)
            child = CoordMap(kids, self.stride // 2, unique=True, origin=('children', self))
            child._k3 = kids_k3
            self._prepared_up = child
            return
        child = self.up()
        child.k3
        self._prepared_up = child

    def drop_caches(self):
        self._table = self._k3 = self._down = self._parent_of = self._prepared_up = None
        self.__dict__.pop('_ingested', None)


def dedup(coords, feats, stride):
    from . import conventions
    table = ops.HashTable(coords, stride, keep_last=conventions.get('dedup_keep') == 'last')
    keep = ops.first_occurrence_mask(coords, table)
    prefix, total = ops.mask_scan(keep)
    n = int(total.item())
    if n == coords.shape[0]:
        return coords, feats
    return ops.compact_coords(coords, keep, prefix, n), ops.compact_feats(feats.contiguous(), keep, prefix, n)


class SparseTensor:

    def __init__(self, features, coordinates=None, tensor_stride=1, device=None, coordinate_map=None, assume_unique=False):
        if isinstance(tensor_stride, (list, tuple)):
            tensor_stride = tensor_stride[0]
        self._F_thunk = None
        self._F_rows = None
        self.unit_features = False
        if coordinate_map is not None:
            self.cmap = coordinate_map
            dev = coordinate_map.device
            if callable(features):
                self._F, self._F_thunk = None, features
                return
            self.F = features if features.device == dev else features.to(dev)
            if self.F.shape[0] != len(coordinate_map):
                raise PcgcError('coordinates / features length mismatch')
        else:
            dev = require_gpu(device if device is not None else coordinates.device)
            coords = coordinates.to(device=dev, dtype=torch.int32).contiguous()
            feats = features.to(device=dev, dtype=torch.float32).contiguous()
            if coords.dim() != 2 or coords.shape[1] != 4:
                raise PcgcError('coordinates must be [N,4] (batch, x, y, z)')
            if coords.shape[0] != feats.shape[0]:
                raise PcgcError('coordinates / features length mismatch')
            descents = ops.check_coords(coords) if coords.shape[0] > 0 else 0
            if not assume_unique and coords.shape[0] > 0:
                coords, feats = dedup(coords, feats, int(tensor_stride))
            self.cmap = CoordMap(coords, int(tensor_stride), unique=True)
            self.cmap.descents = descents
            self.F = feats
            if feats.shape[1] == 1 and feats.shape[0] > 0 and bool((feats == 1).all().item()):
                self.unit_features = True
                self._unit_stamp = (feats.data_ptr(), feats._version)

    @property
    def F(self):
        if self._F is None and self._F_thunk is not None:
            self._F, self._F_thunk, self._F_rows = self._F_thunk(), None, None
        return self._F

    def pending_rows(self):
        return self._F_rows if self._F is None else None

    @F.setter
    def F(self, value):
        self._F, self._F_thunk, self._F_rows = value, None, None
        self.unit_features = False

    def has_unit_features(self):
        f = self._F
        return bool(self.unit_features and f is not None and getattr(self, '_unit_stamp', None) == (f.data_ptr(), f._version))

    @property
    def C(self):
        return self.cmap.C

    @property
    def tensor_stride(self):
        return [self.cmap.stride] * 3

    @property
    def device(self):
        return self.cmap.device

    @property
    def shape(self):
        return self.F.shape

    def __len__(self):
        return len(self.cmap)

    def __repr__(self):
        return f'SparseTensor(N={len(self)}, C={self.F.shape[1]}, stride={self.cmap.stride}, device={self.device})'


def sparse_collate(coords_list, feats_list):
    cs, fs = [], []
    for b, (c, f) in enumerate(zip(coords_list, feats_list)):
        c = torch.as_tensor(c).int()
        cs.append(torch.cat([torch.full((len(c), 1), b, dtype=torch.int32, device=c.device), c], dim=1))
        fs.append(torch.as_tensor(f))
    return torch.cat(cs, 0), torch.cat(fs, 0)
```

Before: 146.1.

## Fuse unit-input conv0 and down0 into one kernel; merge pyramid build launches

Adds a fused kernel that computes the first 1->16 k3 convolution on unit features together with the stride-2 16->32 downsampling convolution using fp32 MFMA. It derives child presence from per-coarse occupancy bytes, so the 16-channel full-resolution intermediate is never materialised. The pyramid build is also restructured: the insert and first-occurrence kernels are fused per level, the per-level scans are batched into one call, and the per-level memsets are replaced by a single fill kernel. These changes cut launches and memory traffic, at the cost of more specialised code paths and a new occupancy buffer.

Result: no change. 146.0, median of 5 (-0.1%).

```diff
diff --git a/include/pcgc_hip.h b/include/pcgc_hip.h
--- a/include/pcgc_hip.h
+++ b/include/pcgc_hip.h
@@ -56,13 +56,15 @@
 int pcgc_down_finish(const int32_t* fine, const int32_t* q, const uint8_t* keep, const int32_t* first_row, const int32_t* prefix,
                      int64_t n, int32_t stride_fine, int64_t n_coarse, int32_t* coarse ,
                      int32_t* parent_of , int32_t* down , void* stream);
+int pcgc_down_occupancy(const int32_t* down , int64_t n_coarse, uint8_t* occ , void* stream);
 int pcgc_down_level(const int32_t* fine , int64_t n, int32_t stride_fine, int32_t* q, uint64_t* keys, int32_t* vals,
                     int64_t cap, uint8_t* keep, int32_t* first_row, int32_t* prefix, int32_t* total, void* scan_ws,
                     size_t scan_ws_bytes, int32_t* coarse , int32_t* parent_of ,
                     int32_t* down , int64_t* n_coarse_out , void* stream);
 size_t pcgc_pyramid_scratch_bytes(int64_t n, int levels);
 int pcgc_pyramid(const int32_t* fine , int64_t n, int32_t stride, int levels, void* scratch, size_t scratch_bytes,
-                 int32_t* const* coarse, int32_t* const* parent_of, int32_t* const* down, int64_t* counts , void* stream);
+                 int32_t* const* coarse, int32_t* const* parent_of, int32_t* const* down, int64_t* counts ,
+                 uint8_t* occ0 , void* stream);
 int pcgc_compact_index(const uint8_t* mask, const int32_t* prefix, int64_t n, int32_t* orig , void* stream);
 
 int pcgc_conv_gather(const int32_t* nbr, int K, int64_t n_out, const float* in, int64_t n_in , int Cin,
@@ -74,6 +76,8 @@
 int pcgc_conv_unit_from_coarse(const int32_t* fine , int64_t n_fine, int32_t stride_fine, const int32_t* parent_of,
                                const int32_t* coarse_nbr , const int32_t* down , int64_t n_coarse,
                                const float* W , const float* bias, int relu, float* out, int Cout, int out_ld, void* stream);
+int pcgc_conv_unit_down(const int32_t* coarse_nbr , const uint8_t* occ , int64_t n_coarse, const float* W0,
+                        const float* b0, const float* table, int64_t table_bytes, const float* b1, float* out, int out_ld, void* stream);
 int pcgc_set_conv_impl(int impl);
 int pcgc_set_up2_impl(int mfma);
 int pcgc_irn_block(const int32_t* nbr , int64_t n, const float* x , int C, int x_ld,
diff --git a/pcgcv2_amd/_build.py b/pcgcv2_amd/_build.py
--- a/pcgcv2_amd/_build.py
+++ b/pcgcv2_amd/_build.py
@@ -9,7 +9,7 @@
 OBJ = os.path.join(CSRC, '_obj' + ('_' + VARIANT if VARIANT else ''))
 LIB = os.path.join(HERE, 'libpcgc_hip' + ('_' + VARIANT if VARIANT else '') + '.so')
 SOURCES = ['coords.hip', 'select.hip', 'conv.hip', 'child_conv.hip', 'child_conv32.hip', 'child_cls_w.hip', 'child_irn.hip', 'child_irn_a16.hip', 'child_irn_b16.hip',
-           'child_irn_a32.hip', 'child_irn_b32.hip', 'child_q4.hip', 'rows_irn.hip', 'rows_q4.hip', 'conv_packed.hip', 'entropy.hip', 'loss.hip', 'occupancy.hip', 'occupancy_rans.hip', 'grad.hip', 'metric.hip', 'colour.hip', 'normals.hip', 'mesh.hip', 'collate.hip', 'hostcodec.cpp', 'ply.cpp', 'mesh_io.cpp']
+           'child_irn_a32.hip', 'child_irn_b32.hip', 'child_q4.hip', 'rows_irn.hip', 'rows_q4.hip', 'unit_down.hip', 'conv_packed.hip', 'entropy.hip', 'loss.hip', 'occupancy.hip', 'occupancy_rans.hip', 'grad.hip', 'metric.hip', 'colour.hip', 'normals.hip', 'mesh.hip', 'collate.hip', 'hostcodec.cpp', 'ply.cpp', 'mesh_io.cpp']
 HEADERS = [os.path.join(CSRC, 'pcgc_common.h'), os.path.join(CSRC, 'mfma_util.h'), os.path.join(CSRC, 'child_kernels.h'), os.path.join(CSRC, 'child_q4.h'), os.path.join(CSRC, 'q4x.h'), os.path.join(CSRC, 'q4x_sched.h'), os.path.join(CSRC, 'rows_q4_policy.h'), os.path.join(CSRC, 'eb_logits.h'), os.path.join(CSRC, 'occupancy_tables.h'), os.path.join(HERE, '..', 'include', 'pcgc_hip.h')]
 FLAGS = ['--offload-arch=gfx950', '-O3', '-std=c++17', '-ffp-contract=off', '-fPIC', '-Wall', '-Wno-unused-result'] + \
         os.environ.get('PCGC_EXTRA_HIPCC_FLAGS', '').split()
diff --git a/pcgcv2_amd/_lib.py b/pcgcv2_amd/_lib.py
--- a/pcgcv2_amd/_lib.py
+++ b/pcgcv2_amd/_lib.py
@@ -31,15 +31,17 @@
     'pcgc_kmap_k3_prune_parent': (ci, [vp, i64, vp, vp, vp, i64, vp, vp]),
     'pcgc_kmap_k3_from_coarse': (ci, [vp, i64, i32, vp, vp, vp, i64, vp, vp]),
     'pcgc_down_maps': (ci, [vp, vp, vp, i64, i32, i64, vp, vp, vp]),
+    'pcgc_down_occupancy': (ci, [vp, i64, vp, vp]),
     'pcgc_down_prepare': (ci, [vp, i64, i32, vp, vp, vp, i64, vp, vp, vp, vp, vp, sz, vp]),
     'pcgc_down_finish': (ci, [vp, vp, vp, vp, vp, i64, i32, i64, vp, vp, vp, vp]),
     'pcgc_down_level': (ci, [vp, i64, i32, vp, vp, vp, i64, vp, vp, vp, vp, vp, sz, vp, vp, vp, vp, vp]),
     'pcgc_pyramid_scratch_bytes': (sz, [i64, ci]),
-    'pcgc_pyramid': (ci, [vp, i64, i32, ci, vp, sz, vp, vp, vp, vp, vp]),
+    'pcgc_pyramid': (ci, [vp, i64, i32, ci, vp, sz, vp, vp, vp, vp, vp, vp]),
     'pcgc_compact_index': (ci, [vp, vp, i64, vp, vp]),
     'pcgc_conv_gather': (ci, [vp, ci, i64, vp, i64, ci, ci, ci, vp, vp, vp, ci, ci, ci, vp, ci, ci, ci, vp]),
     'pcgc_conv_gather_unit': (ci, [vp, ci, i64, vp, vp, ci, vp, ci, ci, vp]),
     'pcgc_conv_unit_from_coarse': (ci, [vp, i64, i32, vp, vp, vp, i64, vp, vp, ci, vp, ci, ci, vp]),
+    'pcgc_conv_unit_down': (ci, [vp, vp, i64, vp, vp, vp, i64, vp, vp, ci, vp]),
     'pcgc_set_conv_impl': (ci, [ci]),
     'pcgc_last_conv_impl': (ci, []),
     'pcgc_set_up2_impl': (ci, [ci]),
diff --git a/pcgcv2_amd/autoencoder.py b/pcgcv2_amd/autoencoder.py
--- a/pcgcv2_amd/autoencoder.py
+++ b/pcgcv2_amd/autoencoder.py
@@ -73,8 +73,21 @@
         self.block2 = make_layer(InceptionResNet, 3, ch[4])
         self.conv3 = Conv(ch[4], ch[5], 3)
 
+    def _front(self, x):
+        c0, d0, cm = self.conv0, self.down0, x.cmap
+        hooked = c0._forward_hooks or c0._forward_pre_hooks or d0._forward_hooks or d0._forward_pre_hooks
+        if (ops.PATH.FUSE_UNIT_DOWN and not hooked and (c0.in_channels, c0.out_channels, d0.in_channels, d0.out_channels) == (1, 16, 16, 32)
+                and c0.bias is not None and d0.bias is not None and not ops.PROFILE.counting and x.F.shape[1] == 1 and cm.origin is None
+                and dispatch.select('conv3', (1, 16), x.F.shape[0], 'plain', extent=x.F.shape[0] * x.F.stride(0) * 4,
+                                    unit_input=x.has_unit_features(), plain_output=True).family == 'unit'
+                and cm.mapless_unit_conv()):
+            coarse, _ = cm.down()
+            y = ops.conv_unit_down(coarse.k3, cm.down_occupancy(), len(cm), c0.kernel, c0.bias, d0._table(ops.child_conv_table), d0.bias)
+            return SparseTensor(y, coordinate_map=coarse)
+        return d0(c0(x, relu=True), relu=True)
+
     def forward(self, x):
-        out0 = self.block0(self.down0(self.conv0(x, relu=True), relu=True))
+        out0 = self.block0(self._front(x))
         out1 = self.block1(self.down1(self.conv1(out0, relu=True), relu=True))
         out2 = self.block2(self.down2(self.conv2(out1, relu=True), relu=True))
         out2 = self.conv3(out2)
diff --git a/pcgcv2_amd/csrc/coords.hip b/pcgcv2_amd/csrc/coords.hip
--- a/pcgcv2_amd/csrc/coords.hip
+++ b/pcgcv2_amd/csrc/coords.hip
@@ -355,6 +355,21 @@
     PCGC_CHECK_LAUNCH("down_maps");
     return 0;
 }
+__global__ void k_down_occupancy(const int32_t* __restrict__ down, int64_t nc, uint8_t* __restrict__ occ) {
+    const int64_t p = (int64_t)blockIdx.x * blockDim.x + threadIdx.x;
+    if (p >= nc) return;
+    unsigned m = 0;
+#pragma unroll
+    for (int j = 0; j < 8; ++j) m |= (down[(int64_t)j * nc + p] >= 0 ? 1u : 0u) << j;
+    occ[p] = (uint8_t)m;
+}
+extern "C" int pcgc_down_occupancy(const int32_t* down, int64_t n_coarse, uint8_t* occ, void* stream) {
+    PCGC_REQUIRE(n_coarse == 0 || (down && occ), "null argument");
+    if (n_coarse == 0) return 0;
+    hipLaunchKernelGGL(k_down_occupancy, dim3(grid_for(n_coarse, 256)), dim3(256), 0, S(stream), down, n_coarse, occ);
+    PCGC_CHECK_LAUNCH("down_occupancy");
+    return 0;
+}
 extern "C" int pcgc_down_prepare(const int32_t* fine, int64_t n, int32_t stride_fine, int32_t* q, uint64_t* keys, int32_t* vals,
                                  int64_t cap, uint8_t* keep, int32_t* first_row, int32_t* prefix, int32_t* total, void* scan_ws,
                                  size_t scan_ws_bytes, void* stream) {
@@ -396,16 +411,28 @@
     int32_t s[PYR_MAX]; uint64_t cap_mask; int levels;
 };
 __device__ static inline int4 pyr_quantise(int4 c, int32_t s) { return make_int4(c.x, c.y / s * s, c.z / s * s, c.w / s * s); }
-__global__ void k_pyr_insert_level(const int4* __restrict__ fine, int64_t n, PyrArgs a, int l) {
+__global__ void k_pyr_step(const int4* __restrict__ fine, int64_t n, PyrArgs a, int lf, int li) {
     const int64_t i = (int64_t)blockIdx.x * blockDim.x + threadIdx.x;
     int4 c = make_int4(-1, -1, -1, -1);
-    bool ok = false;
-    if (i < n && (l == 0 || a.keep[l - 1][i])) { c = fine[i]; ok = coord_in_range(c.x, c.y, c.z, c.w); }
-    const int4 q = pyr_quantise(c, a.s[l]);
+    bool kept = i < n;
+    if (kept) c = fine[i];
+    if (lf >= 0 && kept) {
+        if (lf > 0 && !a.keep[lf - 1][i]) { a.keep[lf][i] = 0; kept = false; }
+        else {
+            const int4 q = pyr_quantise(c, a.s[lf]);
+            const int32_t f = hash_lookup(a.keys[lf], a.vals[lf], a.cap_mask, q.x, q.y, q.z, q.w);
+            a.first[lf][i] = f;
+            kept = f == (int32_t)i;
+            a.keep[lf][i] = kept;
+        }
+    }
+    if (li >= a.levels) return;
+    const bool ok = kept && coord_in_range(c.x, c.y, c.z, c.w);
+    const int4 q = pyr_quantise(c, a.s[li]);
     const uint64_t key = ok ? coord_key(q.x, q.y, q.z, q.w) : PCGC_EMPTY_KEY;
     const uint64_t left = __shfl_up((unsigned long long)key, 1, 64);
     if (!ok || ((threadIdx.x & 63) != 0 && left == key)) return;
-    uint64_t* keys = a.keys[l]; int32_t* vals = a.vals[l];
+    uint64_t* keys = a.keys[li]; int32_t* vals = a.vals[li];
     uint64_t h = hash_slot(key, a.cap_mask);
     for (;;) {
         unsigned long long prev = __builtin_nontemporal_load((const unsigned long long*)&keys[h]);
@@ -413,15 +440,6 @@
         if (prev == PCGC_EMPTY_KEY || prev == key) { if (__builtin_nontemporal_load(&vals[h]) > (int32_t)i) atomicMin(&vals[h], (int32_t)i); return; }
         h = (h + 1) & a.cap_mask;
     }
-}
-__global__ void k_pyr_first_level(const int4* __restrict__ fine, int64_t n, PyrArgs a, int l) {
-    const int64_t i = (int64_t)blockIdx.x * blockDim.x + threadIdx.x;
-    if (i >= n) return;
-    if (l > 0 && !a.keep[l - 1][i]) { a.keep[l][i] = 0; return; }
-    const int4 q = pyr_quantise(fine[i], a.s[l]);
-    const int32_t f = hash_lookup(a.keys[l], a.vals[l], a.cap_mask, q.x, q.y, q.z, q.w);
-    a.first[l][i] = f;
-    a.keep[l][i] = f == (int32_t)i;
 }
 
 struct PyrOut { int4* coarse[PYR_MAX]; int32_t* parent_of[PYR_MAX]; int32_t* down[PYR_MAX]; const int32_t* prefix[PYR_MAX]; int64_t count[PYR_MAX]; int32_t stride; };
@@ -442,12 +460,22 @@
         if (kept_below) { o.coarse[l][p] = pyr_quantise(c, a.s[l]); j = p; }
     }
 }
+__global__ void k_pyr_fill_down(PyrOut o, int levels) {
+    int64_t t = (int64_t)blockIdx.x * blockDim.x + threadIdx.x;
+#pragma unroll
+    for (int l = 0; l < PYR_MAX; ++l) {
+        if (l >= levels) return;
+        const int64_t m = 8 * o.count[l];
+        if (t < m) { o.down[l][t] = -1; return; }
+        t -= m;
+    }
+}
 extern "C" size_t pcgc_pyramid_scratch_bytes(int64_t n, int levels) {
     const size_t cap = (size_t)pcgc_hash_capacity(n), scan = (pcgc_scan_workspace_bytes(n) + 15) & ~(size_t)15, nn = ((size_t)n + 15) & ~(size_t)15;
     return 64 + (size_t)levels * (scan + cap * 12 + nn * 4 * 2 + nn) + 64;
 }
 extern "C" int pcgc_pyramid(const int32_t* fine, int64_t n, int32_t stride, int levels, void* scratch, size_t scratch_bytes,
-                            int32_t* const* coarse, int32_t* const* parent_of, int32_t* const* down, int64_t* counts, void* stream) {
+                            int32_t* const* coarse, int32_t* const* parent_of, int32_t* const* down, int64_t* counts, uint8_t* occ0, void* stream) {
     PCGC_REQUIRE(levels >= 1 && levels <= PYR_MAX, "1 to 4 levels");
     PCGC_REQUIRE(fine && scratch && coarse && parent_of && down && counts, "null argument");
     PCGC_REQUIRE(scratch_bytes >= pcgc_pyramid_scratch_bytes(n, levels) && ((uintptr_t)scratch & 15) == 0, "scratch too small or misaligned");
@@ -476,25 +504,25 @@
     if (e != hipSuccess) { pcgc_set_error("pyramid: %s", hipGetErrorString(e)); return -1; }
     hipLaunchKernelGGL(k_hash_clear, dim3(grid_for((int64_t)cap * levels, 256)), dim3(256), 0, s, keys0, vals0, (int64_t)cap * levels);
     const dim3 g(grid_for(n, 256)), b(256);
-    for (int l = 0; l < levels; ++l) {
-        hipLaunchKernelGGL(k_pyr_insert_level, g, b, 0, s, (const int4*)fine, n, a, l);
-        hipLaunchKernelGGL(k_pyr_first_level, g, b, 0, s, (const int4*)fine, n, a, l);
-    }
-    for (int l = 0; l < levels; ++l)
-        if ((rc = pcgc_mask_scan_zeroed(a.keep[l], n, prefix[l], totals + l, scan_ws[l], pcgc_scan_workspace_bytes(n), stream))) return rc;
+    for (int l = -1; l < levels; ++l) hipLaunchKernelGGL(k_pyr_step, g, b, 0, s, (const int4*)fine, n, a, l, l + 1);
+    if ((rc = pcgc_mask_scan_levels_zeroed(a.keep, n, levels, prefix, totals, scan_ws, stream))) return rc;
     static thread_local int32_t* host_total = nullptr;
     if (!host_total && hipHostMalloc((void**)&host_total, 64, hipHostMallocDefault) != hipSuccess) { host_total = nullptr; pcgc_set_error("pyramid: cannot allocate pinned memory"); return -1; }
     e = hipMemcpyAsync(host_total, totals, (size_t)levels * sizeof(int32_t), hipMemcpyDeviceToHost, s);
     if (e == hipSuccess) e = hipStreamSynchronize(s);
     if (e != hipSuccess) { pcgc_set_error("pyramid: %s", hipGetErrorString(e)); return -1; }
     PyrOut o; o.stride = stride;
+    int64_t fill = 0;
     for (int l = 0; l < levels; ++l) {
         counts[l] = host_total[l];
         o.coarse[l] = (int4*)coarse[l]; o.parent_of[l] = parent_of[l]; o.down[l] = down[l]; o.prefix[l] = prefix[l]; o.count[l] = counts[l];
-        if (counts[l] > 0 && (e = hipMemsetAsync(down[l], 0xFF, (size_t)counts[l] * 8 * sizeof(int32_t), s)) != hipSuccess) { pcgc_set_error("pyramid: %s", hipGetErrorString(e)); return -1; }
-    }
+        fill += 8 * counts[l];
+    }
+    for (int l = levels; l < PYR_MAX; ++l) { o.coarse[l] = nullptr; o.parent_of[l] = nullptr; o.down[l] = nullptr; o.prefix[l] = nullptr; o.count[l] = 0; }
+    if (fill > 0) hipLaunchKernelGGL(k_pyr_fill_down, dim3(grid_for(fill, 256)), b, 0, s, o, levels);
     hipLaunchKernelGGL(k_pyr_finish, g, b, 0, s, (const int4*)fine, n, a, o);
     PCGC_CHECK_LAUNCH("pyramid");
+    if (occ0) return pcgc_down_occupancy(down[0], counts[0], occ0, stream);
     return 0;
 }
 extern "C" int pcgc_compact_index(const uint8_t* mask, const int32_t* prefix, int64_t n, int32_t* orig, void* stream) {
diff --git a/pcgcv2_amd/csrc/pcgc_common.h b/pcgcv2_amd/csrc/pcgc_common.h
--- a/pcgcv2_amd/csrc/pcgc_common.h
+++ b/pcgcv2_amd/csrc/pcgc_common.h
@@ -5,6 +5,8 @@
 #include "../../include/pcgc_hip.h"
 
 void pcgc_set_error(const char* fmt, ...);
+int pcgc_mask_scan_levels_zeroed(uint8_t* const* masks, int64_t n, int levels, int32_t* const* prefix, int32_t* totals, void* const* workspaces,
+                                 void* stream);
 
 #define PCGC_CHECK_LAUNCH(name)                                                            \
     do {                                                                                   \
diff --git a/pcgcv2_amd/csrc/select.hip b/pcgcv2_amd/csrc/select.hip
--- a/pcgcv2_amd/csrc/select.hip
+++ b/pcgcv2_amd/csrc/select.hip
@@ -35,10 +35,8 @@
 }
 
 constexpr uint64_t SCAN_AGG = 1ull << 62, SCAN_INCL = 2ull << 62;
-__global__ void __launch_bounds__(256) k_scan_lookback(const uint8_t* __restrict__ mask, int64_t n, int64_t n_tiles,
-                                                       unsigned long long* desc, int32_t* ticket, int32_t* __restrict__ prefix,
-                                                       int32_t* total, const uint32_t* enable) {
-    if (enable && *enable == 0) return;
+__device__ __forceinline__ void scan_lookback_tile(const uint8_t* __restrict__ mask, int64_t n, int64_t n_tiles, unsigned long long* desc,
+                                                   int32_t* ticket, int32_t* __restrict__ prefix, int32_t* total) {
     __shared__ int tile_s, excl_s;
     if (threadIdx.x == 0) tile_s = atomicAdd(ticket, 1);
     __syncthreads();
@@ -78,6 +76,18 @@
 #pragma unroll
     for (int j = 0; j < 8; ++j) { if (base + j < n) prefix[base + j] = ex; ex += m[j]; }
 }
+__global__ void __launch_bounds__(256) k_scan_lookback(const uint8_t* __restrict__ mask, int64_t n, int64_t n_tiles,
+                                                       unsigned long long* desc, int32_t* ticket, int32_t* __restrict__ prefix,
+                                                       int32_t* total, const uint32_t* enable) {
+    if (enable && *enable == 0) return;
+    scan_lookback_tile(mask, n, n_tiles, desc, ticket, prefix, total);
+}
+constexpr int SCAN_LEVELS_MAX = 4;
+struct ScanLevels { const uint8_t* mask[SCAN_LEVELS_MAX]; unsigned long long* desc[SCAN_LEVELS_MAX]; int32_t* prefix[SCAN_LEVELS_MAX]; int32_t* total; };
+__global__ void __launch_bounds__(256) k_scan_lookback_levels(ScanLevels a, int64_t n, int64_t n_tiles) {
+    const int l = blockIdx.y;
+    scan_lookback_tile(a.mask[l], n, n_tiles, a.desc[l], (int32_t*)(a.desc[l] + n_tiles), a.prefix[l], a.total + l);
+}
 
 static int64_t scan_tiles(int64_t n) { return (n + SCAN_TILE - 1) / SCAN_TILE; }
 extern "C" size_t pcgc_scan_workspace_bytes(int64_t n) { return (size_t)(scan_tiles(n) + 2) * sizeof(uint64_t); }
@@ -94,6 +104,21 @@
     if (n == 0) return 0;
     launch_scan(mask, n, prefix, total, workspace, nullptr, S(stream));
     PCGC_CHECK_LAUNCH("mask_scan");
+    return 0;
+}
+int pcgc_mask_scan_levels_zeroed(uint8_t* const* masks, int64_t n, int levels, int32_t* const* prefix, int32_t* totals, void* const* workspaces,
+                                 void* stream) {
+    PCGC_REQUIRE(levels >= 1 && levels <= SCAN_LEVELS_MAX, "1 to 4 masks");
+    if (n == 0) return 0;
+    ScanLevels a; a.total = totals;
+    for (int l = 0; l < SCAN_LEVELS_MAX; ++l) {
+        const int m = l < levels ? l : 0;
+        PCGC_REQUIRE(((uintptr_t)workspaces[m] & 7) == 0, "workspace must be 8-byte aligned");
+        a.mask[l] = masks[m]; a.desc[l] = (unsigned long long*)workspaces[m]; a.prefix[l] = prefix[m];
+    }
+    const int64_t tiles = scan_tiles(n);
+    hipLaunchKernelGGL(k_scan_lookback_levels, dim3((unsigned)tiles, (unsigned)levels), dim3(256), 0, S(stream), a, n, tiles);
+    PCGC_CHECK_LAUNCH("mask_scan_levels");
     return 0;
 }
 extern "C" int pcgc_mask_scan(const uint8_t* mask, int64_t n, int32_t* prefix, int32_t* total, void* workspace,
diff --git a/pcgcv2_amd/csrc/unit_down.hip b/pcgcv2_amd/csrc/unit_down.hip
--- /dev/null
+++ b/pcgcv2_amd/csrc/unit_down.hip
@@ -0,0 +1,141 @@
+#include "mfma_util.h"
+
+namespace {
+
+__device__ __forceinline__ void wave_lds_sync() {
+    __builtin_amdgcn_fence(__ATOMIC_RELEASE, "wavefront");
+    __builtin_amdgcn_wave_barrier();
+    __builtin_amdgcn_fence(__ATOMIC_ACQUIRE, "wavefront");
+}
+
+constexpr int UD_NW = 4;
+constexpr int UD_SROW = 36;
+
+__global__ void __launch_bounds__(UD_NW * 64)
+k_unit_down(const int32_t* __restrict__ nbr , const uint8_t* __restrict__ occ , int64_t n_c, const float* __restrict__ W0,
+            const float* __restrict__ b0, const float* __restrict__ table, const float* __restrict__ b1, float* __restrict__ out, int out_ld) {
+    __shared__ __attribute__((aligned(16))) float tab_s[8 * 2 * 64 * 4];
+    __shared__ __attribute__((aligned(16))) float w0_s[27 * 4 * 4];
+    __shared__ __attribute__((aligned(16))) unsigned char occ_s[UD_NW][16 * 32];
+    __shared__ __attribute__((aligned(16))) float stage_s[UD_NW][16 * UD_SROW];
+    const int lane = threadIdx.x & 63, mi = lane & 15, mq = lane >> 4;
+    const int wave = __builtin_amdgcn_readfirstlane(threadIdx.x >> 6);
+    {
+        constexpr int NT4 = 8 * 2 * 64 / (UD_NW * 64);
+        float4 t4[NT4]; float w2[2];
+#pragma unroll
+        for (int i = 0; i < NT4; ++i) t4[i] = ((const float4*)table)[threadIdx.x + i * UD_NW * 64];
+#pragma unroll
+        for (int i = 0; i < 2; ++i) {
+            const int e = threadIdx.x + i * UD_NW * 64, ec = e < 27 * 16 ? e : 0;
+            w2[i] = W0[(ec >> 4) * 16 + 4 * (ec & 3) + ((ec >> 2) & 3)];
+        }
+#pragma unroll
+        for (int i = 0; i < NT4; ++i) ((float4*)tab_s)[threadIdx.x + i * UD_NW * 64] = t4[i];
+#pragma unroll
+        for (int i = 0; i < 2; ++i) if (threadIdx.x + i * UD_NW * 64 < 27 * 16) w0_s[threadIdx.x + i * UD_NW * 64] = w2[i];
+    }
+    __syncthreads();
+    float bias0[4];
+#pragma unroll
+    for (int jj = 0; jj < 4; ++jj) bias0[jj] = b0[4 * jj + mq];
+    const float bias1[2] = {b1[mi], b1[16 + mi]};
+    unsigned char* ob = occ_s[wave];
+    float* st = stage_s[wave];
+    const int64_t ntiles = (n_c + 15) >> 4;
+    for (int64_t tile = (int64_t)blockIdx.x * UD_NW + wave; tile < ntiles; tile += (int64_t)gridDim.x * UD_NW) {
+        const int64_t row0 = tile * 16, p = row0 + mi;
+        const bool valid = p < n_c;
+        const int64_t pc = valid ? p : 0;
+        int32_t q[7];
+#pragma unroll
+        for (int t = 0; t < 7; ++t) q[t] = nbr[(int64_t)(mq + 4 * t < 27 ? mq + 4 * t : 26) * n_c + pc];
+        unsigned char o[7];
+#pragma unroll
+        for (int t = 0; t < 7; ++t) o[t] = occ[q[t] > 0 ? q[t] : 0];
+#pragma unroll
+        for (int t = 0; t < 7; ++t) ob[mi * 32 + mq + 4 * t] = (valid && q[t] >= 0) ? o[t] : (unsigned char)0;
+        wave_lds_sync();
+        uint32_t w[8];
+        {
+            const uint4 lo = ((const uint4*)(ob + mi * 32))[0], hi = ((const uint4*)(ob + mi * 32))[1];
+            w[0] = lo.x; w[1] = lo.y; w[2] = lo.z; w[3] = lo.w; w[4] = hi.x; w[5] = hi.y; w[6] = hi.z; w[7] = hi.w;
+        }
+        float a[8][4];
+#pragma unroll
+        for (int j = 0; j < 8; ++j)
+#pragma unroll
+            for (int jj = 0; jj < 4; ++jj) a[j][jj] = 0.0f;
+        f32x4 wnext = *(const f32x4*)&w0_s[mq * 4];
+#pragma unroll
+        for (int k = 0; k < 27; ++k) {
+            const f32x4 wk = wnext;
+            if (k + 1 < 27) wnext = *(const f32x4*)&w0_s[((k + 1) * 4 + mq) * 4];
+#pragma unroll
+            for (int j = 0; j < 8; ++j) {
+                int kp, jn; child_offset(j, k, kp, jn);
+                const float f = (float)((w[kp >> 2] >> (8 * (kp & 3) + jn)) & 1u);
+#pragma unroll
+                for (int jj = 0; jj < 4; ++jj) a[j][jj] = fmaf(f, wk[jj], a[j][jj]);
+            }
+        }
+#pragma unroll
+        for (int j = 0; j < 8; ++j) {
+            const bool present = (w[13 >> 2] >> (8 * (13 & 3) + j)) & 1u;
+#pragma unroll
+            for (int jj = 0; jj < 4; ++jj) {
+                const float v = fmaxf(a[j][jj] + bias0[jj], 0.0f);
+                a[j][jj] = present ? v : 0.0f;
+            }
+        }
+        f32x4 acc[2] = {(f32x4){0.f, 0.f, 0.f, 0.f}, (f32x4){0.f, 0.f, 0.f, 0.f}};
+#pragma unroll
+        for (int j = 0; j < 8; ++j) {
+            const f32x4 bA = ((const f32x4*)tab_s)[(j * 2 + 0) * 64 + lane], bB = ((const f32x4*)tab_s)[(j * 2 + 1) * 64 + lane];
+#pragma unroll
+            for (int jj = 0; jj < 4; ++jj) {
+                acc[0] = __builtin_amdgcn_mfma_f32_16x16x4f32(a[j][jj], bA[jj], acc[0], 0, 0, 0);
+                acc[1] = __builtin_amdgcn_mfma_f32_16x16x4f32(a[j][jj], bB[jj], acc[1], 0, 0, 0);
+            }
+        }
+#pragma unroll
+        for (int t = 0; t < 2; ++t)
+#pragma unroll
+            for (int r = 0; r < 4; ++r) st[(4 * mq + r) * UD_SROW + 16 * t + mi] = acc[t][r] + bias1[t];
+        wave_lds_sync();
+#pragma unroll
+        for (int it = 0; it < 2; ++it) {
+            const int i = lane + 64 * it, lr = i >> 3, c4 = i & 7;
+            const int64_t row = row0 + lr;
+            if (row >= n_c) continue;
+            float4 v = *(const float4*)&st[lr * UD_SROW + 4 * c4];
+            v.x = fmaxf(v.x, 0.0f); v.y = fmaxf(v.y, 0.0f); v.z = fmaxf(v.z, 0.0f); v.w = fmaxf(v.w, 0.0f);
+            *(float4*)(out + row * out_ld + 4 * c4) = v;
+        }
+        wave_lds_sync();
+    }
+}
+
+}
+
+extern "C" int pcgc_conv_unit_down(const int32_t* nbr, const uint8_t* occ, int64_t n_coarse, const float* W0, const float* b0, const float* table,
+                                   int64_t table_bytes, const float* b1, float* out, int out_ld, void* stream) {
+    PCGC_REQUIRE(n_coarse == 0 || (nbr && occ && W0 && b0 && table && b1 && out), "null argument");
+    PCGC_REQUIRE(table_bytes == (int64_t)8 * 16 * 32 * 4, "table size");
+    PCGC_REQUIRE((((uintptr_t)table) & 15) == 0, "unaligned table");
+    PCGC_REQUIRE(out_ld >= 32 && (out_ld & 3) == 0 && (((uintptr_t)out) & 15) == 0, "output rows must be 16-byte aligned");
+    if (n_coarse == 0) return 0;
+    static int resident = 0;
+    if (!resident) {
+        hipDeviceProp_t pr; int dev = 0, per_cu = 0;
+        (void)hipGetDevice(&dev);
+        const int cus = (hipGetDeviceProperties(&pr, dev) == hipSuccess && pr.multiProcessorCount > 0) ? pr.multiProcessorCount : 256;
+        if (hipOccupancyMaxActiveBlocksPerMultiprocessor(&per_cu, k_unit_down, UD_NW * 64, 0) != hipSuccess || per_cu < 1) per_cu = 2;
+        resident = cus * per_cu;
+    }
+    const int64_t want = ((n_coarse + 15) / 16 + UD_NW - 1) / UD_NW;
+    const int64_t grid = want < (int64_t)resident ? want : (int64_t)resident;
+    hipLaunchKernelGGL(k_unit_down, dim3((unsigned)grid), dim3(UD_NW * 64), 0, S(stream), nbr, occ, n_coarse, W0, b0, table, b1, out, out_ld);
+    PCGC_CHECK_LAUNCH("conv_unit_down");
+    return 0;
+}
diff --git a/pcgcv2_amd/ops.py b/pcgcv2_amd/ops.py
--- a/pcgcv2_amd/ops.py
+++ b/pcgcv2_amd/ops.py
@@ -330,24 +330,27 @@
     return coarse_ub[:nc], parent_of, down_ub[:8 * nc].view(8, nc)
 
 
-def pyramid(fine, stride_fine, levels):
+def pyramid(fine, stride_fine, levels, want_occupancy=False):
     import ctypes
     fine = _i32(fine)
     n, dev = fine.shape[0], fine.device
     nbytes = int(lib().pcgc_pyramid_scratch_bytes(n, levels))
     scratch = torch.empty(nbytes, dtype=torch.uint8, device=dev)
-    outbuf = torch.empty(levels * 13 * n, dtype=torch.int32, device=dev)
+    outbuf = torch.empty(levels * 13 * n + (n + 3) // 4, dtype=torch.int32, device=dev)
+    occ_ub = outbuf[levels * 13 * n:].view(torch.uint8) if want_occupancy else None
     parts = [(outbuf[13 * n * l:13 * n * l + 4 * n].view(n, 4), outbuf[13 * n * l + 4 * n:13 * n * l + 5 * n], outbuf[13 * n * l + 5 * n:13 * n * (l + 1)])
              for l in range(levels)]
     ptrs = lambda k: (ctypes.c_void_p * levels)(*[p[k].data_ptr() for p in parts])
     counts = (ctypes.c_int64 * levels)()
-    check(lib().pcgc_pyramid(_p(fine), n, int(stride_fine), int(levels), _p(scratch), nbytes, ptrs(0), ptrs(1), ptrs(2), counts, _stream(fine)),
-          'pyramid')
+    check(lib().pcgc_pyramid(_p(fine), n, int(stride_fine), int(levels), _p(scratch), nbytes, ptrs(0), ptrs(1), ptrs(2), counts, _p(occ_ub),
+                             _stream(fine)), 'pyramid')
     out, below = [], n
     for l, (coarse_ub, parent_ub, down_ub) in enumerate(parts):
         nc = int(counts[l])
         out.append((coarse_ub[:nc], parent_ub[:below], down_ub[:8 * nc].view(8, nc)))
         below = nc
+    if want_occupancy:
+        return out, occ_ub[:int(counts[0])]
     return out
 
 
@@ -521,6 +524,35 @@
         e0.record()
     check(lib().pcgc_conv_unit_from_coarse(_p(_i32(fine)), n, int(stride_fine), _p(parent_of), _p(coarse_nbr), _p(down), coarse_nbr.shape[1],
                                            _p(W), _p(bias), int(relu), _p(out), Cout, Cout, _stream(fine)), 'conv_unit_from_coarse')
+    if prof:
+        e1.record()
+    return out
+
+
+def down_occupancy(down):
+    n_c = down.shape[1]
+    occ = torch.empty(n_c, dtype=torch.uint8, device=down.device)
+    check(lib().pcgc_down_occupancy(_p(down), n_c, _p(occ), _stream(down)), 'down_occupancy')
+    return occ
+
+
+def conv_unit_down(coarse_nbr, occ, n_fine, W0, b0, table, b1):
+    _f32(W0, 'W0')
+    if tuple(W0.shape) != (27, 1, 16) or table.numel() != 8 * 16 * 32 or b0 is None or b1 is None:
+        raise PcgcError('conv_unit_down: conv0 [27, 1, 16] and down0 [8, 16, 32], both with bias, expected')
+    n_c = coarse_nbr.shape[1]
+    out = torch.empty((n_c, 32), dtype=torch.float32, device=W0.device)
+    key = ('unit_down', 16, 32, n_c)
+    prof = PROFILE.want(key)
+    if prof:
+        e0, e1 = PROFILE.bracket(key, 'k_unit_down (k3 conv 1->16 on the unit input + k2 s2 16->32 in one kernel: presence from the stride-2 level\'s '
+                                 'map and occupancy bytes, fp32 MFMA)', n_fine,
+                                 lambda P, n=n_fine, m=n_c: 27 * m * 4 + 27 * m + P * 4 + n * 16 * 4 + m * 32 * 4,
+                                 lambda P, n=n_fine: 2 * P * 16 + 2 * n * 16 * 32,
+                                 compulsory=27 * n_c * 4 + n_c + n_c * 32 * 4, mfma_issued=2 * 8 * ((n_c + 15) // 16 * 16) * 16 * 32)
+        e0.record()
+    check(lib().pcgc_conv_unit_down(_p(coarse_nbr), _p(occ), n_c, _p(W0), _p(b0), _p(table), table.numel() * 4, _p(b1), _p(out), _ld(out),
+                                    _stream(coarse_nbr)), 'conv_unit_down')
     if prof:
         e1.record()
     return out
diff --git a/pcgcv2_amd/pathconfig.py b/pcgcv2_amd/pathconfig.py
--- a/pcgcv2_amd/pathconfig.py
+++ b/pcgcv2_amd/pathconfig.py
@@ -10,6 +10,7 @@
 class PathConfig:
     UNIT_INPUT_CONV: bool = True
     UNIT_CONV_MAPLESS: bool = True
+    FUSE_UNIT_DOWN: bool = True
     FUSE_IRN: bool = True
     ROWS_IRN64: bool = True
     ROWS_IRN64_MIN: int = 1024
diff --git a/pcgcv2_amd/sparse.py b/pcgcv2_amd/sparse.py
--- a/pcgcv2_amd/sparse.py
+++ b/pcgcv2_amd/sparse.py
@@ -26,6 +26,7 @@
         self._k3 = None
         self._down = None
         self._parent_of = None
+        self._down_occ = None
         self._unique = unique
         self._prepared_up = None
         self._batch_rows = None
@@ -90,13 +91,20 @@
             self._down = (CoordMap(coarse_C, 2 * self.stride, unique=True), down)
         return self._down
 
+    def down_occupancy(self):
+        if self._down_occ is None:
+            self._down_occ = ops.down_occupancy(self.down()[1])
+        return self._down_occ
+
     def build_pyramid(self, levels):
         chain, lvl = [], self
         while lvl._down is not None and len(chain) < levels:
             lvl = lvl._down[0]; chain.append(lvl)
         todo = levels - len(chain)
         if todo > 0:
-            for coarse_C, parent_of, down in ops.pyramid(lvl.C, lvl.stride, todo):
+            levels, occ = ops.pyramid(lvl.C, lvl.stride, todo, want_occupancy=True)
+            lvl._down_occ = occ
+            for coarse_C, parent_of, down in levels:
                 lvl._parent_of = parent_of
                 nxt = CoordMap(coarse_C, 2 * lvl.stride, unique=True)
                 lvl._down = (nxt, down)
@@ -125,7 +133,7 @@
         self._prepared_up = child
 
     def drop_caches(self):
-        self._table = self._k3 = self._down = self._parent_of = self._prepared_up = None
+        self._table = self._k3 = self._down = self._parent_of = self._down_occ = self._prepared_up = None
         self.__dict__.pop('_ingested', None)
 
 
```
